# MIT-SPARK/Kimera-Semantics

Measured on AMD Instinct MI355X. Metric: Mvoxel-updates/s + frames/s, 640×480 @5cm voxels, 1/2/4/8 MI355X, higher is better.
Workload: dtype f32; 1 GPU; bag-replay stand-in: 640x480 depth+label trajectory (room), 'fast' integrator, 5 cm voxels, 5 m rays, trunc 0.2 m, p=0.8; pipeline_frames=12, parallelism=frame-sharded x1, points_per_frame=305657, rays_per_frame=85307, updates_per_frame=502687

## Files before the change

include/ks_hip.h:

```cpp
#ifndef KS_HIP_H_
#define KS_HIP_H_

#include <stddef.h>
#include <stdint.h>

#ifdef __cplusplus
extern "C" {
#endif

#define KS_NUM_LABELS 21

enum {
  KS_OK = 0,
  KS_ERR_INVALID_ARG = -1,
  KS_ERR_LABEL_RANGE = -2,
  KS_ERR_PROBABILITY = -3,
  KS_ERR_HIP = -4,
  KS_ERR_POOL_FULL = -5,
  KS_ERR_INDEX_RANGE = -6,
  KS_ERR_NO_DEVICE = -7,
  KS_ERR_UNSUPPORTED = -8,
  KS_ERR_PEER_FAILED = -9
};

// ... 174 lines not shown
typedef struct ks_objects_config {
  float min_weight;
  float surface_distance_m;
  uint32_t label_mask;
  uint32_t min_voxels;
} ks_objects_config;
typedef struct ks_objects_stats {
  uint64_t voxels_surface, components, objects, voxels_in_objects, largest_object_voxels, workspace_bytes;
} ks_objects_stats;
typedef struct ks_object {
  int32_t first_voxel[3];
  uint32_t n_voxels;
  int32_t bb_min[3], bb_max[3];
  int64_t sum[3];
  uint32_t label, pad;
} ks_object;
#define KS_OBJECT_NONE 0xffffffffu
int ks_objects_default_config(ks_objects_config* cfg);
int ks_objects_update(ks_ctx* ctx, const ks_objects_config* cfg, ks_objects_stats* stats );
int ks_objects_size(ks_ctx* ctx, size_t* n);
int ks_objects_download(ks_ctx* ctx, ks_object* out, size_t cap, size_t* n);
int ks_objects_download_blocks(ks_ctx* ctx, const int32_t* idx_xyz, size_t n, uint32_t* out );
int ks_objects_query(ks_ctx* ctx, const float* xyz , size_t n, uint32_t* id);

#define KS_TILE_BYTES 65536
int ks_get_tile_keys(ks_ctx* ctx, uint64_t* out, size_t cap, size_t* n);
int ks_export_tiles_device(ks_ctx* ctx, const uint32_t* slots, size_t n, void* d_payload);
int ks_merge_tiles_device(ks_ctx* ctx, const uint64_t* keys, size_t n, const void* d_payload);
int ks_clear(ks_ctx* ctx);
int ks_clear_voxels(ks_ctx* ctx);
typedef struct ks_remove_stats {
  uint64_t blocks_removed, tiles_removed, tiles_moved, tiles_resident , pool_capacity_tiles;
} ks_remove_stats;
int ks_remove_blocks(ks_ctx* ctx, const int32_t* idx_xyz, size_t n, ks_remove_stats* stats );
int ks_remove_distant_blocks(ks_ctx* ctx, const float center[3], float max_distance_m, ks_remove_stats* stats );
int ks_removed_blocks(ks_ctx* ctx, int32_t* out_xyz, size_t cap, size_t* n);
typedef struct ks_fuse_config {
  float min_weight;
  uint32_t pad;
  uint64_t max_workspace_bytes;
} ks_fuse_config;
typedef struct ks_fuse_stats {
  uint64_t tiles_source, tiles_candidate, tiles_touched, tiles_allocated, voxels_fused, chunks, workspace_bytes;
} ks_fuse_stats;
int ks_fuse_default_config(ks_fuse_config* cfg);
int ks_fuse_map(ks_ctx* dst, ks_ctx* src, const float T_D_S[7], const ks_fuse_config* cfg, ks_fuse_stats* stats );

typedef struct ks_mesh_index_stats {
  uint64_t corners, vertices, max_corners_per_vertex, workspace_bytes;
} ks_mesh_index_stats;
int ks_mesh_index(ks_ctx* ctx, ks_mesh_index_stats* stats );
int ks_mesh_index_size(ks_ctx* ctx, size_t* n_vertices, size_t* n_indices);
int ks_mesh_index_download(ks_ctx* ctx, float* xyz, float* normals, uint8_t* rgba, uint8_t* labels, uint32_t* object_ids,
                           size_t cap_vertices, uint32_t* indices, size_t cap_indices);
int ks_reset_tiles(ks_ctx* ctx, const uint32_t* slots, size_t n);
int ks_tile_owner(uint64_t tile_key, int world);
typedef struct ks_reduce_stats {
  uint64_t tiles_sent, tiles_received, tiles_local, bytes_sent;
} ks_reduce_stats;
int ks_reduce(ks_ctx* ctx, void* rccl_comm, int rank, int world, ks_reduce_stats* stats);

typedef struct ks_round_stats {
  uint64_t updates_marched, updates_applied, bytes_sent, origin_voxel_touched, rays_cast;
} ks_round_stats;
int ks_integrate_round_exact(ks_ctx* marcher, ks_ctx* owner, void* rccl_comm, int rank, int world, uint64_t first_frame,
                             const float T_G_C[7], const float* xyz, const uint8_t* rgba, const uint8_t* labels, size_t n,
                             int freespace_points, ks_round_stats* stats);

int ks_debug_radix_sort(ks_ctx* ctx, void* keys, uint32_t* vals, size_t n, int key_bits, unsigned end_bit);
int ks_debug_radix_sort_range(ks_ctx* ctx, void* keys, uint32_t* vals, size_t n, int key_bits, unsigned begin_bit, unsigned end_bit);
int ks_debug_radix_sort_batch(ks_ctx* ctx, uint64_t* keys, uint32_t* vals, const uint64_t* counts, int nb, size_t cap,
                              unsigned begin_bit, unsigned end_bit);

int ks_synchronize(ks_ctx* ctx);
void* ks_stream(ks_ctx* ctx);
int ks_flush(ks_ctx* ctx, ks_frame_stats* stats);
int ks_profile_enable(ks_ctx* ctx, int level);
int ks_early_out_iterations(ks_ctx* ctx, uint64_t* frames, uint64_t* iterations);
int ks_early_out_stats(ks_ctx* ctx, uint64_t out[5]);
int ks_profile_get(ks_ctx* ctx, ks_profile* out, int reset);
int ks_update_stats(ks_ctx* ctx, uint64_t out[4]);
int ks_pipeline_shape(ks_ctx* ctx, int32_t out[4]);
int ks_stream_plan(ks_ctx* ctx, int32_t out[8]);
int ks_seed_launch_shape(int32_t integration_order_mode, int32_t early_out_phase_growth, uint64_t cap_points, uint32_t* out, int32_t max_phases);

#ifdef __cplusplus
}
#endif
#endif
```

kimera_semantics_amd/binding.py:

```python
from __future__ import annotations

import ctypes as C
import os
import subprocess

import numpy as np

_HERE = os.path.dirname(os.path.abspath(__file__))
LIB_PATH = os.environ.get("KS_HIP_LIB") or os.path.join(_HERE, "libks_hip.so")
NUM_LABELS = 21

KS_METHOD_FAST, KS_METHOD_MERGED = 0, 1
KS_COLOR_MODE_COLOR, KS_COLOR_MODE_SEMANTIC, KS_COLOR_MODE_SEMANTIC_PROBABILITY = 0, 1, 2
KS_ORDER_MIXED, KS_ORDER_SORTED, KS_ORDER_MIXED_1024_GROUPS = 0, 1, 2
KS_BUNDLE_ORDER_REFERENCE, KS_BUNDLE_ORDER_CANONICAL = 0, 1
KS_EARLY_OUT_EXACT = 1
KS_ERR_LABEL_RANGE, KS_ERR_PROBABILITY, KS_ERR_POOL_FULL, KS_ERR_NO_DEVICE, KS_ERR_UNSUPPORTED = -2, -3, -5, -7, -8
KS_ERR_INVALID_ARG, KS_ERR_PEER_FAILED = -1, -9
KS_ERR_HIP, KS_ERR_INDEX_RANGE = -4, -6

STAGES = ["points", "sort_points", "rays", "march", "emit", "sort_pairs", "apply", "apply_long"]

TSDF_DTYPE = np.dtype([("distance", "<f4"), ("weight", "<f4"), ("color", "u1", (4,))])
SEM_DTYPE = np.dtype([("label", "u1"), ("pad", "u1", (3,)), ("priors", "<f4", (NUM_LABELS,)),
                      ("color", "u1", (4,))])

ABI_SYMBOLS = [
    "ks_default_config", "ks_create", "ks_destroy", "ks_last_error", "ks_set_color_to_label",
    "ks_integrate_points", "ks_integrate_points_device", "ks_integrate_depth", "ks_integrate_depth_device", "ks_num_blocks", "ks_get_block_indices",
    "ks_get_updated_block_indices", "ks_count_updated_voxels", "ks_download_updated_voxels", "ks_download_blocks", "ks_upload_blocks", "ks_host_alloc", "ks_host_free", "ks_get_tile_keys", "ks_export_tiles_device", "ks_merge_tiles_device", "ks_clear", "ks_clear_voxels", "ks_reset_tiles", "ks_tile_owner", "ks_reduce",
    "ks_debug_radix_sort", "ks_debug_radix_sort_range", "ks_debug_radix_sort_batch", "ks_synchronize", "ks_flush", "ks_stream",
    "ks_profile_enable", "ks_profile_get", "ks_early_out_iterations", "ks_early_out_stats", "ks_pipeline_shape", "ks_stream_plan", "ks_seed_launch_shape", "ks_update_stats", "ks_integrate_round_exact",
    "ks_mesh_default_config", "ks_mesh_update", "ks_mesh_size", "ks_mesh_download", "ks_mesh_changed_blocks",
    "ks_esdf_default_config", "ks_esdf_update", "ks_esdf_download_blocks", "ks_esdf_query",
    "ks_esdf_refresh", "ks_esdf_changed_blocks",
    "ks_render_default_config", "ks_render_view", "ks_render_view_device",
    "ks_align_default_config", "ks_align_points", "ks_align_points_device",
    "ks_objects_default_config", "ks_objects_update", "ks_objects_size", "ks_objects_download", "ks_objects_download_blocks", "ks_objects_query",
    "ks_remove_blocks", "ks_remove_distant_blocks", "ks_removed_blocks",
    "ks_fuse_default_config", "ks_fuse_map",
    "ks_mesh_index", "ks_mesh_index_size", "ks_mesh_index_download",
]


class KsConfig(C.Structure):
    _fields_ = [
        ("voxel_size", C.c_float), ("voxels_per_side", C.c_int32),
        ("truncation_distance", C.c_float), ("max_weight", C.c_float),
        ("min_ray_length_m", C.c_float), ("max_ray_length_m", C.c_float),
        ("voxel_carving_enabled", C.c_int32), ("use_const_weight", C.c_int32),
        ("allow_clear", C.c_int32), ("use_weight_dropoff", C.c_int32),
        ("use_sparsity_compensation_factor", C.c_int32), ("sparsity_compensation_factor", C.c_float),
        ("enable_anti_grazing", C.c_int32), ("start_voxel_subsampling_factor", C.c_float),
        ("max_consecutive_ray_collisions", C.c_int32), ("clear_checks_every_n_frames", C.c_int32),
        ("integration_order_mode", C.c_int32), ("integrator_threads", C.c_int32),
        ("method", C.c_int32), ("bundle_order", C.c_int32),
        ("semantic_measurement_probability", C.c_float), ("color_mode", C.c_int32),
        ("n_dynamic_labels", C.c_int32), ("dynamic_labels", C.c_uint8 * 32),
        ("label_rgba", (C.c_uint8 * 4) * 256),
        ("early_out_phase_growth", C.c_int32),
        ("device_id", C.c_int32), ("max_tiles", C.c_uint32), ("max_points", C.c_uint32), ("pipeline_frames", C.c_int32),
    ]


class KsRoundStats(C.Structure):
    _fields_ = [("updates_marched", C.c_uint64), ("updates_applied", C.c_uint64), ("bytes_sent", C.c_uint64),
                ("origin_voxel_touched", C.c_uint64), ("rays_cast", C.c_uint64)]


class KsFrameStats(C.Structure):
    _fields_ = [("n_points", C.c_uint64), ("n_valid_points", C.c_uint64), ("n_rays_cast", C.c_uint64),
                ("n_voxel_updates", C.c_uint64), ("n_blocks_allocated", C.c_uint64)]


class KsReduceStats(C.Structure):
    _fields_ = [("tiles_sent", C.c_uint64), ("tiles_received", C.c_uint64), ("tiles_local", C.c_uint64),
                ("bytes_sent", C.c_uint64)]


class KsMeshConfig(C.Structure):
    _fields_ = [("min_weight", C.c_float), ("only_stale", C.c_int32)]


class KsMeshStats(C.Structure):
    _fields_ = [("blocks_meshed", C.c_uint64), ("blocks_total", C.c_uint64), ("triangles_total", C.c_uint64),
                ("triangles_changed", C.c_uint64), ("degenerate_dropped", C.c_uint64)]


MESH_BLOCK_DTYPE = np.dtype([("block", "<i4", (3,)), ("first_vertex", "<u4"), ("n_vertices", "<u4")])


class KsEsdfConfig(C.Structure):
    _fields_ = [("min_weight", C.c_float), ("min_distance_m", C.c_float), ("max_distance_m", C.c_float), ("use_region", C.c_int32),
                ("region_min", C.c_int32 * 3), ("region_max", C.c_int32 * 3), ("max_workspace_bytes", C.c_uint64)]


class KsEsdfStats(C.Structure):
    _fields_ = [("voxels_observed", C.c_uint64), ("voxels_fixed", C.c_uint64), ("voxels_clamped", C.c_uint64),
                ("box_voxels", C.c_uint64 * 3), ("workspace_bytes", C.c_uint64)]


class KsEsdfRefreshStats(C.Structure):
    _fields_ = [("tiles_stale", C.c_uint64), ("tiles_recomputed", C.c_uint64), ("tiles_total", C.c_uint64),
                ("voxels_observed", C.c_uint64), ("voxels_fixed", C.c_uint64), ("voxels_clamped", C.c_uint64),
                ("workspace_bytes", C.c_uint64)]


ESDF_DTYPE = np.dtype([("distance", "<f4"), ("flags", "u1"), ("label", "u1"), ("pad", "u1", (2,))])


class KsRenderConfig(C.Structure):
    _fields_ = [("min_weight", C.c_float), ("min_range_m", C.c_float), ("max_range_m", C.c_float)]


class KsRenderStats(C.Structure):
# ... 44 lines not shown


def object_centroids(records, voxel_size) -> np.ndarray:
    r = np.asarray(records)
    return (r["sum"].astype(np.float64) / np.maximum(r["n_voxels"], 1)[:, None].astype(np.float64) + 0.5) * float(voxel_size)


KS_ALIGN_CONVERGED, KS_ALIGN_ITERATION_LIMIT, KS_ALIGN_TOO_FEW_INLIERS, KS_ALIGN_DEGENERATE = 0, 1, 2, 3


class KsProfile(C.Structure):
    _fields_ = [("ms", C.c_double * 8), ("launches", C.c_uint64 * 8), ("frames", C.c_uint64),
                ("updates", C.c_uint64), ("points", C.c_uint64), ("apply_kernel_ms", C.c_double),
                ("apply_kernel_launches", C.c_uint64), ("apply_kernel_updates", C.c_uint64),
                ("host_ms", C.c_double), ("host_wait_ms", C.c_double)]


def build(force: bool = False) -> str:
    src_dir = os.path.join(_HERE, "csrc")
    srcs = [os.path.join(src_dir, f) for f in ("ks_hip.hip", "ks_types.h", "ks_k_rays.h", "ks_k_bundle_order.h", "ks_k_march.h", "ks_k_exact.h", "ks_k_apply.h",
                                                "ks_k_apply_xl.h", "ks_k_shard.h", "ks_k_shard_merged.h", "ks_k_io.h", "ks_k_mesh.h", "ks_k_mesh_index.h", "ks_k_esdf.h", "ks_k_render.h", "ks_k_align.h", "ks_k_objects.h", "ks_k_remove.h", "ks_k_fuse.h", "ks_mc_tri_table.inc", "ks_device_math.h", "ks_radix_sort.h", "ks_owned.h")]
    srcs.append(os.path.join(_HERE, "..", "include", "ks_hip.h"))
    stale = (not os.path.exists(LIB_PATH)) or any(
        os.path.exists(s) and os.path.getmtime(s) > os.path.getmtime(LIB_PATH) for s in srcs)
    if force or stale:
        subprocess.check_call(["make", "-C", src_dir])
    return LIB_PATH


_lib = None


def lib():
    global _lib
    if _lib is None:
        if not os.path.exists(LIB_PATH):
            raise RuntimeError(f"{LIB_PATH} is missing: run `python -c 'import __graft_entry__ as g; g.build()'` "
                               "(the HIP path has no CPU fallback)")
        L = C.CDLL(LIB_PATH)
        vp = C.c_void_p
        L.ks_default_config.argtypes = [C.POINTER(KsConfig)]
        L.ks_create.argtypes = [C.POINTER(KsConfig), C.POINTER(vp)]
        L.ks_destroy.argtypes = [vp]
        L.ks_destroy.restype = None
        L.ks_last_error.argtypes = [vp]
        L.ks_last_error.restype = C.c_char_p
        L.ks_set_color_to_label.argtypes = [vp, vp, vp, C.c_size_t]
        L.ks_integrate_points.argtypes = [vp, vp, vp, vp, vp, C.c_size_t, C.c_int, C.POINTER(KsFrameStats)]
        L.ks_integrate_points_device.argtypes = [vp, vp, vp, vp, vp, C.c_size_t, C.c_int, C.POINTER(KsFrameStats)]
        L.ks_integrate_depth.argtypes = [vp, vp, vp, C.c_int, vp, vp, C.c_int, C.c_int, vp, C.c_int, C.POINTER(KsFrameStats)]
        L.ks_integrate_depth_device.argtypes = [vp, vp, vp, C.c_int, vp, vp, C.c_int, C.c_int, vp, C.c_int, C.POINTER(KsFrameStats)]
        L.ks_num_blocks.argtypes = [vp, C.POINTER(C.c_size_t)]
        L.ks_get_block_indices.argtypes = [vp, vp, C.c_size_t, C.POINTER(C.c_size_t)]
        L.ks_get_updated_block_indices.argtypes = [vp, vp, C.c_size_t, C.POINTER(C.c_size_t), C.c_int]
        L.ks_download_blocks.argtypes = [vp, vp, C.c_size_t, vp, vp]
        L.ks_count_updated_voxels.argtypes = [vp, C.POINTER(C.c_size_t), C.POINTER(C.c_size_t)]
        L.ks_download_updated_voxels.argtypes = [vp, vp, C.c_size_t, C.POINTER(C.c_size_t), vp, C.c_size_t, C.POINTER(C.c_size_t)]
        L.ks_upload_blocks.argtypes = [vp, vp, C.c_size_t, vp, vp]
        L.ks_host_alloc.argtypes = [C.c_size_t]
        L.ks_host_alloc.restype = C.c_void_p
        L.ks_host_free.argtypes = [vp]
        L.ks_host_free.restype = None
        L.ks_get_tile_keys.argtypes = [vp, vp, C.c_size_t, C.POINTER(C.c_size_t)]
        L.ks_export_tiles_device.argtypes = [vp, vp, C.c_size_t, vp]
        L.ks_merge_tiles_device.argtypes = [vp, vp, C.c_size_t, vp]
        L.ks_clear.argtypes = [vp]
        L.ks_clear_voxels.argtypes = [vp]
        L.ks_reset_tiles.argtypes = [vp, vp, C.c_size_t]
        L.ks_tile_owner.argtypes = [C.c_uint64, C.c_int]
        L.ks_reduce.argtypes = [vp, vp, C.c_int, C.c_int, C.POINTER(KsReduceStats)]
        L.ks_debug_radix_sort.argtypes = [vp, vp, vp, C.c_size_t, C.c_int, C.c_uint]
        L.ks_debug_radix_sort_range.argtypes = [vp, vp, vp, C.c_size_t, C.c_int, C.c_uint, C.c_uint]
        L.ks_debug_radix_sort_batch.argtypes = [vp, vp, vp, vp, C.c_int, C.c_size_t, C.c_uint, C.c_uint]
        L.ks_synchronize.argtypes = [vp]
        L.ks_flush.argtypes = [vp, C.POINTER(KsFrameStats)]
        L.ks_stream.argtypes = [vp]
        L.ks_stream.restype = vp
        L.ks_profile_enable.argtypes = [vp, C.c_int]
        L.ks_profile_get.argtypes = [vp, C.POINTER(KsProfile), C.c_int]
        L.ks_early_out_iterations.argtypes = [vp, C.POINTER(C.c_uint64), C.POINTER(C.c_uint64)]
        L.ks_early_out_stats.argtypes = [vp, C.POINTER(C.c_uint64)]
        L.ks_pipeline_shape.argtypes = [vp, C.POINTER(C.c_int32)]
        L.ks_stream_plan.argtypes = [vp, C.POINTER(C.c_int32)]
        L.ks_seed_launch_shape.argtypes = [C.c_int32, C.c_int32, C.c_uint64, C.POINTER(C.c_uint32), C.c_int32]
        L.ks_update_stats.argtypes = [vp, C.POINTER(C.c_uint64)]
        L.ks_integrate_round_exact.argtypes = [vp, vp, vp, C.c_int, C.c_int, C.c_uint64, vp, vp, vp, vp, C.c_size_t, C.c_int, C.POINTER(KsRoundStats)]
        L.ks_mesh_default_config.argtypes = [C.POINTER(KsMeshConfig)]
        L.ks_mesh_update.argtypes = [vp, C.POINTER(KsMeshConfig), C.POINTER(KsMeshStats)]
        L.ks_mesh_size.argtypes = [vp, C.POINTER(C.c_size_t), C.POINTER(C.c_size_t)]
        L.ks_mesh_download.argtypes = [vp, vp, C.c_size_t, vp, vp, vp, vp, C.c_size_t]
        L.ks_mesh_changed_blocks.argtypes = [vp, vp, C.c_size_t, C.POINTER(C.c_size_t)]
        L.ks_esdf_default_config.argtypes = [C.POINTER(KsEsdfConfig)]
        L.ks_esdf_update.argtypes = [vp, C.POINTER(KsEsdfConfig), C.POINTER(KsEsdfStats)]
        L.ks_esdf_download_blocks.argtypes = [vp, vp, C.c_size_t, vp]
        L.ks_esdf_query.argtypes = [vp, vp, C.c_size_t, vp, vp, vp]
        L.ks_esdf_refresh.argtypes = [vp, C.c_uint64, C.POINTER(KsEsdfRefreshStats)]
        L.ks_esdf_changed_blocks.argtypes = [vp, vp, C.c_size_t, C.POINTER(C.c_size_t)]
        L.ks_render_default_config.argtypes = [C.POINTER(KsRenderConfig)]
        L.ks_render_view.argtypes = [vp, vp, vp, C.c_int, C.c_int, C.POINTER(KsRenderConfig), vp, vp, vp, vp, C.POINTER(KsRenderStats)]
        L.ks_render_view_device.argtypes = [vp, vp, vp, C.c_int, C.c_int, C.POINTER(KsRenderConfig), vp, vp, vp, vp, C.POINTER(KsRenderStats)]
        L.ks_align_default_config.argtypes = [C.POINTER(KsAlignConfig)]
        L.ks_align_points.argtypes = [vp, vp, vp, C.c_size_t, C.POINTER(KsAlignConfig), vp, C.POINTER(KsAlignStats)]
        L.ks_align_points_device.argtypes = [vp, vp, vp, C.c_size_t, C.POINTER(KsAlignConfig), vp, C.POINTER(KsAlignStats)]
        L.ks_objects_default_config.argtypes = [C.POINTER(KsObjectsConfig)]
        L.ks_objects_update.argtypes = [vp, C.POINTER(KsObjectsConfig), C.POINTER(KsObjectsStats)]
        L.ks_objects_size.argtypes = [vp, C.POINTER(C.c_size_t)]
        L.ks_objects_download.argtypes = [vp, vp, C.c_size_t, C.POINTER(C.c_size_t)]
        L.ks_objects_download_blocks.argtypes = [vp, vp, C.c_size_t, vp]
        L.ks_objects_query.argtypes = [vp, vp, C.c_size_t, vp]
        L.ks_remove_blocks.argtypes = [vp, vp, C.c_size_t, C.POINTER(KsRemoveStats)]
        L.ks_remove_distant_blocks.argtypes = [vp, vp, C.c_float, C.POINTER(KsRemoveStats)]
        L.ks_removed_blocks.argtypes = [vp, vp, C.c_size_t, C.POINTER(C.c_size_t)]
        L.ks_fuse_default_config.argtypes = [C.POINTER(KsFuseConfig)]
        L.ks_fuse_map.argtypes = [vp, vp, vp, C.POINTER(KsFuseConfig), C.POINTER(KsFuseStats)]
        L.ks_mesh_index.argtypes = [vp, C.POINTER(KsMeshIndexStats)]
        L.ks_mesh_index_size.argtypes = [vp, C.POINTER(C.c_size_t), C.POINTER(C.c_size_t)]
        L.ks_mesh_index_download.argtypes = [vp, vp, vp, vp, vp, vp, C.c_size_t, vp, C.c_size_t]
        _lib = L
    return _lib


def default_config(**overrides) -> KsConfig:
    cfg = KsConfig()
    lib().ks_default_config(C.byref(cfg))
    apply_overrides(cfg, **overrides)
    return cfg


def apply_overrides(cfg, **overrides):
    for k, v in overrides.items():
        if k == "dynamic_labels":
            cfg.n_dynamic_labels = len(v)
            for i, lab in enumerate(v):
                cfg.dynamic_labels[i] = int(lab)
        elif k == "label_rgba":
            arr = np.ascontiguousarray(np.asarray(v, dtype=np.uint8).reshape(256, 4))
            C.memmove(cfg.label_rgba, arr.ctypes.data, 1024)
        else:
            if not hasattr(cfg, k):
                raise AttributeError(k)
            setattr(cfg, k, v)
    return cfg


class KsError(RuntimeError):
    def __init__(self, code, msg):
        super().__init__(f"ks error {code}: {msg}")
        self.code = code


def _ptr(a):
    return None if a is None else a.ctypes.data


class HipIntegrator:

    def __init__(self, cfg: KsConfig):
        self.cfg = cfg
        self.vps = cfg.voxels_per_side
        self._h = C.c_void_p()
        rc = lib().ks_create(C.byref(cfg), C.byref(self._h))
        if rc != 0:
            raise KsError(rc, lib().ks_last_error(None).decode())

    def _chk(self, rc):
        if rc != 0:
# ... 357 lines not shown
        return stats

    def reset_tiles(self, slots: np.ndarray):
        s = np.ascontiguousarray(slots, dtype=np.uint32)
        self._chk(lib().ks_reset_tiles(self._h, _ptr(s), len(s)))

    def reduce(self, rccl_comm, rank: int, world: int) -> dict:
        st = KsReduceStats()
        self._chk(lib().ks_reduce(self._h, C.c_void_p(rccl_comm) if rccl_comm else None, rank, world, C.byref(st)))
        return {"tiles_sent": st.tiles_sent, "tiles_received": st.tiles_received, "tiles_local": st.tiles_local,
                "bytes_sent": st.bytes_sent}

    def debug_radix_sort(self, keys: np.ndarray, vals=None, end_bit=None):
        keys = np.ascontiguousarray(keys).copy()
        bits = keys.dtype.itemsize * 8
        vals = None if vals is None else np.ascontiguousarray(vals, dtype=np.uint32).copy()
        self._chk(lib().ks_debug_radix_sort(self._h, _ptr(keys), _ptr(vals), keys.shape[0], bits,
                                            bits if end_bit is None else end_bit))
        return keys, vals

    def debug_radix_sort_range(self, keys: np.ndarray, vals=None, begin_bit=0, end_bit=None):
        keys = np.ascontiguousarray(keys).copy()
        bits = keys.dtype.itemsize * 8
        vals = None if vals is None else np.ascontiguousarray(vals, dtype=np.uint32).copy()
        self._chk(lib().ks_debug_radix_sort_range(self._h, _ptr(keys), _ptr(vals), keys.shape[0], bits, begin_bit,
                                                  bits if end_bit is None else end_bit))
        return keys, vals

    def debug_radix_sort_batch(self, keys: np.ndarray, vals: np.ndarray, counts, begin_bit, end_bit):
        keys = np.ascontiguousarray(keys, dtype=np.uint64).copy()
        vals = np.ascontiguousarray(vals, dtype=np.uint32).copy()
        counts = np.ascontiguousarray(counts, dtype=np.uint64)
        nb, cap = keys.shape
        assert vals.shape == (nb, cap) and counts.shape == (nb,)
        self._chk(lib().ks_debug_radix_sort_batch(self._h, _ptr(keys), _ptr(vals), _ptr(counts), nb, cap, begin_bit, end_bit))
        return keys, vals

    def synchronize(self):
        self._chk(lib().ks_synchronize(self._h))

    @property
    def stream(self) -> int:
        return lib().ks_stream(self._h) or 0

    def profile_enable(self, level=1):
        self._chk(lib().ks_profile_enable(self._h, int(level)))

    def early_out_stats(self):
        out = (C.c_uint64 * 5)()
        self._chk(lib().ks_early_out_stats(self._h, out))
        return dict(frames=int(out[0]), rounds=int(out[1]), fallbacks=int(out[2]), event_driven=bool(out[3]), pipelined=bool(out[4]))

    def integrate_round_exact(self, marcher: "HipIntegrator", rccl_comm, rank: int, world: int, first_frame: int, T_G_C, xyz, rgba, labels,
                              freespace=False) -> dict:
        T = np.ascontiguousarray(T_G_C, dtype=np.float32)
        n = 0 if xyz is None else len(xyz)
        x = None if xyz is None else np.ascontiguousarray(xyz, dtype=np.float32)
        c = None if rgba is None else np.ascontiguousarray(rgba, dtype=np.uint8)
        l = None if labels is None else np.ascontiguousarray(labels, dtype=np.uint8)
        st = KsRoundStats()
        self._chk(lib().ks_integrate_round_exact(marcher._h, self._h, rccl_comm, int(rank), int(world), int(first_frame), _ptr(T),
                                                 _ptr(x) if x is not None else None, _ptr(c) if c is not None else None,
                                                 _ptr(l) if l is not None else None, n, int(bool(freespace)), C.byref(st)))
        return dict(updates_marched=int(st.updates_marched), updates_applied=int(st.updates_applied), bytes_sent=int(st.bytes_sent),
                    origin_voxel_touched=bool(st.origin_voxel_touched), rays_cast=int(st.rays_cast))

    def update_stats(self):
        out = (C.c_uint64 * 4)()
        self._chk(lib().ks_update_stats(self._h, out))
        return dict(walked=int(out[0]), serial=int(out[1]), chunks=int(out[2]), replayed=int(out[3]))

    def pipeline_shape(self):
        out = (C.c_int32 * 4)()
        self._chk(lib().ks_pipeline_shape(self._h, out))
        return dict(lag=int(out[0]), slots=int(out[1]), batch=int(out[2]), march_streams=int(out[3]))

    def stream_plan(self):
        out = (C.c_int32 * 8)()
        self._chk(lib().ks_stream_plan(self._h, out))
        side = {1: "own", 0: "tail", -1: "none"}
        return dict(budget=int(out[0]), streams=int(out[1]), march_streams=int(out[2]), long=side[int(out[3])], xlong=side[int(out[4])],
                    march="own" if out[5] else "A", tail="own" if out[6] else "A", streams_held=int(out[7]))

    def early_out_iterations(self):
        f, it = C.c_uint64(), C.c_uint64()
        self._chk(lib().ks_early_out_iterations(self._h, C.byref(f), C.byref(it)))
        return f.value, it.value

    def flush(self) -> KsFrameStats:
        st = KsFrameStats()
        self._chk(lib().ks_flush(self._h, C.byref(st)))
        return st

    def profile(self, reset=False) -> dict:
        p = KsProfile()
        self._chk(lib().ks_profile_get(self._h, C.byref(p), int(reset)))
        return {"ms": {STAGES[i]: p.ms[i] for i in range(8)}, "launches": {STAGES[i]: p.launches[i] for i in range(8)},
                "frames": p.frames, "updates": p.updates, "points": p.points,
                "apply_kernel_ms": p.apply_kernel_ms, "apply_kernel_launches": p.apply_kernel_launches,
                "apply_kernel_updates": p.apply_kernel_updates, "host_ms": p.host_ms, "host_wait_ms": p.host_wait_ms}
```

kimera_semantics_amd/csrc/ks_hip.hip:

```cpp

#include <atomic>
#include <chrono>
#include <condition_variable>
#include <mutex>
#include <thread>
#include <cstring>
#include <string.h>

#include <dlfcn.h>
#include <hip/hip_runtime.h>
#include <hip/hip_ext.h>
#include <rccl/rccl.h>

#include <algorithm>
#include <iterator>
#include <cmath>
#include <cstdio>
#include <cstring>
#include <string>
#include <unordered_map>
#include <vector>

#include "../../include/ks_hip.h"
#include "ks_device_math.h"
// ... 18 lines not shown
#include "ks_k_render.h"
#include "ks_k_align.h"
#include "ks_k_objects.h"
#include "ks_k_remove.h"
#include "ks_k_fuse.h"

using namespace ksk;

namespace {

std::string g_create_error;

const char* dbg_env(const char* name) {
  const char* g = getenv("KS_DEBUG");
  return (g && g[0] == '1') ? getenv(name) : nullptr;
}

}

constexpr int kMaxLag = 16;
constexpr int kSlots = kMaxLag + 8;
constexpr int kMarchStreams = 8;
constexpr int kObsTables = 16;
struct HostSnap {
  Counters c;
  uint32_t n_tiles;
  uint32_t pad[7];
};
struct FrameSlot {
  int index = 0;
  DevBuf<RayDesc> d_rays;
  DevBuf<float> d_deltas;
  DevBuf<uint64_t> d_pairs;
  DevBuf<uint32_t> d_cnt;
  DevBuf<uint32_t> d_lp;
  DevBuf<unsigned long long> d_bt;
  DevBuf<uint8_t> d_live;
  DevBuf<uint32_t> d_seed_gen, d_seed_items, d_seed_n;
  bool wide = false;
  DevBuf<FrameParams> d_F;
  DevBuf<uint64_t> d_gkeys, d_rkeys;
  struct GraphSet {
    hipGraphExec_t g1 = nullptr, g2 = nullptr, g3 = nullptr;
    uint64_t key = 0;
    GraphSet() = default;
    GraphSet(const GraphSet&) = delete;
    GraphSet& operator=(const GraphSet&) = delete;
    ~GraphSet() { reset(); }
    void reset() {
      for (hipGraphExec_t* g : {&g1, &g2, &g3}) {
        if (*g) (void)hipGraphExecDestroy(*g);
        *g = nullptr;
      }
      key = 0;
    }
  } b_graphs[2];
  DevBuf<uint64_t> d_eo_keys[2];
  DevBuf<uint32_t> d_eo_vals[2];
  size_t eo_cap_marks = 0;
  DevBuf<uint4> d_eo_tab;
  DevBuf<unsigned long long> d_eo_xnode;
  DevBuf<uint32_t> d_eo_cnt_b, d_eo_ux, d_eo_dirty, d_eo_list[2], d_eo_chg, d_eo_consulted, d_eo_lp;
  DevBuf<unsigned long long> d_eo_bt;
  DevBuf<EoCtl> d_eo_ctl;
  DevBuf<uint32_t> d_eo_sort_ws;
  DevBuf<uint32_t> d_eo_hseq, d_eo_where;
  DevBuf<uint4> d_eo_rinfo, d_eo_ckpt;
  DevBuf<uint8_t> d_eo_hitb;
  DevBuf<unsigned long long> d_eo_bits_a, d_eo_bits_b;
  DevBuf<unsigned long long> d_eo_btp;
  Event eo_committed;
  Counters* d_counters = nullptr;
  DevBuf<uint32_t> d_ray_list;
  PinnedBuf<HostSnap> h_snap;
  Event a_done;
  Event ready;
  Event tail_done;
  Event fork, join;
  Event join_x;
  Event found;
  bool tail_recorded = false;
  bool join_recorded = false;
  bool b_launched = false;
  size_t steps_max = 0;
  uint64_t frame_no = 0;
  FrameParams F{};
  size_t n = 0;
  int prof_set = -1;
  bool pending = false;
  const Counters& counters() const { return h_snap->c; }
  uint32_t n_tiles() const { return h_snap->n_tiles; }
};

constexpr int kProfSets = 32;
constexpr int kStageEvents = KS_STAGE_COUNT + 3;
struct ProfSet {
  Event ev[kStageEvents];
  Event k0, k1;
  bool used = false, complete = false, stages = false, apply = false, applied = false;
  uint64_t n_pairs = 0, n_points = 0;
};

struct StreamPlanIn {
  bool uses_early_out = false;
  bool exact_early_out = false;
  bool frames_independent = true;
  int pipeline_frames = 0;
  int batch = 1;
  bool xlong = true;
  int budget = 4;
};
struct StreamPlan {
  int budget = 4;
  int n_march = 1;
  bool march_own = false;
  bool tail_own = false;
  bool long_own = true;
  bool xlong_own = true;
  int distinct = 1;
};
inline StreamPlan stream_plan(const StreamPlanIn& in) {
  StreamPlan p;
  p.budget = in.budget;
  if (in.pipeline_frames) {
    p.n_march = (!in.frames_independent || in.batch > 1) ? 1 : std::min(kMarchStreams, std::max(4, in.pipeline_frames));
    if (in.exact_early_out && p.n_march > 4) p.n_march = 4;
    if (in.exact_early_out && in.batch > 1) p.n_march = 2;
    if (!in.uses_early_out) p.n_march = 1;
    p.march_own = in.uses_early_out;
    p.tail_own = true;
  }
  p.long_own = true;
  p.xlong_own = in.xlong;
  auto count = [&p] { return 1 + (p.march_own ? p.n_march : 0) + (p.tail_own ? 1 : 0) + (p.long_own ? 1 : 0) + (p.xlong_own ? 1 : 0); };
  if (p.budget < 8 && count() > p.budget) p.xlong_own = false;
  if (p.budget < 8 && count() > p.budget) p.long_own = false;
  p.distinct = count();
  return p;
}
inline int hw_queue_budget() {
  auto number = [](const char* s, int* out) {
    if (!s) return false;
    char* end = nullptr;
    const long v = strtol(s, &end, 10);
    if (end == s) return false;
    *out = (int)std::min<long>(32, std::max<long>(1, v));
    return true;
  };
  int b = 4;
  number(getenv("GPU_MAX_HW_QUEUES"), &b);
  number(dbg_env("KS_HW_QUEUES"), &b);
  return b;
}

struct ks_ctx {
  Stream streams[kMarchStreams + 4];
  int n_streams = 0;
  ks_config cfg{};
  std::string err;
  hipStream_t stream = nullptr;
  hipStream_t stream_march_[kMarchStreams] = {};
  int n_march = 1;
  int batch = 1;
  std::vector<FrameSlot*> batch_slots;
  hipStream_t prof_march_stream = nullptr;
  hipStream_t stream_tail = nullptr;
  hipStream_t stream_long = nullptr;
  hipStream_t stream_xlong = nullptr;
  StreamPlan plan;
  bool xlong = true;
  float voxel_size_inv = 0.f, log_match = 0.f, log_non_match = 0.f;
  int vps_shift = 1;

  TileTable table{};
  Pool pool{};
  DevBuf<TileEntry> table_ent;
  DevBuf<uint64_t> table_slot_keys;
  DevBuf<uint4> pool_vox;
  DevBuf<uint8_t> pool_updated, pool_dirty;
  DevBuf<uint64_t> d_start_set;
  DevBuf<uint64_t> d_observed_[kObsTables];
  int n_obs = 1;
  uint64_t start_offset = 0, observed_offset = 0;
  int64_t reset_counter = 0;
  uint32_t obs_tag = 0, obs_tag_lo = 1;
  DevBuf<Counters> d_retry_counters;
  std::atomic<size_t> pairs_hint{0};
  bool uses_early_out = false;
  std::vector<SeedPhase> seed_phases;
  DevBuf<SeedPhase> d_seed_phases;
  size_t seed_cap_items = 0;
  std::thread tail_thread;
  std::mutex tail_mu;
  std::mutex capture_mu;
  std::condition_variable tail_cv;
  FrameSlot* tail_job = nullptr;
  bool tail_busy = false, tail_quit = false;
  int tail_rc = KS_OK;
  bool use_tail_thread = false;
  bool use_graphs = true;
  bool test_overlap = true;
  std::atomic<uint64_t> buffers_epoch{1};
  DevBuf<uint8_t> d_color_lut;
  DevBuf<uint32_t> d_label_lut;
  uint32_t tiles_initialised = 0;

  size_t cap_points = 0;
  DevBuf<float> d_xyz;
  DevBuf<uint8_t> d_rgba;
  DevBuf<uint8_t> d_labels;
  DevBuf<uint32_t> d_hash;
  DevBuf<uint32_t> d_skeys32, d_skeys32b;
  DevBuf<float4> d_gpw;
  DevBuf<uint64_t> d_ray_keys;
  DevBuf<uint2> d_glc;
  DevBuf<unsigned long long> d_long_list_[2];
  DevBuf<uint32_t> d_blong;
  std::atomic<uint32_t> bo_hint{~0u};
  bool bo_hint_fixed = false;
  DevBuf<uint64_t> d_key_overflow;
  uint32_t key_overflow_mask = 0;
  uint32_t key_bits = 0;
  DevBuf<uint64_t> d_pkeys, d_pkeys2;
  DevBuf<uint32_t> d_pvals, d_pvals2;
  DevBuf<uint32_t> d_order;
  DevBuf<uint32_t> d_inv_order;
  DevBuf<uint32_t> d_okeys, d_okeys2, d_ovals;
  size_t cap_pairs = 0;
  DevBuf<uint64_t> d_pairs2_[2];
  hipEvent_t pending_join = nullptr;
  ksrs::Workspace sort_ws, sort_ws_tail;
  bool exact_early_out = false;
  DevBuf<uint64_t> d_eo_keys[2];
  DevBuf<uint32_t> d_eo_vals[2];
  size_t cap_marks = 0;
  DevBuf<uint2> d_eo_range;
  DevBuf<uint64_t> d_eo_plain;
  DevBuf<uint32_t> d_eo_lp;
  DevBuf<unsigned long long> d_eo_bt;
  DevBuf<EoState> d_eo_state;
  PinnedBuf<EoState> h_eo_state;
  uint64_t eo_iterations = 0, eo_frames = 0;
  bool eo_device = false;
  int eo_bulk_rounds = 6;
  static constexpr int eo_sweeps = 12;
  int eo_sweep_chunks = 16;
  std::atomic<int> eo_want_bulk{0};
  DevBuf<uint32_t> d_eo_committed;
  uint32_t eo_frame_no = 0;
  hipEvent_t eo_last_commit = nullptr;
  std::atomic<size_t> eo_want_marks{0}, eo_want_x{0};
  size_t eo_cap_marks = 0, eo_cap_x = 0;
  std::atomic<uint64_t> eo_fallbacks{0};
  uint64_t eo_fallbacks_seen = 0;
  std::atomic<int> eo_hopeless{0};
  bool eo_device_off = false;
  bool use_bundle_rank = false;
  BoCtx bo{};
  BoSchedule bo_sched{};
  DevBuf<uint8_t> d_bo_slab;
  int bo_epochs = 0;
  DevBuf<int32_t> d_rx_counts;
  DevBuf<uint64_t> d_tx_keys, d_rx_keys;
  DevBuf<uint32_t> d_tx_slots;
  DevBuf<uint8_t> d_tx_payload, d_rx_payload;
  size_t cap_tx = 0, cap_rx = 0;
  DevBuf<uint32_t> d_xchg_u32;
  DevBuf<uint64_t> d_xchg_u64;
  DevBuf<uint8_t> d_state;
  FrameSlot slot[kSlots];
  int n_slots = 1;
  uint64_t frame_no = 0;
  ks_frame_stats owed{};
  DevBuf<int32_t> d_block_idx;
  DevBuf<uint8_t> d_tsdf_out, d_sem_out;
  DevBuf<uint8_t> d_vox_out;
  size_t cap_out_blocks = 0;

  DevBuf<uint32_t> d_depth_blocks;
  DevBuf<uint8_t> d_img_depth;
  DevBuf<uint8_t> d_img_aux;

  int profiling = 0;
  unsigned long long apply_runs_min_pairs = 1ull << 20;
  bool xl_parallel = true;
  unsigned long long xl_min_pairs = 1ull << 23;
  DevBuf<XlRun> d_xl_runs;
  DevBuf<XlHeader> d_xl_hdr;
  DevBuf<XlChunk> d_xl_chunks;
  DevBuf<uint32_t> d_xl_idx;
  bool shard_export = false;
  int shard_world = 1;
  uint64_t shard_frames_seen = 0;
  DevBuf<uint64_t> d_sh_okey[2];
  DevBuf<uint64_t> d_sh_gkey[2];
  DevBuf<uint32_t> d_sh_seq[2];
  DevBuf<float> d_sh_sdf[2];
  DevBuf<float> d_sh_uw[2];
  DevBuf<uint32_t> d_sh_counts;
  size_t cap_sh = 0;
  uint32_t sh_counts[65] = {0};
  uint64_t sh_exported = 0;
  DevBuf<uint64_t> d_sh_tk;
  DevBuf<uint64_t> d_sh_pairs[2];
  DevBuf<uint32_t> d_sh_vals[2];
  size_t cap_sh_rx = 0;
  DevBuf<uint32_t> d_shm_bno;
  DevBuf<float2> d_shm_btab;
  DevBuf<uint32_t> d_shm_mpos;
  DevBuf<uint32_t> d_shm_cnt;
  size_t cap_shm_n = 0;
  DevBuf<float> d_shm_mixed;
// ... 280 lines not shown
      if ((rc = c->slot[i].d_gkeys.alloc(c, cap))) return rc;
      if ((rc = c->slot[i].d_rkeys.alloc(c, cap))) return rc;
    }
    if (c->cfg.method == KS_METHOD_MERGED && (rc = c->slot[i].d_deltas.alloc(c, cap * kNumLabels))) return rc;
  }
  if ((rc = c->d_hash.alloc(c, cap))) return rc;
  if ((rc = c->d_skeys32.alloc(c, cap))) return rc;
  if ((rc = c->d_skeys32b.alloc(c, cap))) return rc;
  if ((rc = c->d_pkeys.alloc(c, cap))) return rc;
  if ((rc = c->d_pkeys2.alloc(c, cap))) return rc;
  if ((rc = c->d_pvals.alloc(c, cap))) return rc;
  if ((rc = c->d_pvals2.alloc(c, cap))) return rc;
  if ((rc = c->d_order.alloc(c, cap))) return rc;
  if ((rc = c->d_inv_order.alloc(c, cap))) return rc;
  if ((rc = c->d_okeys.alloc(c, cap))) return rc;
  if ((rc = c->d_okeys2.alloc(c, cap))) return rc;
  if ((rc = c->d_ovals.alloc(c, cap))) return rc;
  if (c->cfg.method == KS_METHOD_MERGED) {
    if ((rc = c->d_gpw.alloc(c, cap))) return rc;
    if ((rc = c->d_glc.alloc(c, cap))) return rc;
    if ((rc = c->d_ray_keys.alloc(c, cap))) return rc;
    if ((rc = c->d_blong.alloc(c, cap / kLongRun + 64))) return rc;
    if (c->key_bits) {
      size_t slots = 1024;
      while (slots < 2 * cap) slots <<= 1;
      if ((rc = c->d_key_overflow.alloc(c, slots))) return rc;
      HIPCHK(c, hipMemsetAsync(c->d_key_overflow, 0, slots * sizeof(uint64_t), c->stream));
      c->key_overflow_mask = (uint32_t)(slots - 1);
    }
  }
  if (c->use_bundle_rank && (rc = ensure_bundle_order(c, cap))) return rc;
  if (c->exact_early_out) {
    if ((rc = c->d_eo_lp.alloc(c, cap))) return rc;
    if ((rc = c->d_eo_bt.alloc(c, cap / kScanBlock + 2))) return rc;
    if ((rc = ensure_exact_points(c, cap))) return rc;
  }
  c->cap_points = cap;
  return KS_OK;
}

int ensure_pairs_in(ks_ctx* c, FrameSlot& S, size_t bound) {
  if (bound <= S.d_pairs.size()) return KS_OK;
  if (int rc = S.d_pairs.alloc(c, std::max<size_t>(bound, 1 << 20))) return rc;
  ++c->buffers_epoch;
  return KS_OK;
}
int ensure_pairs_out(ks_ctx* c, size_t n) {
  if (n <= c->cap_pairs) return KS_OK;
  const size_t cap = std::max<size_t>(n + n / 4, 1 << 20);
  c->cap_pairs = 0;
  int rc;
  HIPCHK(c, hipStreamSynchronize(c->stream_long));
  if (c->stream_xlong) HIPCHK(c, hipStreamSynchronize(c->stream_xlong));
  if (c->stream_tail) HIPCHK(c, hipStreamSynchronize(c->stream_tail));
  for (int b = 0; b < 2; ++b) {
    if ((rc = c->d_pairs2_[b].alloc(c, cap))) return rc;
    if ((rc = c->d_long_list_[b].alloc(c, cap / kLongRunLanes + 64 + cap / kXLongRun + 64))) return rc;
    if (c->long_lanes && (rc = c->d_long_sorted_[b].alloc(c, cap / kLongRunLanes + 64))) return rc;
  }
  if (c->d_xl_hdr && (rc = c->d_xl_fb.alloc(c, cap / kXLongRun + 64))) return rc;
  c->cap_pairs = cap;
  return KS_OK;
}

template <typename K>
int sort_keys(ks_ctx* c, K* a, K* b, size_t n, unsigned end_bit, K** result, unsigned begin_bit = 0, bool tail = false) {
  HIPCHK(c, (ksrs::sort<K, false>(tail ? c->sort_ws_tail : c->sort_ws, a, b, nullptr, nullptr, n, end_bit,
                                  tail ? c->stream_tail : c->stream, result, nullptr, begin_bit)));
  return KS_OK;
}
template <typename K>
int sort_pairs(ks_ctx* c, K* ka, K* kb, uint32_t* va, uint32_t* vb, size_t n, unsigned end_bit, K** kres,
               uint32_t** vres, unsigned begin_bit = 0) {
  HIPCHK(c, (ksrs::sort<K, true>(c->sort_ws, ka, kb, va, vb, n, end_bit, c->stream, kres, vres, begin_bit)));
  return KS_OK;
}

inline unsigned bits_for(uint64_t n) {
  unsigned b = 1;
  while (b < 64 && (1ull << b) < n) ++b;
  return b;
}

int launch_batch(ks_ctx* c);
int quiesce(ks_ctx* c);
int reset_set(ks_ctx* c, uint64_t* d_set0, uint64_t* offset, bool observed) {
  const bool full = ++(*offset) >= kFullResetThreshold;
  const bool retag = observed && !full && c->obs_tag + (uint32_t)c->cfg.clear_checks_every_n_frames + 2u >= kObsMaxTag;
  if (full || retag) {
    if (int rc = launch_batch(c)) return rc;
    if (full && c->exact_early_out) {
      if (int rc = quiesce(c)) return rc;
    }
    if (int rc = sync_march(c)) return rc;
    if (full) *offset = 0;
    for (int t = 0; t < (observed ? c->n_obs : 1); ++t) {
      uint64_t* d_set = observed ? c->d_observed_[t] : d_set0;
      if (full) {
        HIPCHK(c, hipMemsetAsync(d_set, 0, (observed ? 2 : 1) * (sizeof(uint64_t) << kSetBits), c->stream));
        const uint64_t poison = observed ? kObsPoison : ~0ull;
        HIPCHK(c, hipMemcpyAsync(d_set, &poison, sizeof(poison), hipMemcpyHostToDevice, c->stream));
      } else {
        hipLaunchKernelGGL(k_obs_retag, dim3((2u << kSetBits) / 256), dim3(256), 0, c->stream, d_set);
      }
    }
    if (observed && full && c->d_eo_plain) {
      HIPCHK(c, hipMemsetAsync(c->d_eo_plain, 0, sizeof(uint64_t) << kSetBits, c->stream));
      const uint64_t poison = ~0ull;
      HIPCHK(c, hipMemcpyAsync(c->d_eo_plain, &poison, sizeof(poison), hipMemcpyHostToDevice, c->stream));
    }
    HIPCHK(c, hipStreamSynchronize(c->stream));
    if (observed) c->obs_tag = 0;
  }
  if (observed) c->obs_tag_lo = c->obs_tag + 1;
  return KS_OK;
}

inline void stage_mark(ks_ctx* c, int set, int ev) {
  if (set >= 0 && c->pset[set].stages)
    (void)hipEventRecord(c->pset[set].ev[ev], ev <= 3 ? c->stream : ev <= 5 ? c->prof_march_stream : c->stream_tail);
}

void resolve_prof(ks_ctx* c, int set) {
  ProfSet& P = c->pset[set];
  if (!P.used || !P.complete) return;
  (void)hipEventSynchronize(P.ev[kStageEvents - 1]);
  if (P.stages) {
    for (int s = 0; s < KS_STAGE_COUNT; ++s) {
      float ms = 0.f;
      const int a = s < 3 ? s : s == 3 ? 4 : s + 2;
      if (hipEventElapsedTime(&ms, P.ev[a], P.ev[a + 1]) == hipSuccess) {
        c->prof.ms[s] += ms;
        c->prof.launches[s] += 1;
      }
    }
  }
  if (P.applied) {
    float kms = 0.f;
    if (hipEventElapsedTime(&kms, P.k0, P.k1) == hipSuccess) {
      c->prof.apply_kernel_ms += kms;
      c->prof.apply_kernel_launches += 1;
      c->prof.apply_kernel_updates += P.n_pairs;
    }
  }
  c->prof.frames += 1;
  c->prof.updates += P.n_pairs;
  c->prof.points += P.n_points;
  P.used = P.complete = P.applied = false;
}

SlotView slot_view(const FrameSlot& S, Counters* counters = nullptr) {
  SlotView v{};
  v.F = S.d_F;
  v.rays = S.d_rays;
  v.cnt = S.d_cnt;
  v.lp = S.d_lp;
  v.bt = S.d_bt;
  v.ray_list = S.d_ray_list;
  v.pairs = S.d_pairs;
  v.pairs_cap = (unsigned long long)S.d_pairs.size();
  v.C = counters ? counters : S.d_counters;
  v.host_snap = (uint32_t*)S.h_snap.get();
  v.eo_stats = S.d_eo_ctl ? &S.d_eo_ctl->n_x : nullptr;
  v.seed_gen = S.d_seed_gen;
  v.seed_items = S.d_seed_items;
  v.seed_n = S.d_seed_n;
  return v;
}

void launch_emit(ks_ctx* c, const BatchView& V, uint32_t nb, bool wide, hipStream_t st) {
  const size_t n = c->cap_points;
  const size_t lds = ((2 * n + kScanBlock - 1) / kScanBlock) * sizeof(unsigned long long);
  if (!(c->cfg.method == KS_METHOD_MERGED && c->cfg.enable_anti_grazing)) {
    if (wide || c->cfg.method == KS_METHOD_MERGED || !c->uses_early_out) {
      hipLaunchKernelGGL(k_emit_lane<8>, dim3((uint32_t)((n + 31) / 32), nb), dim3(256), lds, st, V, c->table, c->pool);
    } else {
      hipLaunchKernelGGL(k_emit_lane<16>, dim3((uint32_t)((n + 63) / 64), nb), dim3(256), lds, st, V, c->table, c->pool);
    }
  } else if (wide) {
    hipLaunchKernelGGL(k_emit<64>, dim3((uint32_t)((n + 3) / 4), nb), dim3(256), lds, st, V, c->table, c->pool);
  } else {
    hipLaunchKernelGGL(k_emit<16>, dim3((uint32_t)((n + 15) / 16), nb), dim3(256), lds, st, V, c->table, c->pool);
  }
}

void enqueue_stage_b(ks_ctx* c, const BatchView& V, uint32_t nb, bool wide, hipStream_t sm, size_t steps_max, int part = 0) {
  const ks_config& cfg = c->cfg;
  const size_t n = c->cap_points;
  if (c->uses_early_out && part != 2) {
    for (size_t j = 0; j < c->seed_phases.size(); ++j) {
      const SeedPhase& P = c->seed_phases[j];
      if (P.item_cap == 0) continue;
      const uint32_t steps_cap = (uint32_t)((steps_max + 3) & ~(size_t)3);
      const size_t lds_wave = (size_t)test_lds_words64(steps_cap) * sizeof(unsigned long long);
      const uint32_t wpb = lds_wave * 4 <= 60 * 1024 ? 4u : lds_wave * 2 <= 60 * 1024 ? 2u : 1u;
      const dim3 grid((P.item_cap + wpb - 1) / wpb, nb), block(64 * wpb);
      if (c->test_overlap) hipLaunchKernelGGL(k_test<true>, grid, block, lds_wave * wpb, sm, V, P.g0, P.g1, (uint32_t)j, P.item_off, P.item_cap, steps_cap);
      else hipLaunchKernelGGL(k_test<false>, grid, block, lds_wave * wpb, sm, V, P.g0, P.g1, (uint32_t)j, P.item_off, P.item_cap, steps_cap);
    }
  }
  if (part == 1) return;
  if (cfg.method == KS_METHOD_MERGED && cfg.enable_anti_grazing)
    hipLaunchKernelGGL(k_count_grazing<16>, dim3((uint32_t)((n + 15) / 16), nb), dim3(256), 0, sm, V);
  hipLaunchKernelGGL(k_scan_local, dim3((uint32_t)(((cfg.method == KS_METHOD_MERGED ? 2 : 1) * n + kScanBlock - 1) / kScanBlock), nb),
                     dim3(1024), 0, sm, V);
  launch_emit(c, V, nb, wide, sm);
  hipLaunchKernelGGL(k_publish, dim3(nb), dim3(64), 0, sm, V, (const uint32_t*)c->table.n_tiles);
}

int ensure_marks(ks_ctx* c, size_t n) {
  if (n <= c->cap_marks) return KS_OK;
  const size_t cap = std::max<size_t>(n + n / 4, 1 << 20);
  c->cap_marks = 0;
  int rc;
  for (int b = 0; b < 2; ++b) {
    if ((rc = c->d_eo_keys[b].alloc(c, cap))) return rc;
    if ((rc = c->d_eo_vals[b].alloc(c, cap))) return rc;
  }
  c->cap_marks = cap;
  return KS_OK;
}
constexpr int kEoMaxIterations = 4096;
int exact_early_out(ks_ctx* c, FrameSlot& S, hipStream_t st, Counters* counters = nullptr) {
  const size_t n = S.n;
  Counters* const d_counters = counters ? counters : S.d_counters;
// ... 240 lines not shown
        going = going || (w[0] != 0u && w[1] == 0u);
      }
      if (!going || chunk >= c->eo_sweep_chunks) break;
      enqueue_sweeps(c, Bt, nb, c->eo_sweeps, sm);
    }
    hipLaunchKernelGGL(k_eo2_sweep_done, dim3(nb), dim3(64), 0, sm, Bt);
    return KS_OK;
  }
  int exact_device() const {
    int rc;
    auto seed_and_rounds = [&] {
      enqueue_stage_b(c, V, nb, S0.wide, sm, steps_max, 1);
      return enqueue_exact_rounds(c, slots, nb, sm);
    };
    auto finish = [&] {
      for (uint32_t k = 0; k < nb; ++k) enqueue_exact_finish(c, *slots[k], sm);
      return KS_OK;
    };
    auto emission = [&] { return enqueue_stage_b(c, V, nb, S0.wide, sm, steps_max, 2), KS_OK; };
    bool graphs = c->use_graphs && !S0.wide;
    if (graphs && (G.key != key || !G.g1 || !G.g2 || !G.g3)) {
      std::lock_guard<std::mutex> cap(c->capture_mu);
      G.reset();
      if ((G.g1 = capture_graph(sm, seed_and_rounds)) && (G.g2 = capture_graph(sm, finish)) && (G.g3 = capture_graph(sm, emission))) {
        G.key = key;
      } else {
        (void)hipGetLastError();
        G.reset();
        c->use_graphs = graphs = false;
      }
    }
    if (graphs) HIPCHK(c, hipGraphLaunch(G.g1, sm));
    else if ((rc = seed_and_rounds()) || (S0.wide && (rc = sweeps_host_driven()))) return rc;
    if (c->eo_last_commit && c->eo_last_commit != S0.eo_committed) HIPCHK(c, hipStreamWaitEvent(sm, c->eo_last_commit, 0));
    if (graphs) HIPCHK(c, hipGraphLaunch(G.g2, sm));
    else finish();
    HIPCHK(c, hipEventRecord(S0.eo_committed, sm));
    c->eo_last_commit = S0.eo_committed;
    if (graphs) HIPCHK(c, hipGraphLaunch(G.g3, sm));
    else emission();
    return KS_OK;
  }
  int exact_host() const {
    enqueue_stage_b(c, V, nb, S0.wide, sm, steps_max, 1);
    if (int rc = exact_early_out(c, S0, sm)) return rc;
    enqueue_stage_b(c, V, nb, S0.wide, sm, steps_max, 2);
    return KS_OK;
  }
  int plain_or_replayed() const {
    if (c->use_graphs && (G.key != key || !G.g1)) {
      std::lock_guard<std::mutex> cap(c->capture_mu);
      G.reset();
      if ((G.g1 = capture_graph(sm, [&] { return enqueue_stage_b(c, V, nb, S0.wide, sm, steps_max), KS_OK; }))) {
        G.key = key;
      } else {
        (void)hipGetLastError();
        c->use_graphs = false;
      }
    }
    if (c->use_graphs && G.g1) HIPCHK(c, hipGraphLaunch(G.g1, sm));
    else enqueue_stage_b(c, V, nb, S0.wide, sm, steps_max);
    return KS_OK;
  }
};

int launch_batch(ks_ctx* c) {
  if (c->batch_slots.empty()) return KS_OK;
  std::vector<FrameSlot*> slots;
  slots.swap(c->batch_slots);
  const uint32_t nb = (uint32_t)slots.size();
  FrameSlot& S0 = *slots[0];
  hipStream_t sm = c->batch > 1 ? c->stream_march_[(S0.frame_no / (uint64_t)c->batch) % (uint64_t)c->n_march] : march_stream(c, S0.frame_no);
  c->prof_march_stream = sm;
  if (sm != c->stream) HIPCHK(c, hipStreamWaitEvent(sm, slots[nb - 1]->a_done, 0));
  const bool stage_events = nb == 1 && S0.prof_set >= 0 && c->pset[S0.prof_set].stages;
  if (stage_events) (void)hipEventRecord(c->pset[S0.prof_set].ev[4], sm);
  BatchView V{};
  size_t steps_max = 0;
  ParamsBatch PB{};
  for (uint32_t k = 0; k < nb; ++k) {
    FrameSlot& S = *slots[k];
    S.F.observed = observed_table(c, S.frame_no);
    if (c->exact_early_out) S.F.eo_frame = c->eo_frame_no++;
    PB.F[k] = S.F;
    PB.out[k] = S.d_F;
    V.s[k] = slot_view(S);
    steps_max = std::max(steps_max, S.steps_max);
  }
  if (nb == 1) hipLaunchKernelGGL(k_set_params, dim3(1), dim3(64), 0, sm, slots[0]->F, slots[0]->d_F);
  else hipLaunchKernelGGL(k_set_params_batch, dim3(nb), dim3(64), 0, sm, PB);
  const uint64_t key = ((uint64_t)c->cap_points << 24) ^ (c->buffers_epoch.load() << 4) ^ (S0.wide ? 1u : 0u) ^ ((uint64_t)nb << 1);
  const BatchLaunch B{c, slots.data(), nb, S0, sm, V, steps_max, key, S0.b_graphs[nb == (uint32_t)c->batch ? 0 : 1]};
  if (int rc = !c->exact_early_out ? B.plain_or_replayed() : c->eo_device && !c->eo_device_off ? B.exact_device() : B.exact_host()) return rc;
  for (uint32_t k = 0; k < nb; ++k) {
    HIPCHK(c, hipEventRecord(slots[k]->ready, sm));
    slots[k]->b_launched = true;
  }
  if (stage_events) (void)hipEventRecord(c->pset[S0.prof_set].ev[5], sm);
  return KS_OK;
}

void fill_frame_params(ks_ctx* c, FrameParams& F, const float Tq[7], size_t n, int freespace) {
  const ks_config& cfg = c->cfg;
  F = FrameParams{};
  F.T.w = Tq[0];
  F.T.v = {Tq[1], Tq[2], Tq[3]};
  F.T.t = {Tq[4], Tq[5], Tq[6]};
  F.voxel_size_inv = c->voxel_size_inv;
  F.min_ray = cfg.min_ray_length_m;
  F.max_ray = cfg.max_ray_length_m;
  F.trunc = cfg.truncation_distance;
  F.start_inv = cfg.start_voxel_subsampling_factor * c->voxel_size_inv;
  F.log_match = c->log_match;
  F.log_non_match = c->log_non_match;
  F.tsdf.voxel_size = cfg.voxel_size;
  F.tsdf.trunc = cfg.truncation_distance;
  F.tsdf.max_weight = cfg.max_weight;
  F.tsdf.dropoff_denominator = cfg.truncation_distance - cfg.voxel_size;
  F.tsdf.sparsity_factor = cfg.sparsity_compensation_factor;
  F.tsdf.use_dropoff = cfg.use_weight_dropoff;
  F.tsdf.use_sparsity = cfg.use_sparsity_compensation_factor;
  F.start_offset = c->start_offset;
  F.observed_offset = c->observed_offset;
  F.obs_tag = c->obs_tag;
  F.obs_tag_lo = c->obs_tag_lo;
  F.max_collisions = cfg.max_consecutive_ray_collisions;
  F.n = (uint32_t)n;
  const uint32_t q = (uint32_t)(n / kOrderStep);
  const bool by_1024 = cfg.integration_order_mode == KS_ORDER_MIXED_1024_GROUPS;
  F.order_groups = q == 0 ? 1u : by_1024 ? kOrderStep : q;
  F.order_per = q == 0 ? 0u : by_1024 ? q : kOrderStep;
  F.chains = order_chains(cfg.integration_order_mode, n);
  F.carving = cfg.voxel_carving_enabled;
  F.allow_clear = cfg.allow_clear;
  F.freespace = freespace;
  F.use_const_weight = cfg.use_const_weight;
  F.method = cfg.method;
  F.color_mode = cfg.color_mode;
  F.sorted_order = cfg.integration_order_mode == KS_ORDER_SORTED;
  F.n_dynamic = cfg.n_dynamic_labels;
  const unsigned pb = bits_for(n);
  F.point_mask = (1u << pb) - 1u;
  F.clear_bit = (cfg.method == KS_METHOD_MERGED) ? (1u << pb) : 0u;
  F.seq_bits = pb + (cfg.method == KS_METHOD_MERGED ? 1u : 0u);
  F.inv_order = F.sorted_order ? c->d_inv_order : nullptr;
  std::memcpy(F.dynamic_labels, cfg.dynamic_labels, 32);
  F.early_out = c->uses_early_out;
}
void begin_prof_set(ks_ctx* c, FrameSlot& S, size_t n) {
  const int set = (int)(c->frame_no % kProfSets);
  resolve_prof(c, set);
  ProfSet& P = c->pset[set];
  P.used = true;
  P.complete = P.applied = false;
  P.stages = c->profiling == 1;
  P.apply = c->profiling == 1 || (c->frame_no % 4) == 0;
  P.n_points = n;
  P.n_pairs = 0;
  S.prof_set = set;
}
int stage_a_fast(ks_ctx* c, FrameSlot& S, const float* d_xyz, const uint8_t* d_rgba, const uint8_t* d_labels, size_t n) {
  const FrameParams& F = S.F;
  hipStream_t st = c->stream;
  const uint32_t nb1k = (uint32_t)((n + 1023) / 1024);
  hipLaunchKernelGGL(k_points_fast, dim3(nb1k), dim3(1024), 0, st, F, d_xyz, d_rgba, d_labels, c->d_color_lut,
                     S.d_rays, c->d_hash, c->d_skeys32, c->d_pvals, S.d_cnt, S.d_live, S.d_counters);
  stage_mark(c, S.prof_set, 1);
  uint32_t *sk = nullptr, *sv = nullptr;
  if (int rc = sort_pairs(c, c->d_skeys32.get(), c->d_skeys32b.get(), c->d_pvals.get(), c->d_pvals2.get(), n, kSetBits + 1, &sk, &sv)) return rc;
  stage_mark(c, S.prof_set, 2);
  hipLaunchKernelGGL(k_dedup, dim3(nb1k), dim3(1024), 0, st, F, sk, sv, c->d_hash, c->d_start_set, S.d_ray_list, S.d_rays, S.d_cnt, S.d_live, S.d_counters);
  if (c->uses_early_out && n > 0) {
    const uint32_t n_gen = (uint32_t)((n + F.chains - 1) / F.chains);
    uint32_t n_ph = 0;
    while (n_ph < c->seed_phases.size() && c->seed_phases[n_ph].g0 < n_gen) ++n_ph;
    HIPCHK(c, hipMemsetAsync(S.d_seed_n, 0, c->seed_phases.size() * sizeof(uint32_t), st));
    hipLaunchKernelGGL(k_seed_list, dim3((F.chains + 63u) / 64u, n_ph), dim3(64 * kSeedSegs), 0, st, F, (const SeedPhase*)c->d_seed_phases,
                       (const uint8_t*)S.d_live, S.d_seed_gen, S.d_seed_items, S.d_seed_n, S.d_counters);
  }
  hipLaunchKernelGGL(k_dedup_commit, dim3(nb1k), dim3(1024), 0, st, F, sk, sv, c->d_hash, c->d_start_set, S.d_counters);
  return KS_OK;
}
void enqueue_bundle_order(ks_ctx* c, hipStream_t st, size_t n, const uint64_t* sk, const uint32_t* sv) {
  const uint32_t capb = (uint32_t)((c->cap_points + kBoBlock - 1) / kBoBlock);
  const size_t lds_f = (2 * c->cap_points / kBoBlock + 3) * sizeof(uint32_t), lds_e = ((size_t)capb + 2) * sizeof(uint32_t);
  hipLaunchKernelGGL(k_bo_scan_flags, dim3((uint32_t)((2 * n + kBoBlock - 1) / kBoBlock)), dim3(kBoBlock), 0, st, (uint32_t)n, c->bo);
  hipLaunchKernelGGL(k_bo_init, dim3((uint32_t)((n + kBoBlock - 1) / kBoBlock)), dim3(kBoBlock), lds_f, st, (uint32_t)n, sk, sv, c->bo);
  const uint32_t nbb = (uint32_t)((n + kBoBlock - 1) / kBoBlock);
  int e_small = 0;
  while (e_small < c->bo_epochs && c->bo_sched.b[e_small] <= kBoSmallBuckets) ++e_small;
  if (e_small > 0) hipLaunchKernelGGL(k_bo_small, dim3(2), dim3(kBoBlock), 0, st, c->bo, e_small);
  const size_t nh_floor = c->bo_hint_fixed ? (e_small > 0 ? (size_t)c->bo_sched.t[e_small - 1] + 1 : 1) : 2 * (size_t)kBoSmallBuckets;
  const size_t nh = std::min<size_t>(n, std::max<size_t>(c->bo_hint.load(std::memory_order_relaxed), nh_floor));
  int e_last = -1;
  for (int e = e_small; e <= c->bo_epochs; ++e) {
    if (e > 0 && c->bo_sched.t[e - 1] >= nh) break;
    hipLaunchKernelGGL(k_bo_link, dim3(nbb, 2), dim3(kBoBlock), lds_e, st, c->bo, e, (e == e_small && e_small > 0) ? 1 : 0);
    if (e < c->bo_epochs && c->bo_sched.t[e] < nh)
      hipLaunchKernelGGL(k_bo_walk, dim3(nbb, 2), dim3(kBoBlock), 0, st, c->bo, e);
    else
      e_last = e;
  }
  if (nh < n && e_last >= 0 && e_last < c->bo_epochs) hipLaunchKernelGGL(k_bo_rest, dim3(2), dim3(kBoBlock), lds_e, st, c->bo, e_last);
}
int stage_a_merged(ks_ctx* c, FrameSlot& S, const float* d_xyz, const uint8_t* d_rgba, const uint8_t* d_labels, size_t n, const uint32_t* order_ptr) {
  const ks_config& cfg = c->cfg;
  FrameParams& F = S.F;
  hipStream_t st = c->stream;
  const uint32_t nb = (uint32_t)((n + 255) / 256);
  const uint32_t nb1k = (uint32_t)((n + 1023) / 1024);
  if (c->key_bits) {
    const float reach = cfg.max_ray_length_m + 2.0f * cfg.voxel_size;
    const float tq[3] = {F.T.t.x, F.T.t.y, F.T.t.z};
    for (int a = 0; a < 3; ++a) {
      const float lo = std::floor((tq[a] - reach) * c->voxel_size_inv) - 2.0f;
      F.key_base[a] = (int32_t)std::min(std::max(lo, -2.0e9f), 2.0e9f);
    }
    F.key_bits = c->key_bits;
  }
  hipLaunchKernelGGL(k_points_merged, dim3(nb1k), dim3(1024), 0, st, F, d_xyz, d_rgba, d_labels, c->d_color_lut, c->d_pkeys, c->d_skeys32, c->d_pvals,
                     S.d_cnt, c->use_bundle_rank ? c->bo.flag : nullptr, c->d_key_overflow, c->key_overflow_mask, S.d_counters);
  stage_mark(c, S.prof_set, 1);
  uint64_t* sk = nullptr;
  uint32_t *sk32 = nullptr, *sv = nullptr;
  if (c->key_bits) {
    if (int rc = sort_pairs(c, c->d_skeys32.get(), c->d_skeys32b.get(), c->d_pvals.get(), c->d_pvals2.get(), n, 32, &sk32, &sv)) return rc;
    sk = c->d_pkeys;
// ... 184 lines not shown
  HIPCHK(c, hipStreamSynchronize(st));
  if (int rc = ensure_pairs_in(c, S, (size_t)cnt->n_pairs + (size_t)cnt->n_pairs / 4)) return rc;
  return repeat_emission(c, S, st, false, cnt, new_tiles);
}
int take_error_exits(ks_ctx* c, int set, hipStream_t st, uint32_t err) {
  skip_update_stages(c, set);
  finish_prof(c, set, st, 0);
  if (err & kErrLabel) {
    c->err = "semantic label >= 21 (CHECK_LT in the reference)";
    return KS_ERR_LABEL_RANGE;
  }
  c->fatal = true;
  c->err = (err & kErrPool) ? "voxel tile pool exhausted: raise ks_config.max_tiles" : "voxel index out of the packed range / tile table full";
  return (err & kErrPool) ? KS_ERR_POOL_FULL : KS_ERR_INDEX_RANGE;
}
#define KS_LAUNCH_TIMED_IF(timed, ev0, ev1, kernel, grid, block, stream, ...)                 \
  if (timed) hipExtLaunchKernelGGL(kernel, grid, block, 0, stream, ev0, ev1, 0, __VA_ARGS__); \
  else hipLaunchKernelGGL(kernel, grid, block, 0, stream, __VA_ARGS__)
struct UpdateLaunch {
  ks_ctx* c;
  const FrameSlot& S;
  const FrameParams& F;
  hipStream_t st, sl, sx;
  int set, par;
  uint64_t* sp;
  unsigned long long n_pairs, *d_long_list, *d_xlong_list;
  bool by_runs, time_apply, lanes_on;
  template <int MODE, bool MERGED> void apply() const {
    if (by_runs) {
      const uint32_t rb = (uint32_t)((n_pairs + kRunPer * 256u - 1) / (kRunPer * 256u));
      KS_LAUNCH_TIMED_IF(time_apply, c->pset[set].k0, c->pset[set].k1, (k_apply_runs<MODE, MERGED, 256u>), dim3(rb), dim3(256), st, F, n_pairs, sp,
                         S.d_rays.get(), S.d_deltas.get(), c->table, c->pool, c->d_label_lut.get(), kLongRun);
    } else {
      const uint32_t ab = (uint32_t)((n_pairs + 255) / 256);
      KS_LAUNCH_TIMED_IF(time_apply, c->pset[set].k0, c->pset[set].k1, (k_apply<MODE, MERGED>), dim3(ab), dim3(256), st, F, n_pairs, sp,
                         S.d_rays.get(), S.d_deltas.get(), c->table, c->pool, c->d_label_lut.get(), d_long_list, S.d_counters);
    }
  }
  template <int MODE> void xlong_runs() const {
    const uint32_t xb = (uint32_t)std::min<unsigned long long>(n_pairs / kXLongRun + 1, 512);
    if (c->xl_parallel && n_pairs >= c->xl_min_pairs) {
      hipLaunchKernelGGL(k_xl_measure<MODE>, dim3(kXlMaxRuns / 256), dim3(256), 0, sx, F, n_pairs, (const uint64_t*)sp, c->pool,
                         (const unsigned long long*)d_xlong_list, (const Counters*)S.d_counters, c->d_xl_runs);
      hipLaunchKernelGGL(k_xl_number, dim3(1), dim3(1024), 0, sx, (const unsigned long long*)d_xlong_list, (const Counters*)S.d_counters,
                         c->d_xl_runs, c->d_xl_idx, c->d_xl_fb, c->d_xl_hdr, c->cap_xl_chunks);
      hipLaunchKernelGGL(k_xl_chunks, dim3(4096), dim3(256), 0, sx, F, (const uint64_t*)sp, (const RayDesc*)S.d_rays, (const float*)S.d_deltas,
                         c->table, c->d_xl_runs, (const uint32_t*)c->d_xl_idx, (const XlHeader*)c->d_xl_hdr, c->d_xl_chunks);
      hipLaunchKernelGGL(k_xl_walk<MODE>, dim3(2048), dim3(64), 0, sx, F, (const uint64_t*)sp, (const RayDesc*)S.d_rays, (const float*)S.d_deltas,
                         c->table, c->pool, (const uint32_t*)c->d_label_lut, c->d_xl_runs, (const uint32_t*)c->d_xl_idx, c->d_xl_hdr,
                         (const XlChunk*)c->d_xl_chunks, c->d_xl_fb);
      hipLaunchKernelGGL(k_apply_xlong<MODE>, dim3(xb), dim3(256), 0, sx, F, n_pairs, sp, S.d_rays, S.d_deltas, c->table, c->pool, c->d_label_lut,
                         (const unsigned long long*)c->d_xl_fb, (const uint32_t*)&c->d_xl_hdr->n_fallback);
    } else {
      hipLaunchKernelGGL(k_apply_xlong<MODE>, dim3(xb), dim3(256), 0, sx, F, n_pairs, sp, S.d_rays, S.d_deltas, c->table, c->pool, c->d_label_lut,
                         d_xlong_list, (const uint32_t*)&S.d_counters->n_xlong);
    }
  }
  template <int MODE> void long_runs() const {
    const uint32_t lb = (uint32_t)std::min<unsigned long long>(n_pairs / kLongRun + 1, 4096);
    if (lanes_on) {
      const uint32_t cap_long = (uint32_t)(n_pairs / (kLongRun + 1) + 1);
      hipLaunchKernelGGL(k_long_measure, dim3((cap_long + 255) / 256), dim3(256), 0, sl, F.seq_bits, n_pairs, (const uint64_t*)sp, d_long_list,
                         (const Counters*)S.d_counters, c->d_long_hdr_[par], kLongRun);
      hipLaunchKernelGGL(k_long_bucket, dim3((cap_long + 255) / 256), dim3(256), 0, sl, (const unsigned long long*)d_long_list,
                         (const Counters*)S.d_counters, c->d_long_hdr_[par], c->d_long_sorted_[par]);
      hipLaunchKernelGGL((k_apply_long_lanes<MODE, 6u>), dim3((cap_long / 64 + kLongClasses + 3) / 4), dim3(256), 0, sl, F, (const uint64_t*)sp,
                         (const RayDesc*)S.d_rays, (const float*)S.d_deltas, c->table, c->pool, (const uint32_t*)c->d_label_lut,
                         (const LongHdr*)c->d_long_hdr_[par], (const unsigned long long*)c->d_long_sorted_[par]);
      hipLaunchKernelGGL(k_apply_long<MODE>, dim3(std::min<uint32_t>(lb, 1024u)), dim3(128), 0, sl, F, n_pairs, sp, S.d_rays, S.d_deltas, c->table,
                         c->pool, c->d_label_lut, (const unsigned long long*)c->d_long_sorted_[par], (const Counters*)S.d_counters,
                         (const LongHdr*)c->d_long_hdr_[par]);
    } else {
      hipLaunchKernelGGL(k_apply_long<MODE>, dim3(lb), dim3(128), 0, sl, F, n_pairs, sp, S.d_rays, S.d_deltas, c->table, c->pool, c->d_label_lut,
                         d_long_list, S.d_counters);
    }
  }
  template <int MODE> void launch() const {
    c->cfg.method == KS_METHOD_MERGED ? apply<MODE, true>() : apply<MODE, false>();
    stage_mark(c, set, 9);
    if (sx) xlong_runs<MODE>();
    long_runs<MODE>();
  }
};
#undef KS_LAUNCH_TIMED_IF
int enqueue_update(ks_ctx* c, FrameSlot& S, hipStream_t st, unsigned long long n_pairs, uint32_t new_tiles, int set) {
  if (n_pairs == 0) {
    if (c->pending_join) HIPCHK(c, hipStreamWaitEvent(st, c->pending_join, 0));
    c->pending_join = nullptr;
    skip_update_stages(c, set);
    return KS_OK;
  }
  const FrameParams& F = S.F;
  int rc;
  if ((rc = ensure_pairs_out(c, n_pairs))) return rc;
  stage_mark(c, set, 7);
  const unsigned end_bit = F.seq_bits + 9 + bits_for(new_tiles);
  uint64_t* sp = nullptr;
  const int par = (int)(S.frame_no & 1u);
  unsigned long long* const d_long_list = c->d_long_list_[par];
  if ((rc = sort_keys(c, S.d_pairs.get(), c->d_pairs2_[par].get(), n_pairs, std::min(56u, end_bit), &sp, F.seq_bits, true))) return rc;
  stage_mark(c, set, 8);
  const bool by_runs = n_pairs >= c->apply_runs_min_pairs;
  const bool time_apply = set >= 0 && c->pset[set].apply;
  if (time_apply) c->pset[set].applied = true;
  hipStream_t sl = c->stream_long, sx = c->stream_xlong;
  const bool long_beside = sl != st, xlong_beside = sx && sx != st;
  unsigned long long* const d_xlong_list = sx ? d_long_list + (c->cap_pairs / kLongRunLanes + 64) : nullptr;
  const bool lanes_on = by_runs && sx && c->long_lanes && n_pairs >= c->long_lanes_min_pairs;
  const bool find_beside = by_runs && xlong_beside && long_beside;
  const dim3 find_grid((uint32_t)((n_pairs + 256 * kFindLongItems - 1) / (256 * kFindLongItems)));
  if (!find_beside)
    hipLaunchKernelGGL(k_find_long, find_grid, dim3(256), 0, st, F.seq_bits, n_pairs, (const uint64_t*)sp, d_long_list, d_xlong_list,
                       S.d_counters, kLongRun);
  if (c->pending_join) HIPCHK(c, hipStreamWaitEvent(st, c->pending_join, 0));
  c->pending_join = nullptr;
  if (long_beside || xlong_beside) HIPCHK(c, hipEventRecord(S.fork, st));
  if (long_beside) HIPCHK(c, hipStreamWaitEvent(sl, S.fork, 0));
  if (lanes_on) HIPCHK(c, hipMemsetAsync(c->d_long_hdr_[par], 0, sizeof(LongHdr), sl));
  if (find_beside) {
    hipLaunchKernelGGL(k_find_long, find_grid, dim3(256), 0, sl, F.seq_bits, n_pairs, (const uint64_t*)sp, d_long_list, d_xlong_list,
                       S.d_counters, kLongRun);
    HIPCHK(c, hipEventRecord(S.found, sl));
    HIPCHK(c, hipStreamWaitEvent(sx, S.found, 0));
  } else if (xlong_beside) {
    HIPCHK(c, hipStreamWaitEvent(sx, S.fork, 0));
  }
  const UpdateLaunch U{c, S, F, st, sl, sx, set, par, sp, n_pairs, d_long_list, d_xlong_list, by_runs, time_apply, lanes_on};
  switch (c->cfg.color_mode) {
    case KS_COLOR_MODE_COLOR: U.launch<KS_COLOR_MODE_COLOR>(); break;
    case KS_COLOR_MODE_SEMANTIC: U.launch<KS_COLOR_MODE_SEMANTIC>(); break;
    default: U.launch<KS_COLOR_MODE_SEMANTIC_PROBABILITY>(); break;
  }
  if (xlong_beside) {
    HIPCHK(c, hipEventRecord(S.join_x, sx));
    HIPCHK(c, hipStreamWaitEvent(sl, S.join_x, 0));
  }
  if (long_beside) {
    HIPCHK(c, hipEventRecord(S.join, sl));
    S.join_recorded = true;
    if (!(set >= 0 && c->pset[set].stages)) c->pending_join = S.join;
    else HIPCHK(c, hipStreamWaitEvent(st, S.join, 0));
  }
  return KS_OK;
}

int frame_tail(ks_ctx* c, FrameSlot& S) {
  if (!S.pending) return KS_OK;
  S.pending = false;
  if (c->fatal) return KS_OK;
  int rc;
  if (!S.b_launched && (rc = launch_batch(c))) return rc;
  hipStream_t st = c->stream_tail;
  const auto w0 = std::chrono::steady_clock::now();
  HIPCHK(c, hipEventSynchronize(S.ready));
  if (c->profiling) c->prof.host_wait_ms += std::chrono::duration<double, std::milli>(std::chrono::steady_clock::now() - w0).count();
  Counters cnt = S.counters();
  uint32_t new_tiles = std::min(S.n_tiles(), c->cfg.max_tiles);
  const uint32_t tiles_before = c->tiles_initialised;
  const int set = S.prof_set;
  stage_mark(c, set, 6);
  if (c->eo_device && !c->eo_device_off) {
    c->eo_frames += 1;
    c->eo_iterations += S.h_snap->pad[2];
    if (!(cnt.err & kErrExact)) c->eo_hopeless.store(0, std::memory_order_relaxed);
  }
  if ((cnt.err & kErrExact) && !(cnt.err & (kErrLabel | kErrIndex)) && (rc = repair_after_fallback(c, S, st, &cnt, &new_tiles))) return rc;
  c->pairs_hint.store(std::max<size_t>(c->pairs_hint.load(std::memory_order_relaxed), cnt.n_pairs), std::memory_order_relaxed);
  if ((cnt.err & kErrPairs) && !(cnt.err & ~kErrPairs) && (rc = repair_after_overflow(c, S, st, &cnt, &new_tiles))) return rc;
  if (new_tiles > c->tiles_initialised) {
    hipLaunchKernelGGL(k_init_tiles, dim3(new_tiles - c->tiles_initialised), dim3(512), 0, st, c->pool, c->tiles_initialised);
    c->tiles_initialised = new_tiles;
  }
  if (cnt.err) return take_error_exits(c, set, st, cnt.err);
  const unsigned long long n_pairs = cnt.n_pairs;
  const bool marcher = c->shard_export;
  if (marcher) skip_update_stages(c, set);
  if ((rc = marcher ? shard_export_frame(c, S, n_pairs, st) : enqueue_update(c, S, st, n_pairs, new_tiles, set))) return rc;
  finish_prof(c, set, st, n_pairs);
  HIPCHK(c, hipEventRecord(S.tail_done, st));
  S.tail_recorded = true;
  if (!marcher) HIPCHK(c, hipGetLastError());
  owe_stats(c, S, cnt, n_pairs, !marcher && new_tiles > tiles_before ? new_tiles - tiles_before : 0u);
  if (c->use_bundle_rank && !c->bo_hint_fixed && !marcher) {
    const uint32_t want = cnt.n_rays + cnt.n_rays / 4u + 2048u;
    const uint32_t cur = c->bo_hint.load(std::memory_order_relaxed);
    c->bo_hint.store(cur == ~0u ? want : std::max(want, cur - cur / 64u), std::memory_order_relaxed);
  }
  return KS_OK;
}

void deliver_stats(ks_ctx* c, ks_frame_stats* stats) {
  if (stats) *stats = c->owed;
  c->owed = ks_frame_stats{};
}

int flush_pending(ks_ctx* c) {
  for (int k = 0; k < c->n_slots; ++k) {
    FrameSlot& S = c->slot[(c->frame_no + k) % (uint64_t)c->n_slots];
    if (S.pending) {
      const int rc = frame_tail(c, S);
      if (rc) return rc;
    }
  }
  return KS_OK;
}

int ensure_exchange(ks_ctx* c, size_t n) {
  if (n <= c->d_xchg_u64.size()) return KS_OK;
  const size_t cap = std::max<size_t>(n + n / 2, 1024);
  c->d_xchg_u64.release();
  if (int rc = c->d_xchg_u32.alloc(c, 2 * cap + 2)) return rc;
  return c->d_xchg_u64.alloc(c, cap);
}

int quiesce(ks_ctx* c) {
  const int rc = flush_pending(c);
  if (c->stream_tail != c->stream) HIPCHK(c, hipStreamSynchronize(c->stream_tail));
  HIPCHK(c, hipStreamSynchronize(c->stream_long));
  c->pending_join = nullptr;
  if (int rc2 = sync_march(c)) return rc2;
  HIPCHK(c, hipStreamSynchronize(c->stream));
  return rc;
}

void tail_worker(ks_ctx* c) {
  (void)hipSetDevice(c->cfg.device_id);
  std::unique_lock<std::mutex> lk(c->tail_mu);
  for (;;) {
    c->tail_cv.wait(lk, [&] { return c->tail_job != nullptr || c->tail_quit; });
    if (c->tail_quit) return;
    FrameSlot* S = c->tail_job;
    c->tail_job = nullptr;
    lk.unlock();
    int rc;
    {
      std::lock_guard<std::mutex> cap(c->capture_mu);
      rc = frame_tail(c, *S);
    }
    lk.lock();
    c->tail_rc = rc;
    c->tail_busy = false;
    c->tail_cv.notify_all();
  }
}
void tail_post(ks_ctx* c, FrameSlot* S) {
  std::lock_guard<std::mutex> lk(c->tail_mu);
  c->tail_job = S;
  c->tail_busy = true;
  c->tail_rc = KS_OK;
  c->tail_cv.notify_all();
// ... 357 lines not shown
    c->eo_device = c->exact_early_out && !(hl && hl[0] == '1');
    if (c->exact_early_out && (!c->eo_device || c->cfg.clear_checks_every_n_frames > 1)) c->cfg.pipeline_frames = 0;
    const bool wide_rays = steps_max_of(c->cfg, (float)(1.0 / cfg->voxel_size)) > 400;
    if (c->exact_early_out && wide_rays) c->cfg.pipeline_frames = 0;
    c->eo_bulk_rounds = wide_rays ? 32 : 20;
  }
  c->uses_early_out = uses_early_out;
  c->use_bundle_rank = cfg->method == KS_METHOD_MERGED && cfg->bundle_order == KS_BUNDLE_ORDER_REFERENCE;
  if (const char* bh = dbg_env("KS_BO_HINT")) {
    c->bo_hint_fixed = true;
    c->bo_hint.store(atoi(bh) > 0 ? (uint32_t)atoi(bh) : ~0u, std::memory_order_relaxed);
  }
  if (cfg->method == KS_METHOD_MERGED && !cfg->enable_anti_grazing) {
    const double extent = 2.0 * std::ceil(((double)cfg->max_ray_length_m + 2.0 * (double)cfg->voxel_size) / (double)cfg->voxel_size) + 8.0;
    unsigned w = 1;
    while (w < 32 && (double)(1u << w) < extent) ++w;
    if (const char* kb = dbg_env("KS_KEY_WINDOW_BITS")) w = (unsigned)std::max(0, atoi(kb));
    c->key_bits = (w >= 1 && w <= 10) ? w : 0;
  }
  c->log_match = lm;
  c->log_non_match = lnm;
  c->voxel_size_inv = (float)(1.0 / cfg->voxel_size);
  c->vps_shift = vps == 8 ? 0 : vps == 16 ? 1 : vps == 32 ? 2 : 3;
#define CRCHK(expr)                                                        \
  do {                                                                     \
    hipError_t e_ = (expr);                                                \
    if (e_ != hipSuccess) {                                                \
      g_create_error = std::string(#expr) + ": " + hipGetErrorString(e_);  \
      ks_destroy(c);                                                       \
      return KS_ERR_HIP;                                                   \
    }                                                                      \
  } while (0)
#define CRKS(expr)                \
  do {                            \
    if ((expr) != KS_OK) {        \
      g_create_error = c->err;    \
      ks_destroy(c);              \
      return KS_ERR_HIP;          \
    }                             \
  } while (0)
  auto new_stream = [c](hipStream_t* out) {
    Stream& s = c->streams[c->n_streams];
    if (int rc = s.create(c, hipStreamNonBlocking)) return rc;
    ++c->n_streams;
    *out = s;
    return (int)KS_OK;
  };
  CRCHK(hipSetDevice(cfg->device_id));
  CRKS(new_stream(&c->stream));
  const bool frames_independent = !uses_early_out || c->cfg.clear_checks_every_n_frames <= 1;
  c->batch = 1;
  if (const char* ov = dbg_env("KS_TEST_OVERLAP")) c->test_overlap = atoi(ov) != 0;
  if (c->cfg.pipeline_frames >= 2 && frames_independent && (!c->exact_early_out || c->eo_device) && c->cfg.integration_order_mode != KS_ORDER_SORTED) {
    c->batch = c->cfg.pipeline_frames >= 16 ? 8 : c->cfg.pipeline_frames >= 8 ? 4 : 1;
  }
  c->n_slots = !c->cfg.pipeline_frames ? 1 : (c->cfg.pipeline_frames > 8 || c->batch > 4) ? kSlots : 12;
  {
    const char* xp = dbg_env("KS_XLONG");
    c->xlong = xp ? atoi(xp) != 0 : true;
    StreamPlanIn in;
    in.uses_early_out = uses_early_out;
    in.exact_early_out = c->exact_early_out;
    in.frames_independent = frames_independent;
    in.pipeline_frames = c->cfg.pipeline_frames;
    in.batch = c->batch;
    in.xlong = c->xlong;
    in.budget = hw_queue_budget();
    c->plan = stream_plan(in);
  }
  {
    const StreamPlan& P = c->plan;
    c->n_march = P.n_march;
    for (int i = 0; i < P.n_march; ++i) {
      if (P.march_own) CRKS(new_stream(&c->stream_march_[i]));
      else c->stream_march_[i] = c->stream;
    }
    if (P.tail_own) CRKS(new_stream(&c->stream_tail));
    else c->stream_tail = c->stream;
    if (P.long_own) CRKS(new_stream(&c->stream_long));
    else c->stream_long = c->stream_tail;
    if (P.xlong_own) CRKS(new_stream(&c->stream_xlong));
    else if (c->xlong) c->stream_xlong = c->stream_tail;
    if (const char* ar = dbg_env("KS_APPLY_RUNS")) c->apply_runs_min_pairs = atoi(ar) ? 0ull : ~0ull;
    if (const char* ll = dbg_env("KS_LONG_LANES")) {
      c->long_lanes = atoi(ll) != 0;
      if (atoi(ll) == 2) c->long_lanes_min_pairs = 0ull;
    }
    if (c->long_lanes)
      for (int b = 0; b < 2; ++b) CRKS(c->d_long_hdr_[b].alloc(c, 1));
    if (const char* xl = dbg_env("KS_XL_PARALLEL")) {
      c->xl_parallel = atoi(xl) != 0;
      if (atoi(xl) == 2) c->xl_min_pairs = 0ull;
    }
    if (const char* xc = dbg_env("KS_XL_CAP_CHUNKS")) c->cap_xl_chunks = (uint32_t)std::max(1, atoi(xc));
    if (c->stream_xlong && c->xl_parallel) {
      CRKS(c->d_xl_runs.alloc(c, kXlMaxRuns));
      CRKS(c->d_xl_idx.alloc(c, kXlMaxRuns));
      CRKS(c->d_xl_hdr.alloc(c, 1));
      CRCHK(hipMemset(c->d_xl_hdr, 0, sizeof(XlHeader)));
      CRKS(c->d_xl_chunks.alloc(c, c->cap_xl_chunks));
    }
  }
  for (auto& P : c->pset) {
    for (auto& e : P.ev) CRKS(e.create(c, 0));
    CRKS(P.k0.create(c, 0));
    CRKS(P.k1.create(c, 0));
  }
  uint32_t cap = 1024;
  while (cap < 2u * cfg->max_tiles) cap <<= 1;
  c->table.mask = cap - 1;
  c->table.max_tiles = cfg->max_tiles;
  const size_t mt = cfg->max_tiles;
  CRKS(c->table_ent.alloc(c, cap));
  CRKS(c->table_slot_keys.alloc(c, mt));
  c->table.ent = c->table_ent;
  c->table.slot_keys = c->table_slot_keys;
  CRCHK(hipMemset(c->table.ent, 0xff, cap * sizeof(TileEntry)));
  CRKS(c->pool_vox.alloc(c, mt * kTileVoxels * 8));
  CRKS(c->pool_updated.alloc(c, kFlagPlane + mt));
  CRKS(c->pool_dirty.alloc(c, mt));
  c->pool.vox = c->pool_vox;
  c->pool.updated = c->pool_updated;
  c->pool.dirty = c->pool_dirty;
  CRCHK(hipMemset(c->pool.updated, 0, mt));
  CRCHK(hipMemset(c->pool.dirty, 0, mt));
  CRCHK(hipMemset(c->pool.mesh_stale(), 0, mt));
  CRKS(c->d_start_set.alloc(c, (size_t)1 << kSetBits));
  c->n_obs = (uses_early_out && frames_independent) ? std::min(kObsTables, std::max(c->n_march, c->batch * c->n_march)) : 1;
  for (int t = 0; t < c->n_obs; ++t) {
    CRKS(c->d_observed_[t].alloc(c, (size_t)2 << kSetBits));
    CRCHK(hipMemset(c->d_observed_[t], 0, 2 * (sizeof(uint64_t) << kSetBits)));
    CRCHK(hipMemcpy(c->d_observed_[t], &kObsPoison, 8, hipMemcpyHostToDevice));
  }
  CRCHK(hipMemset(c->d_start_set, 0, sizeof(uint64_t) << kSetBits));
  const uint64_t poison = ~0ull;
  CRCHK(hipMemcpy(c->d_start_set, &poison, 8, hipMemcpyHostToDevice));
  CRKS(c->d_retry_counters.alloc(c, 1));
  if (c->exact_early_out) {
    CRKS(c->d_eo_committed.alloc(c, 16));
    CRCHK(hipMemset(c->d_eo_committed, 0, 64));
    CRKS(c->d_eo_range.alloc(c, (size_t)1 << kSetBits));
    CRKS(c->d_eo_plain.alloc(c, (size_t)1 << kSetBits));
    CRCHK(hipMemset(c->d_eo_plain, 0, sizeof(uint64_t) << kSetBits));
    CRCHK(hipMemcpy(c->d_eo_plain, &poison, 8, hipMemcpyHostToDevice));
    CRKS(c->d_eo_state.alloc(c, 1));
    CRKS(c->h_eo_state.alloc(c, 1));
  }
  CRKS(c->d_label_lut.alloc(c, 256));
  CRCHK(hipMemcpy(c->d_label_lut, cfg->label_rgba, 1024, hipMemcpyHostToDevice));
  static_assert(sizeof(Counters) == 32, "snapshot layout");
  CRKS(c->d_state.alloc(c, 64 * (kSlots + 1)));
  CRCHK(hipMemset(c->d_state, 0, 64 * (kSlots + 1)));
  c->table.n_tiles = (uint32_t*)(c->d_state + 64 * kSlots);
  for (int i = 0; i < kSlots; ++i) {
    FrameSlot& S = c->slot[i];
    S.index = i;
    S.d_counters = (Counters*)(c->d_state + 64 * i);
    CRKS(S.h_snap.alloc(c, 1));
    CRKS(S.d_F.alloc(c, 1));
    std::memset(S.h_snap, 0, sizeof(HostSnap));
    for (Event* e : {&S.a_done, &S.ready, &S.tail_done, &S.fork, &S.join, &S.join_x, &S.found}) CRKS(e->create(c, hipEventDisableTiming));
  }
#undef CRKS
#undef CRCHK
  c->pairs_hint.store((size_t)cfg->max_points * 4, std::memory_order_relaxed);
  size_t eo_marks0 = std::max<size_t>((size_t)1 << 20, 4 * (size_t)cfg->max_points), eo_x0 = std::max<size_t>((size_t)1 << 17, (size_t)cfg->max_points);
// ... 2443 lines not shown
    HIPCHK(d, hipStreamSynchronize(st));
    HIPCHK(d, hipGetLastError());
    if (stats) {
      stats->tiles_touched += nu;
      stats->voxels_fused += voxels;
      stats->tiles_allocated = d->tiles_initialised - tiles_before;
    }
  }
  return KS_OK;
}

int ks_clear_voxels(ks_ctx* c) {
  if (!c) return KS_ERR_INVALID_ARG;
  return clear_impl(c, true);
}

int ks_flush(ks_ctx* c, ks_frame_stats* stats) {
  if (!c) return KS_ERR_INVALID_ARG;
  if (stats) std::memset(stats, 0, sizeof(*stats));
  const int rc = flush_pending(c);
  deliver_stats(c, stats);
  return rc;
}

int ks_synchronize(ks_ctx* c) {
  if (!c) return KS_ERR_INVALID_ARG;
  if (int rc = quiesce(c)) return rc;
  HIPCHK(c, hipStreamSynchronize(c->stream));
  return KS_OK;
}

void* ks_stream(ks_ctx* c) { return c ? (void*)c->stream : nullptr; }

#ifdef KS_STATS
int ks_debug_test_stats(unsigned long long* out16) {
  if (hipMemcpyFromSymbol(out16, HIP_SYMBOL(g_test_stats), 16 * sizeof(unsigned long long)) != hipSuccess) return KS_ERR_HIP;
  unsigned long long z[16] = {0};
  if (hipMemcpyToSymbol(HIP_SYMBOL(g_test_stats), z, sizeof(z)) != hipSuccess) return KS_ERR_HIP;
  return KS_OK;
}
#endif

int ks_early_out_iterations(ks_ctx* c, uint64_t* frames, uint64_t* iterations) {
  if (!c) return KS_ERR_INVALID_ARG;
  if (frames) *frames = c->eo_frames;
  if (iterations) *iterations = c->eo_iterations;
  return KS_OK;
}

int ks_early_out_stats(ks_ctx* c, uint64_t out[5]) {
  if (!c || !out) return KS_ERR_INVALID_ARG;
  out[0] = c->eo_frames;
  out[1] = c->eo_iterations;
  out[2] = c->eo_fallbacks.load(std::memory_order_relaxed);
  out[3] = (c->eo_device && !c->eo_device_off) ? 1 : 0;
  out[4] = (c->exact_early_out && c->cfg.pipeline_frames > 0) ? 1 : 0;
  return KS_OK;
}

int ks_update_stats(ks_ctx* c, uint64_t out[4]) {
  if (!c || !out) return KS_ERR_INVALID_ARG;
  out[0] = out[1] = out[2] = out[3] = 0;
  if (!c->d_xl_hdr) return KS_OK;
  if (int rc = quiesce(c)) return rc;
  if (c->stream_xlong) HIPCHK(c, hipStreamSynchronize(c->stream_xlong));
  XlHeader h;
  HIPCHK(c, hipMemcpy(&h, c->d_xl_hdr, sizeof(h), hipMemcpyDeviceToHost));
  out[0] = h.tot_walked;
  out[1] = h.tot_fallback;
  out[2] = h.tot_chunks;
  out[3] = h.tot_replayed;
  return KS_OK;
}

int ks_pipeline_shape(ks_ctx* c, int32_t out[4]) {
  if (!c || !out) return KS_ERR_INVALID_ARG;
  out[0] = c->cfg.pipeline_frames;
  out[1] = c->n_slots;
  out[2] = c->batch;
  out[3] = c->n_march;
  return KS_OK;
}

int ks_stream_plan(ks_ctx* c, int32_t out[8]) {
  if (!c || !out) return KS_ERR_INVALID_ARG;
  const StreamPlan& P = c->plan;
  out[0] = P.budget;
  out[1] = P.distinct;
  out[2] = P.n_march;
  out[3] = P.long_own ? 1 : 0;
  out[4] = !c->xlong ? -1 : P.xlong_own ? 1 : 0;
  out[5] = P.march_own ? 1 : 0;
  out[6] = P.tail_own ? 1 : 0;
  out[7] = c->n_streams;
  return KS_OK;
}

int ks_seed_launch_shape(int32_t order_mode, int32_t phase_growth, uint64_t cap_points, uint32_t* out, int32_t max_phases) {
  if (order_mode < KS_ORDER_MIXED || order_mode > KS_ORDER_MIXED_1024_GROUPS || phase_growth < 16 || phase_growth > 4096 || cap_points == 0 ||
      cap_points > kObsMaxPoints || (max_phases > 0 && !out))
    return KS_ERR_INVALID_ARG;
  const std::vector<SeedPhase> ph = seed_launch_shape(order_mode, phase_growth, std::max<size_t>((size_t)cap_points, 1024));
  for (size_t j = 0; j < ph.size() && (int64_t)j < (int64_t)max_phases; ++j) {
    out[3 * j] = ph[j].g0;
    out[3 * j + 1] = ph[j].g1;
    out[3 * j + 2] = ph[j].item_cap;
  }
  return (int)ph.size();
}

int ks_profile_enable(ks_ctx* c, int level) {
  if (!c || level < 0 || level > 2) return KS_ERR_INVALID_ARG;
  c->profiling = level;
  return KS_OK;
}

int ks_profile_get(ks_ctx* c, ks_profile* out, int reset) {
  if (!c || !out) return KS_ERR_INVALID_ARG;
  if (int rc = quiesce(c)) return rc;
  HIPCHK(c, hipStreamSynchronize(c->stream));
  for (int i = 0; i < kProfSets; ++i) resolve_prof(c, i);
  *out = c->prof;
  if (reset) c->prof = ks_profile{};
  return KS_OK;
}

}
```

kimera_semantics_amd/csrc/ks_k_apply.h:

```cpp
#pragma once
#include "ks_types.h"

namespace ksk {
struct VoxelRef {
  uint32_t slot, local;
  int vx, vy, vz;
};
__device__ __forceinline__ VoxelRef voxel_ref(const TileTable& T, uint32_t vox) {
  VoxelRef v;
  v.slot = vox >> 9;
  v.local = vox & 511u;
  int tx, ty, tz;
  unpack_tile(T.slot_keys[v.slot], tx, ty, tz);
  v.vx = tx * 8 + (int)(v.local & 7u);
  v.vy = ty * 8 + (int)((v.local >> 3) & 7u);
  v.vz = tz * 8 + (int)(v.local >> 6);
  return v;
}

__device__ __forceinline__ uint32_t perm_u(uint32_t x, uint32_t src_lane) {
  return (uint32_t)__builtin_amdgcn_ds_bpermute((int)(src_lane << 2), (int)x);
}
__device__ __forceinline__ float perm_f(float x, uint32_t src_lane) { return __uint_as_float(perm_u(__float_as_uint(x), src_lane)); }

struct UpdateOps {
  float sdf, uw, dm, dn;
  uint32_t info, color, rp;
};
template <bool HOT_ONLY>
__device__ __forceinline__ UpdateOps load_update_ops(const FrameParams& F, const RayDesc* __restrict__ rays, uint64_t key,
                                                     const VoxelRef& v) {
  UpdateOps u;
  u.rp = (uint32_t)key & F.point_mask;
  const uint4* r4 = (const uint4*)rays + (size_t)ray_index(F, u.rp) * 2;
  const uint4 d0 = r4[0];
  tsdf_operands(F.tsdf, F.T.t, {__uint_as_float(d0.x), __uint_as_float(d0.y), __uint_as_float(d0.z)}, v.vx, v.vy, v.vz,
                __uint_as_float(d0.w), u.sdf, u.uw);
  if (HOT_ONLY) {
    const uint32_t b = (uint32_t)(key >> 56);
    u.color = 0u;
    u.dm = F.log_match;
    u.dn = F.log_non_match;
    u.info = (b & 0x1fu) | (((b >> 5) & 3u) << 8) | (((b >> 7) & 1u) << 10);
  } else {
    const uint4 d1 = r4[1];
    u.color = d1.x;
    u.dm = __uint_as_float(d1.y);
    u.dn = __uint_as_float(d1.z);
    u.info = d1.w;
  }
  return u;
}

template <int COLOR_MODE, bool MERGED>
__global__ void __launch_bounds__(256) k_apply(FrameParams F, unsigned long long n_pairs,
                                               const uint64_t* __restrict__ pairs, const RayDesc* __restrict__ rays,
                                               const float* __restrict__ deltas, TileTable T, Pool P,
                                               const uint32_t* __restrict__ label_lut,
                                               unsigned long long* __restrict__ long_list, Counters* C) {
  __shared__ uint32_t s_lut[256];
  s_lut[threadIdx.x] = label_lut[threadIdx.x];
  const uint32_t lane = lane_id();
  const unsigned long long wbase = ((unsigned long long)blockIdx.x * 4ull + (threadIdx.x >> 6)) * 64ull;
  const unsigned long long i = wbase + lane;
  const bool valid = i < n_pairs;
  uint64_t key = 0;
  uint32_t vox = 0xffffffffu;
  bool head = false, is_long = false;
  UpdateOps u{};
  if (valid) {
    key = pairs[i];
    vox = (uint32_t)(key >> F.seq_bits);
    head = (i == 0) || ((uint32_t)(pairs[i - 1] >> F.seq_bits) != vox);
    if (head) is_long = (i + kLongRun < n_pairs) && ((uint32_t)(pairs[i + kLongRun] >> F.seq_bits) == vox);
    u = load_update_ops<!MERGED && COLOR_MODE != KS_COLOR_MODE_COLOR>(F, rays, key, voxel_ref(T, vox));
  }
  __syncthreads();

  const unsigned long long bounds = __ballot(head || !valid);
  const unsigned long long H = __ballot(head && !is_long);
  const uint32_t grp = lane >> 3, sub = lane & 7u;
  const uint32_t cbase = (sub - 1u) * 4u;
  const unsigned long long below = (1ull << lane) - 1ull;
  const uint32_t nh = (uint32_t)__popcll(H);
  const bool is_h = (H >> lane) & 1ull;
  const uint32_t dst = is_h ? (uint32_t)__popcll(H & below) : nh + (uint32_t)__popcll(~H & below);
  const uint32_t head_lane = (uint32_t)__builtin_amdgcn_ds_permute((int)(dst << 2), (int)lane);
  uint32_t it = 0;
  auto next_head = [&]() {
    const uint32_t r = 8u * it + grp;
    ++it;
    const uint32_t p = perm_u(head_lane, r & 63u);
    return r < nh ? (int)p : -1;
  };
  auto fetch = [&](int& pos, uint32_t& v, uint4& q) {
    pos = (8u * it < nh) ? next_head() : (++it, -1);
    v = perm_u(vox, pos >= 0 ? (uint32_t)pos : lane);
    q = (P.vox + (size_t)(pos >= 0 ? v : 0u) * 8)[sub];
  };
  const uint32_t n_it = (nh + 7u) >> 3;
  int nxt_pos, nxt2_pos;
  uint32_t nxt_vox, nxt2_vox;
  uint4 nxt_q, nxt2_q;
  fetch(nxt_pos, nxt_vox, nxt_q);
  fetch(nxt2_pos, nxt2_vox, nxt2_q);
  for (uint32_t cur = 0; cur < n_it; ++cur) {
    const int my_pos = nxt_pos;
    const bool active = my_pos >= 0;
    const uint32_t hp = active ? (uint32_t)my_pos : lane;
    const uint32_t hvox = nxt_vox;
    const uint4 q = nxt_q;
    nxt_pos = nxt2_pos;
    nxt_vox = nxt2_vox;
    nxt_q = nxt2_q;
    fetch(nxt2_pos, nxt2_vox, nxt2_q);
    uint32_t len = 0;
    if (active) {
      const unsigned long long above = (hp < 63u) ? (bounds >> (hp + 1u)) : 0ull;
      len = above ? (uint32_t)__ffsll((long long)above) : (64u - hp);
    }
    uint4* rec = P.vox + (size_t)(active ? hvox : 0u) * 8;
    float dist = __uint_as_float(q.x), weight = __uint_as_float(q.y);
    uint32_t color = q.z;
    float p0 = __uint_as_float(q.x), p1 = __uint_as_float(q.y), p2 = __uint_as_float(q.z), p3 = __uint_as_float(q.w);

    for (uint32_t s = 0;; ++s) {
      const bool on = active && s < len;
      if (__ballot(on) == 0ull) break;
      const uint32_t src = on ? hp + s : lane;
      const float sdf_s = perm_f(u.sdf, src), uw_s = perm_f(u.uw, src);
      constexpr bool per_ray_inc = MERGED;
      const float dm_s = per_ray_inc ? perm_f(u.dm, src) : F.log_match;
      const float dn_s = per_ray_inc ? perm_f(u.dn, src) : F.log_non_match;
      const uint32_t info_s = perm_u(u.info, src);
      uint32_t color_s = 0, rp_s = 0;
      if (COLOR_MODE == KS_COLOR_MODE_COLOR) color_s = perm_u(u.color, src);
      if (MERGED) rp_s = perm_u(u.rp, src);
      {
        const float nw = weight + uw_s;
        const bool upd = on && sub == 0u && !(nw < kEps);
        const float ns = (sdf_s * uw_s + dist * weight) / nw;
        const float nd = __builtin_amdgcn_fmed3f(ns, -F.tsdf.trunc, F.tsdf.trunc);
        if (COLOR_MODE == KS_COLOR_MODE_COLOR) {
          if (upd && fabsf(sdf_s) < F.tsdf.trunc) color = blend_two_colors(color, weight, color_s, uw_s);
        }
        dist = upd ? nd : dist;
        weight = upd ? std_min(F.tsdf.max_weight, nw) : weight;
      }
      const uint32_t kind = (info_s >> 8) & 3u;
      const bool sem_lane = on && (sub - 1u) < 6u;
      {
        const uint32_t lab = info_s & 0xffu;
        const bool pure = sem_lane && kind == 1u;
        const float a0 = p0 + ((cbase == lab) ? dm_s : dn_s);
        const float a1 = p1 + ((cbase + 1u == lab) ? dm_s : dn_s);
        const float a2 = p2 + ((cbase + 2u == lab) ? dm_s : dn_s);
        const float a3 = p3 + ((cbase + 3u == lab) ? dm_s : dn_s);
        p0 = pure ? a0 : p0;
        p1 = pure ? a1 : p1;
        p2 = pure ? a2 : p2;
        p3 = pure ? a3 : p3;
      }
      if (MERGED) {
        if (sem_lane && kind == 2u) {
          const float* dl = deltas + (size_t)rp_s * kNumLabels + cbase;
          p0 += dl[0];
          if (sub < 6u) { p1 += dl[1]; p2 += dl[2]; p3 += dl[3]; }
        }
      }
    }
    if (active && hp + len == 64u) {
      const VoxelRef v = voxel_ref(T, hvox);
      for (unsigned long long j = wbase + 64ull; j < n_pairs; ++j) {
        const uint64_t k = pairs[j];
        if ((uint32_t)(k >> F.seq_bits) != hvox) break;
        const UpdateOps t = load_update_ops<!MERGED && COLOR_MODE != KS_COLOR_MODE_COLOR>(F, rays, k, v);
        if (sub == 0u) {
          tsdf_combine<COLOR_MODE == KS_COLOR_MODE_COLOR>(F.tsdf, t.sdf, t.uw, t.color, dist, weight, color);
        } else if (sub < 7u) {
          const uint32_t kind = (t.info >> 8) & 3u;
          if (kind == 1u) {
            const uint32_t lab = t.info & 0xffu;
            p0 += (cbase == lab) ? t.dm : t.dn;
            p1 += (cbase + 1u == lab) ? t.dm : t.dn;
            p2 += (cbase + 2u == lab) ? t.dm : t.dn;
            p3 += (cbase + 3u == lab) ? t.dm : t.dn;
          } else if (kind == 2u) {
            const float* dl = deltas + (size_t)t.rp * kNumLabels + cbase;
            p0 += dl[0];
            if (sub < 6u) { p1 += dl[1]; p2 += dl[2]; p3 += dl[3]; }
          }
        }
      }
    }

    float bv = -INFINITY;
    uint32_t bi = 1000u;
    if (sub >= 1u && sub < 7u) {
      bv = p0; bi = cbase;
      if (sub < 6u) {
        if (p1 > bv) { bv = p1; bi = cbase + 1u; }
        if (p2 > bv) { bv = p2; bi = cbase + 2u; }
        if (p3 > bv) { bv = p3; bi = cbase + 3u; }
      }
    }
#pragma unroll
    for (int o = 1; o < 8; o <<= 1) {
      const float ov = perm_f(bv, lane ^ (uint32_t)o);
      const uint32_t oi = perm_u(bi, lane ^ (uint32_t)o);
      if (ov > bv || (ov == bv && oi < bi)) { bv = ov; bi = oi; }
    }
    if (COLOR_MODE == KS_COLOR_MODE_SEMANTIC) color = s_lut[bi & 255u];
    else if (COLOR_MODE == KS_COLOR_MODE_SEMANTIC_PROBABILITY) color = rainbow_color_map((double)(float)exp((double)bv));
    uint4 outv = make_uint4(0u, 0u, 0u, 0u);
    if (sub == 0u) outv = make_uint4(__float_as_uint(dist), __float_as_uint(weight), color, bi);
    else if (sub < 6u) outv = make_uint4(__float_as_uint(p0), __float_as_uint(p1), __float_as_uint(p2), __float_as_uint(p3));
    else if (sub == 6u) outv = make_uint4(__float_as_uint(p0), 1u, 0u, 0u);
    const bool wr = active && sub < 7u;
    rec[wr ? sub : 7u] = wr ? outv : make_uint4(0u, 0u, 0u, 0u);
  }
}

constexpr uint32_t kRunPer = 4;
constexpr uint32_t kRunThreads = 512;
constexpr uint32_t kRunTile = kRunPer * kRunThreads;
constexpr uint32_t kRunHalo = 32;

template <int COLOR_MODE, bool MERGED, uint32_t THREADS = kRunThreads>
__global__ void __launch_bounds__(THREADS) k_apply_runs(FrameParams F, unsigned long long n_pairs,
                                                            const uint64_t* __restrict__ pairs, const RayDesc* __restrict__ rays,
                                                            const float* __restrict__ deltas, TileTable T, Pool P,
                                                            const uint32_t* __restrict__ label_lut, uint32_t max_len) {
  constexpr bool HOT_ONLY = !MERGED && COLOR_MODE != KS_COLOR_MODE_COLOR;
  constexpr bool BLEND = COLOR_MODE == KS_COLOR_MODE_COLOR;
  constexpr uint32_t kTile = kRunPer * THREADS, kSlots = kTile + kRunHalo;
  constexpr uint32_t kMixSlots = kTile / 32;
  static_assert(kRunHalo == kLongRun, "a short run must end inside the halo");
  static_assert(kRunHalo <= 64 && THREADS % 64 == 0 && THREADS >= 256, "tile shape");
  __shared__ float s_sdf[kSlots], s_uw[kSlots];
  __shared__ uint16_t s_info[kSlots];
  __shared__ float s_dm[MERGED ? kSlots : 1], s_dn[MERGED ? kSlots : 1];
  __shared__ uint32_t s_col[BLEND ? kSlots : 1];
  __shared__ unsigned long long s_bounds[kSlots / 64 + 3 + THREADS / 64];
  __shared__ uint32_t s_run[kTile];
  __shared__ uint32_t s_run_vox[kTile];
  __shared__ uint32_t s_hist[kLongRun + 2];
  __shared__ uint32_t s_lut[256];
  __shared__ float s_mix[MERGED ? kMixSlots : 1][kNumLabels];
  __shared__ uint32_t s_n_mix, s_next_task;
  const uint32_t lane = lane_id(), tid = threadIdx.x;
  const unsigned long long base = (unsigned long long)blockIdx.x * kTile;
  if (tid < 256u) s_lut[tid] = label_lut[tid];
  if (tid < kLongRun + 2) s_hist[tid] = 0u;
  if (tid == 0) {
    s_n_mix = 0u;
    s_next_task = 0u;
  }
  if (tid < 2) s_bounds[kSlots / 64 + 1 + tid] = ~0ull;

  constexpr uint32_t NA = kRunPer + 1;
  uint64_t key[NA];
  bool valid[NA];
  {
    uint64_t pkey[NA];
#pragma unroll
    for (uint32_t k = 0; k < NA; ++k) {
      const uint32_t j = k * THREADS + tid;
      const unsigned long long i = base + j;
      valid[k] = j < kSlots && i < n_pairs;
      key[k] = valid[k] ? pairs[i] : 0ull;
      pkey[k] = (valid[k] && i > 0) ? pairs[i - 1] : ~0ull;
    }
    __syncthreads();
#pragma unroll
    for (uint32_t k = 0; k < NA; ++k) {
      const uint32_t j = k * THREADS + tid;
      const bool head = valid[k] && ((base + j == 0) || ((uint32_t)(pkey[k] >> F.seq_bits) != (uint32_t)(key[k] >> F.seq_bits)));
      const unsigned long long m = __ballot(head || !valid[k]);
      if (lane == 0) s_bounds[j >> 6] = m;
    }
  }
  __syncthreads();

  uint32_t my_len[kRunPer];
  bool need[NA];
#pragma unroll
  for (uint32_t k = 0; k < NA; ++k) {
    const uint32_t j = k * THREADS + tid;
    need[k] = false;
    if (k < kRunPer) my_len[k] = 0u;
    if (valid[k]) {
      const uint32_t q = j + 1u, sh = q & 63u;
      const unsigned long long lo = s_bounds[q >> 6], hi = s_bounds[(q >> 6) + 1u];
      const uint32_t fwd = (uint32_t)(sh ? ((lo >> sh) | (hi << (64u - sh))) : lo);
      uint32_t back;
      {
        const int p0 = (int)j - 31;
        const uint32_t w0 = (uint32_t)(p0 >= 0 ? p0 : 0) >> 6;
        const unsigned long long a0 = s_bounds[w0], a1 = s_bounds[w0 + 1u];
        if (p0 >= 0) {
          const uint32_t s0 = (uint32_t)p0 & 63u;
          back = (uint32_t)(s0 ? ((a0 >> s0) | (a1 << (64u - s0))) : a0);
        } else {
// ... 344 lines not shown
    p[0] = __uint_as_float(q1.x); p[1] = __uint_as_float(q1.y); p[2] = __uint_as_float(q1.z); p[3] = __uint_as_float(q1.w);
    p[4] = __uint_as_float(q2.x); p[5] = __uint_as_float(q2.y); p[6] = __uint_as_float(q2.z); p[7] = __uint_as_float(q2.w);
    p[8] = __uint_as_float(q3.x); p[9] = __uint_as_float(q3.y); p[10] = __uint_as_float(q3.z); p[11] = __uint_as_float(q3.w);
    p[12] = __uint_as_float(q4.x); p[13] = __uint_as_float(q4.y); p[14] = __uint_as_float(q4.z); p[15] = __uint_as_float(q4.w);
    p[16] = __uint_as_float(q5.x); p[17] = __uint_as_float(q5.y); p[18] = __uint_as_float(q5.z); p[19] = __uint_as_float(q5.w);
    p[20] = __uint_as_float(q6);
    const VoxelRef v = voxel_ref(T, vox);
    const float vs = F.tsdf.voxel_size;
    v_voxel_origin = sub3({((float)v.vx + 0.5f) * vs, ((float)v.vy + 0.5f) * vs, ((float)v.vz + 0.5f) * vs}, F.T.t);
  } else {
#pragma unroll
    for (int l = 0; l < kNumLabels; ++l) p[l] = 0.f;
  }
  const TsdfParams& Pm = F.tsdf;
  for (uint32_t g = 0; __ballot(g < len) != 0ull; g += D) {
#pragma unroll
    for (uint32_t j = 0; j < D; ++j) {
      const uint32_t s = g + j;
      const bool on = s < len;
      const RayDesc d = dq[j];
      const uint32_t rp = (uint32_t)kq[j] & F.point_mask;
      dq[j] = rays[(s + D < len) ? ray_index(F, (uint32_t)kq[j + D] & F.point_mask) : 0u];
      if (on) {
        const f3 v_point_origin = sub3({d.px, d.py, d.pz}, F.T.t);
        const float dist_G = norm3(v_point_origin);
        const float dist_G_V = dot3(v_voxel_origin, v_point_origin) / dist_G;
        const float sdf = dist_G - dist_G_V;
        float uw = d.weight;
        if (Pm.use_dropoff && sdf < -Pm.voxel_size) {
          uw = d.weight * (Pm.trunc + sdf) / Pm.dropoff_denominator;
          uw = std_max(uw, 0.0f);
        }
        if (Pm.use_sparsity) {
          if (fabsf(sdf) < Pm.trunc) uw *= Pm.sparsity_factor;
        }
        const float nw = weight + uw;
        if (!(nw < kEps)) {
          const float ns = (sdf * uw + dist * weight) / nw;
          if (BLEND) {
            if (fabsf(sdf) < Pm.trunc) color = blend_two_colors(color, weight, d.color, uw);
          }
          dist = __builtin_amdgcn_fmed3f(ns, -Pm.trunc, Pm.trunc);
          weight = std_min(Pm.max_weight, nw);
        }
        const uint32_t kind = (d.info >> 8) & 3u, lab = d.info & 0xffu;
        if (kind == 1u) {
          const float dm = d.d_match, dn = d.d_non;
#pragma unroll
          for (int l = 0; l < kNumLabels; ++l) p[l] += ((uint32_t)l == lab) ? dm : dn;
        } else if (kind == 2u) {
          const float* dl = deltas + (size_t)rp * kNumLabels;
#pragma unroll
          for (int l = 0; l < kNumLabels; ++l) p[l] += dl[l];
        }
      }
    }
#pragma unroll
    for (uint32_t j = 0; j < D; ++j) {
      kq[j] = kq[j + D];
      kq[j + D] = (g + 2 * D + j < len) ? pairs[start + g + 2 * D + j] : 0ull;
    }
  }
  if (has) {
    float bv = p[0];
    uint32_t bi = 0u;
#pragma unroll
    for (int l = 1; l < kNumLabels; ++l)
      if (p[l] > bv) {
        bv = p[l];
        bi = (uint32_t)l;
      }
    if (COLOR_MODE == KS_COLOR_MODE_SEMANTIC) color = s_lut[bi & 255u];
    else if (COLOR_MODE == KS_COLOR_MODE_SEMANTIC_PROBABILITY) color = rainbow_color_map((double)(float)exp((double)bv));
    rec[0] = make_uint4(__float_as_uint(dist), __float_as_uint(weight), color, bi);
    rec[1] = make_uint4(__float_as_uint(p[0]), __float_as_uint(p[1]), __float_as_uint(p[2]), __float_as_uint(p[3]));
    rec[2] = make_uint4(__float_as_uint(p[4]), __float_as_uint(p[5]), __float_as_uint(p[6]), __float_as_uint(p[7]));
    rec[3] = make_uint4(__float_as_uint(p[8]), __float_as_uint(p[9]), __float_as_uint(p[10]), __float_as_uint(p[11]));
    rec[4] = make_uint4(__float_as_uint(p[12]), __float_as_uint(p[13]), __float_as_uint(p[14]), __float_as_uint(p[15]));
    rec[5] = make_uint4(__float_as_uint(p[16]), __float_as_uint(p[17]), __float_as_uint(p[18]), __float_as_uint(p[19]));
    rec[6] = make_uint4(__float_as_uint(p[20]), 1u, 0u, 0u);
  }
}

template <int COLOR_MODE>
__global__ void __launch_bounds__(128) k_apply_long(FrameParams F, unsigned long long n_pairs,
                                                   const uint64_t* __restrict__ pairs, const RayDesc* __restrict__ rays,
                                                   const float* __restrict__ deltas, TileTable T, Pool P,
                                                   const uint32_t* __restrict__ label_lut,
                                                   const unsigned long long* __restrict__ long_list, const Counters* C,
                                                   const LongHdr* __restrict__ H = nullptr) {
  __shared__ float s_inc[2][64][kNumLabels];
  __shared__ int s_cnt[2];
  __shared__ uint32_t s_best;
  __shared__ float s_best_val;
  constexpr int PF = 4;
  uint32_t n_long = C->n_long, list_base = 0u;
  if (H) {
    n_long = 0u;
    for (int c = 0; c < kLongClasses; ++c) {
      if (c < kLongLaneClasses) list_base += H->count[c];
      else n_long += H->count[c];
    }
  }
  const int lane = (int)lane_id();
  const bool consumer = (threadIdx.x >> 6) != 0u;
  const int cls = lane < kNumLabels ? lane : 0;
  const TsdfParams& Pm = F.tsdf;
  for (uint32_t run = blockIdx.x; run < n_long; run += gridDim.x) {
    const unsigned long long start = long_list[list_base + run] & 0xffffffffffffull;
    const uint32_t vox = (uint32_t)(pairs[start] >> F.seq_bits);
    const VoxelRef v = voxel_ref(T, vox);
    uint32_t* rec = (uint32_t*)(P.vox + (size_t)vox * 8);
    float dist = __uint_as_float(rec[0]), weight = __uint_as_float(rec[1]);
    uint32_t color = rec[2];
    if (consumer) {
      float pri = (lane < kNumLabels) ? __uint_as_float(rec[4 + lane]) : 0.0f;
      for (int buf = 0;; buf ^= 1) {
        __syncthreads();
        const int cnt = s_cnt[buf];
        if (cnt == 0) break;
        if (cnt == 64) {
          float x[64];
#pragma unroll
          for (int k = 0; k < 64; ++k) x[k] = s_inc[buf][k][cls];
#pragma unroll
          for (int k = 0; k < 64; ++k) pri += x[k];
        } else {
#pragma unroll 8
          for (int k = 0; k < cnt; ++k) pri += s_inc[buf][k][cls];
        }
        if (cnt < 64) break;
      }
      int best = 0;
      float m = bcast_f(pri, 0);
#pragma unroll
      for (int l = 1; l < kNumLabels; ++l) {
        const float x = bcast_f(pri, l);
        if (x > m) { m = x; best = l; }
      }
      if (lane < kNumLabels) rec[4 + lane] = __float_as_uint(pri);
      if (lane == 0) {
        s_best = (uint32_t)best;
        s_best_val = m;
      }
      __syncthreads();
      __syncthreads();
      continue;
    }
    int buf = 0;
    const f3 c = {((float)v.vx + 0.5f) * Pm.voxel_size, ((float)v.vy + 0.5f) * Pm.voxel_size,
                  ((float)v.vz + 0.5f) * Pm.voxel_size};
    const f3 v_voxel_origin = sub3(c, F.T.t);

    const unsigned long long last = n_pairs - 1ull;
    unsigned long long base = start;
    uint64_t key_q[PF], key_n[PF];
    RayDesc d_q[PF];
#pragma unroll
    for (int i = 0; i < PF; ++i) {
      key_q[i] = pairs[min(base + 64ull * i + lane, last)];
      key_n[i] = pairs[min(base + 64ull * (PF + i) + lane, last)];
    }
#pragma unroll
    for (int i = 0; i < PF; ++i) d_q[i] = rays[ray_index(F, (uint32_t)key_q[i] & F.point_mask)];

    auto batch = [&](const uint64_t key_cur, const RayDesc& d) -> bool {
      const bool in = (base + lane < n_pairs) && ((uint32_t)(key_cur >> F.seq_bits) == vox);
      const int cnt = (int)__popcll(__ballot(in));
      if (cnt == 0) {
        if (lane == 0) s_cnt[buf] = 0;
        __syncthreads();
        return false;
      }
      float sdf = 0.f, uw = 0.f;
      if (in) {
        const f3 v_point_origin = sub3({d.px, d.py, d.pz}, F.T.t);
        const float dist_G = norm3(v_point_origin);
        const float dist_G_V = dot3(v_voxel_origin, v_point_origin) / dist_G;
        sdf = dist_G - dist_G_V;
        uw = d.weight;
        if (Pm.use_dropoff && sdf < -Pm.voxel_size) {
          uw = d.weight * (Pm.trunc + sdf) / Pm.dropoff_denominator;
          uw = std_max(uw, 0.0f);
        }
        if (Pm.use_sparsity) {
          if (fabsf(sdf) < Pm.trunc) uw *= Pm.sparsity_factor;
        }
        const uint32_t kind = (d.info >> 8) & 3u;
        const uint32_t lab = d.info & 0xffu;
        if (kind == 2u) {
          const float* dl = deltas + (size_t)((uint32_t)key_cur & F.point_mask) * kNumLabels;
#pragma unroll
          for (int l = 0; l < kNumLabels; ++l) s_inc[buf][lane][l] = dl[l];
        } else {
          const float a = (kind == 1u) ? d.d_match : 0.0f, b = (kind == 1u) ? d.d_non : 0.0f;
#pragma unroll
          for (int l = 0; l < kNumLabels; ++l) s_inc[buf][lane][l] = ((uint32_t)l == lab) ? a : b;
        }
      }
      __builtin_amdgcn_wave_barrier();

      float my_w = 0.0f, my_nw = 1.0f;
      if (weight == Pm.max_weight && __ballot(in && !(uw >= 0.0f)) == 0ull) {
        my_w = weight;
        my_nw = weight + uw;
      } else {
        float w_run = weight;
        for (int k = 0; k < cnt; ++k) {
          const float nw = w_run + bcast_f(uw, k);
          if (lane == k) { my_w = w_run; my_nw = nw; }
          if (!(nw < kEps)) w_run = std_min(Pm.max_weight, nw);
        }
        weight = w_run;
      }
      const bool my_skip = my_nw < kEps;
      const float my_r = 1.0f / my_nw;
      const float my_p = sdf * uw;
      const bool my_sat = my_skip || ((sdf - Pm.trunc) * uw >= 1e-6f * Pm.trunc * my_nw);
      const bool all_sat = (__ballot(in && !my_sat) == 0ull);
      if (!(all_sat && dist == Pm.trunc && COLOR_MODE != KS_COLOR_MODE_COLOR)) {
        for (int k = 0; k < cnt; ++k) {
          if (bcast_u(my_skip ? 1u : 0u, k)) continue;
          const float w_k = bcast_f(my_w, k), nw_k = bcast_f(my_nw, k), r_k = bcast_f(my_r, k);
          const float num = bcast_f(my_p, k) + dist * w_k;
          const float q = div_by_recip(num, nw_k, r_k);
          if (COLOR_MODE == KS_COLOR_MODE_COLOR) {
            if (fabsf(bcast_f(sdf, k)) < Pm.trunc)
              color = blend_two_colors(color, w_k, bcast_u(d.color, k), bcast_f(uw, k));
          }
          dist = (q > 0.0f) ? std_min(Pm.trunc, q) : std_max(-Pm.trunc, q);
        }
      }
      if (lane == 0) s_cnt[buf] = cnt;
      __syncthreads();
      buf ^= 1;
      return cnt == 64;
    };
    for (bool more = true; more;) {
#pragma unroll
      for (int j = 0; j < PF; ++j) {
        const uint64_t key_cur = key_q[j];
        const RayDesc d = d_q[j];
        key_q[j] = key_n[j];
        d_q[j] = rays[ray_index(F, (uint32_t)key_n[j] & F.point_mask)];
        key_n[j] = pairs[min(base + 64ull * (2 * PF) + lane, last)];
        more = batch(key_cur, d);
        if (!more) break;
        base += 64;
      }
    }
    __syncthreads();
    const uint32_t best = s_best;
    const float m = s_best_val;
    if (COLOR_MODE == KS_COLOR_MODE_SEMANTIC) color = label_lut[best];
    else if (COLOR_MODE == KS_COLOR_MODE_SEMANTIC_PROBABILITY)
      color = rainbow_color_map((double)(float)exp((double)m));
    if (lane == 0) {
      *(uint4*)rec = make_uint4(__float_as_uint(dist), __float_as_uint(weight), color, best);
      rec[25] = 1u;
    }
    __syncthreads();
  }
}

template <int COLOR_MODE>
__global__ void __launch_bounds__(256) k_apply_xlong(FrameParams F, unsigned long long n_pairs,
                                                    const uint64_t* __restrict__ pairs, const RayDesc* __restrict__ rays,
                                                    const float* __restrict__ deltas, TileTable T, Pool P,
                                                    const uint32_t* __restrict__ label_lut,
                                                    const unsigned long long* __restrict__ xlong_list, const uint32_t* __restrict__ n_runs_ptr) {
  __shared__ float s_inc[2][16][kNumLabels][4];
  __shared__ float4 s_tab[3][64];
  __shared__ int s_cnt[3];
  __shared__ uint32_t s_best;
  __shared__ float s_best_val;
  const uint32_t n_x = *n_runs_ptr;
  const int lane = (int)lane_id();
  const int role = (int)(threadIdx.x >> 6);
  const int cls = lane < kNumLabels ? lane : 0;
  const TsdfParams& Pm = F.tsdf;
  for (uint32_t run = blockIdx.x; run < n_x; run += gridDim.x) {
    const unsigned long long start = xlong_list[run];
    const uint32_t vox = (uint32_t)(pairs[start] >> F.seq_bits);
    uint32_t* rec = (uint32_t*)(P.vox + (size_t)vox * 8);
    if (role >= 2) {
      const int f = role - 2;
      const VoxelRef v = voxel_ref(T, vox);
      const f3 c = {((float)v.vx + 0.5f) * Pm.voxel_size, ((float)v.vy + 0.5f) * Pm.voxel_size,
                    ((float)v.vz + 0.5f) * Pm.voxel_size};
      const f3 v_voxel_origin = sub3(c, F.T.t);
      const unsigned long long last = n_pairs - 1ull;
      auto key_of = [&](unsigned long long own) { return pairs[min(start + 64ull * ((unsigned long long)f + 2ull * own) + lane, last)]; };
      uint64_t key_q[2] = {key_of(0), key_of(1)}, key_n[2] = {key_of(2), key_of(3)};
      RayDesc d_q[2] = {rays[ray_index(F, (uint32_t)key_q[0] & F.point_mask)], rays[ray_index(F, (uint32_t)key_q[1] & F.point_mask)]};
      unsigned long long own = 0;
      bool h_in = false;
      uint32_t h_kind = 0, h_lab = 0, h_rp = 0;
      float h_a = 0.f, h_b = 0.f;
      auto first_half = [&]() {
        const unsigned long long b = (unsigned long long)f + 2ull * own;
        const uint64_t key_cur = key_q[0];
        const RayDesc d = d_q[0];
        const RayDesc d_new = rays[ray_index(F, (uint32_t)key_n[0] & F.point_mask)];
        const uint64_t key_new = key_of(own + 4ull);
        const bool in = (start + 64ull * b + lane < n_pairs) && ((uint32_t)(key_cur >> F.seq_bits) == vox);
        const int cnt = (int)__popcll(__ballot(in));
        float sdf = 0.f, uw = 0.f;
        if (in) {
          const f3 v_point_origin = sub3({d.px, d.py, d.pz}, F.T.t);
          const float dist_G = norm3(v_point_origin);
          const float dist_G_V = dot3(v_voxel_origin, v_point_origin) / dist_G;
          sdf = dist_G - dist_G_V;
          uw = d.weight;
          if (Pm.use_dropoff && sdf < -Pm.voxel_size) {
            uw = d.weight * (Pm.trunc + sdf) / Pm.dropoff_denominator;
            uw = std_max(uw, 0.0f);
          }
          if (Pm.use_sparsity) {
            if (fabsf(sdf) < Pm.trunc) uw *= Pm.sparsity_factor;
          }
        }
        s_tab[b % 3ull][lane] = make_float4(sdf, uw, __uint_as_float(d.color), 0.0f);
        if (lane == 0) s_cnt[b % 3ull] = cnt;
        h_in = in;
        h_kind = (d.info >> 8) & 3u;
        h_lab = d.info & 0xffu;
        h_rp = (uint32_t)key_cur & F.point_mask;
        h_a = (h_kind == 1u) ? d.d_match : 0.0f;
        h_b = (h_kind == 1u) ? d.d_non : 0.0f;
        key_q[0] = key_q[1];
        d_q[0] = d_q[1];
        key_q[1] = key_n[0];
        d_q[1] = d_new;
        key_n[0] = key_n[1];
        key_n[1] = key_new;
      };
      auto second_half = [&]() {
        const unsigned long long b = (unsigned long long)f + 2ull * own;
        float* inc = &s_inc[b & 1ull][lane >> 2][0][lane & 3];
        if (h_in) {
          if (h_kind == 2u) {
            const float* dl = deltas + (size_t)h_rp * kNumLabels;
#pragma unroll
            for (int l = 0; l < kNumLabels; ++l) inc[4 * l] = dl[l];
          } else {
            float a = h_a, b = h_b;
            KS_VALUE_BARRIER(a);
            KS_VALUE_BARRIER(b);
#pragma unroll
            for (int l = 0; l < kNumLabels; ++l) inc[4 * l] = ((uint32_t)l == h_lab) ? a : b;
          }
        }
        ++own;
      };
      if (f == 0) first_half();
      for (unsigned long long s = 0;; ++s) {
        if ((int)(s & 1ull) == f) second_half();
        else first_half();
        const int cnt_prev = s >= 1ull ? s_cnt[(s - 1ull) % 3ull] : 64;
        __syncthreads();
        if (cnt_prev < 64) break;
      }
      __syncthreads();
      __syncthreads();
      continue;
    }
    if (role == 1) {
      float pri = (lane < kNumLabels) ? __uint_as_float(rec[4 + lane]) : 0.0f;
      __syncthreads();
      for (unsigned long long s = 1;; ++s) {
        const unsigned long long b = s - 1ull;
        const int cnt = s_cnt[b % 3ull];
        if (cnt == 64) {
          float4 x[16];
#pragma unroll
          for (int g = 0; g < 16; ++g) x[g] = *(const float4*)&s_inc[b & 1ull][g][cls][0];
#pragma unroll
          for (int g = 0; g < 16; ++g) {
            pri += x[g].x;
            pri += x[g].y;
            pri += x[g].z;
            pri += x[g].w;
          }
        } else {
#pragma unroll 4
          for (int k = 0; k < cnt; ++k) pri += s_inc[b & 1ull][k >> 2][cls][k & 3];
        }
        __syncthreads();
        if (cnt < 64) break;
      }
      int best = 0;
      float m = bcast_f(pri, 0);
#pragma unroll
      for (int l = 1; l < kNumLabels; ++l) {
        const float x = bcast_f(pri, l);
        if (x > m) { m = x; best = l; }
      }
      if (lane < kNumLabels) rec[4 + lane] = __float_as_uint(pri);
      if (lane == 0) {
        s_best = (uint32_t)best;
        s_best_val = m;
      }
      __syncthreads();
      __syncthreads();
      continue;
    }
    float dist = __uint_as_float(rec[0]), weight = __uint_as_float(rec[1]);
    uint32_t color = rec[2];
    __syncthreads();
    for (unsigned long long s = 1;; ++s) {
      const unsigned long long b = s - 1ull;
      const int cnt = s_cnt[b % 3ull];
      const float4 t = s_tab[b % 3ull][lane];
      const bool in = lane < cnt;
      const float sdf = t.x, uw = t.y;
      const uint32_t d_color = __float_as_uint(t.z);
      if (cnt > 0) {
        float my_w = 0.0f, my_nw = 1.0f;
        if (weight == Pm.max_weight && __ballot(in && !(uw >= 0.0f)) == 0ull) {
          my_w = weight;
          my_nw = weight + uw;
        } else {
          float w_run = weight;
          for (int k = 0; k < cnt; ++k) {
            const float nw = w_run + bcast_f(uw, k);
            if (lane == k) { my_w = w_run; my_nw = nw; }
            if (!(nw < kEps)) w_run = std_min(Pm.max_weight, nw);
          }
          weight = w_run;
        }
        const bool my_skip = my_nw < kEps;
        const float my_r = 1.0f / my_nw;
        const float my_p = sdf * uw;
        const bool my_sat = my_skip || ((sdf - Pm.trunc) * uw >= 1e-6f * Pm.trunc * my_nw);
        const bool all_sat = (__ballot(in && !my_sat) == 0ull);
        if (!(all_sat && dist == Pm.trunc && COLOR_MODE != KS_COLOR_MODE_COLOR)) {
          for (int k = 0; k < cnt; ++k) {
            if (bcast_u(my_skip ? 1u : 0u, k)) continue;
            const float w_k = bcast_f(my_w, k), nw_k = bcast_f(my_nw, k), r_k = bcast_f(my_r, k);
            const float num = bcast_f(my_p, k) + dist * w_k;
            const float q = div_by_recip(num, nw_k, r_k);
            if (COLOR_MODE == KS_COLOR_MODE_COLOR) {
              if (fabsf(bcast_f(sdf, k)) < Pm.trunc)
                color = blend_two_colors(color, w_k, bcast_u(d_color, k), bcast_f(uw, k));
            }
            dist = (q > 0.0f) ? std_min(Pm.trunc, q) : std_max(-Pm.trunc, q);
          }
        }
      }
      __syncthreads();
      if (cnt < 64) break;
    }
    __syncthreads();
    const uint32_t best = s_best;
    const float m = s_best_val;
    if (COLOR_MODE == KS_COLOR_MODE_SEMANTIC) color = label_lut[best];
    else if (COLOR_MODE == KS_COLOR_MODE_SEMANTIC_PROBABILITY)
      color = rainbow_color_map((double)(float)exp((double)m));
    if (lane == 0) {
      *(uint4*)rec = make_uint4(__float_as_uint(dist), __float_as_uint(weight), color, best);
      rec[25] = 1u;
    }
    __syncthreads();
  }
}

}
```

kimera_semantics_amd/csrc/ks_k_march.h:

```cpp
#pragma once
#include "ks_types.h"

namespace ksk {

constexpr uint64_t kObsPoison = 0x00000000ffffffffull;
constexpr uint64_t kObsRetired = 0x00000000fffffffeull;
constexpr uint32_t kObsMaxTag = 1023;
constexpr uint32_t kObsMaxPoints = (1u << 22) - 2;

__device__ __forceinline__ uint64_t obs_entry(uint32_t tag, uint32_t pos, uint32_t hash) {
  return ((uint64_t)tag << 54) | ((uint64_t)(pos + 1u) << 32) | (uint64_t)hash;
}
__device__ __forceinline__ bool obs_match(uint64_t e, uint32_t h, uint32_t tag_lo, uint32_t tag) {
  const uint32_t posf = (uint32_t)(e >> 32) & 0x3fffffu, t = (uint32_t)(e >> 54);
  return posf != 0u && t >= tag_lo && t <= tag && (uint32_t)e == h;
}

__global__ void __launch_bounds__(256) k_obs_retag(uint64_t* __restrict__ set) {
  const uint32_t i = blockIdx.x * blockDim.x + threadIdx.x;
  if (i < (2u << kSetBits)) {
    const uint64_t e = set[i];
    if (e != 0ull) set[i] = kObsRetired;
  }
}
// ... 500 lines not shown
#pragma unroll
  for (int o = 1; o < 64; o <<= 1) {
    const uint32_t y = __shfl_up(x, o);
    if (lane >= (uint32_t)o) x += y;
  }
  if (lane == 63) s_wave[wave] = x;
  __syncthreads();
  uint32_t wbase = 0;
  for (uint32_t w = 0; w < wave; ++w) wbase += s_wave[w];
  uint32_t run = wbase + x - mine;
#pragma unroll
  for (int k = 0; k < 4; ++k) {
    if (i0 + k < n_scan) lp[i0 + k] = run;
    run += v[k];
  }
  if (threadIdx.x == 1023) bt[blockIdx.x] = (unsigned long long)(wbase + x);
}

#define KS_SLOT_ARGS(V)                                       \
  const SlotView& sv = (V).s[blockIdx.y];                     \
  const uint32_t* __restrict__ ray_list = sv.ray_list;        \
  const RayDesc* __restrict__ rays = sv.rays;                 \
  const uint32_t* __restrict__ cnt = sv.cnt;                  \
  const uint32_t* __restrict__ lp = sv.lp;                    \
  const unsigned long long* __restrict__ bt = sv.bt;          \
  uint64_t* __restrict__ pairs = sv.pairs;                    \
  const unsigned long long pairs_cap = sv.pairs_cap;          \
  Counters* C = sv.C;                                         \
  const FrameParams F = *sv.F;

template <int LPR>
__global__ void __launch_bounds__(256) k_emit(BatchView V, TileTable T, Pool P) {
  KS_SLOT_ARGS(V)
  if (blockIdx.x != 0 && blockIdx.x * (256u / LPR) >= C->n_rays) return;
  extern __shared__ unsigned long long s_bt[];
  __shared__ unsigned long long s_carry;
  const uint32_t nb = (scan_length(F) + kScanBlock - 1) / kScanBlock;
  if (threadIdx.x == 0) s_carry = 0ull;
  __syncthreads();
  for (uint32_t b0 = 0; b0 < nb; b0 += 256) {
    const uint32_t b = b0 + threadIdx.x;
    const unsigned long long v = b < nb ? bt[b] : 0ull;
    __shared__ unsigned long long s_w[4];
    unsigned long long x = v;
#pragma unroll
    for (int o = 1; o < 64; o <<= 1) {
      const unsigned long long y = __shfl_up(x, o);
      if (lane_id() >= (uint32_t)o) x += y;
    }
    if (lane_id() == 63) s_w[threadIdx.x >> 6] = x;
    __syncthreads();
    unsigned long long wb = s_carry;
    for (uint32_t w = 0; w < (threadIdx.x >> 6); ++w) wb += s_w[w];
    if (b < nb) s_bt[b] = wb + x - v;
    __syncthreads();
    if (threadIdx.x == 255) s_carry = wb + x;
    __syncthreads();
  }
  const unsigned long long total = s_carry;
  if (blockIdx.x == 0 && threadIdx.x == 0) C->n_pairs = total;
  if (total > pairs_cap) {
    if (blockIdx.x == 0 && threadIdx.x == 0) atomicOr(&C->err, kErrPairs);
    return;
  }
  if (C->err & (kErrLabel | kErrIndex | kErrExact)) return;
  const LaneGroup<LPR> G;
  const uint32_t n_rays = C->n_rays;
  const uint32_t r = (blockIdx.x * 256u + threadIdx.x) / LPR;
  const bool have = r < n_rays;
  uint32_t p = 0, count = 0;
  unsigned long long base = 0;
  uint64_t key_lo = 0;
  bool clearing = false;
  uint64_t own_key = 0;
  Dda round{};
  if (have) {
    p = ray_list[r];
    const RayDesc d = rays[ray_index(F, p)];
    clearing = ((d.info >> 10) & 1u) != 0;
    const uint32_t si = p + ((F.method == KS_METHOD_MERGED && clearing) ? F.n : 0u);
    count = cnt[si] & ~kCntBroke;
    base = s_bt[si / kScanBlock] + lp[si];
    key_lo = ((uint64_t)((d.info & 0x1fu) | (((d.info >> 8) & 3u) << 5) | (((d.info >> 10) & 1u) << 7)) << 56) |
             (uint64_t)((F.method == KS_METHOD_MERGED && clearing) ? (p | F.clear_bit) : p);
    own_key = F.ray_keys ? F.ray_keys[p] : 0ull;
    round.setup(F.T.t, {d.px, d.py, d.pz}, clearing, F.carving != 0, F.max_ray, F.voxel_size_inv, F.trunc,
                F.method == KS_METHOD_MERGED);
  }
  const uint32_t walk = have ? (F.grazing_keys ? (uint32_t)round.steps + 1u : count) : 0u;
  uint32_t emitted = 0;
  uint64_t last_tile = kEmpty64;
  uint32_t slot = 0;
  for (uint32_t s0 = 0; __ballot(s0 < walk) != 0ull; s0 += LPR) {
    const bool in = s0 < walk;
    const Dda mine = dda_at_lane<LPR>(round, G.l);
    const bool step_on = in && (s0 + G.l < walk);
    const bool emit = step_on && !grazing_skip(F, mine.cx, mine.cy, mine.cz, clearing, own_key);
    uint32_t hpos = 0, got = 0;
    bool need_tile = false;
    if (emit) {
      const uint64_t tk = pack_tile(mine.cx >> 3, mine.cy >> 3, mine.cz >> 3);
      if (tk != last_tile) {
        need_tile = true;
        last_tile = tk;
        got = tile_slot_nowait(T, C, tk, &hpos);
      }
    }
    if (need_tile) {
      uint32_t spins = 0;
      while (got == kSlotPending) {
        got = __hip_atomic_load(&T.ent[hpos].val, __ATOMIC_RELAXED, __HIP_MEMORY_SCOPE_AGENT);
        if (++spins > (1u << 22)) {
          atomicOr(&C->err, kErrTable);
          got = kSlotBad;
        }
      }
      slot = got;
      if (slot < T.max_tiles) { P.updated[slot] = 1; P.dirty[slot] = 1; P.mesh_stale()[slot] = kStaleAll; }
      else atomicOr(&C->err, kErrPool);
    }
    const uint64_t em = G.bits(__ballot(emit));
    if (emit) {
      const uint32_t local = (uint32_t)(mine.cx & 7) + 8u * ((uint32_t)(mine.cy & 7) + 8u * (uint32_t)(mine.cz & 7));
      const uint32_t k = emitted + (uint32_t)__popcll(em & ((1ull << G.l) - 1ull));
      pairs[base + k] = ((uint64_t)(slot * (uint32_t)kTileVoxels + local) << F.seq_bits) | key_lo;
    }
    emitted += (uint32_t)__popcll(em);
    if (in && s0 + LPR < walk) dda_next_round<LPR>(G, round, mine);
  }
}

template <int RPW>
__global__ void __launch_bounds__(256) k_emit_lane(BatchView V, TileTable T, Pool P) {
  KS_SLOT_ARGS(V)
  if (blockIdx.x != 0 && blockIdx.x * 4u * (uint32_t)RPW >= C->n_rays) return;
  extern __shared__ unsigned long long s_bt[];
  __shared__ unsigned long long s_carry;
  __shared__ float s_e[4][3 * kES];
  const uint32_t nb = (scan_length(F) + kScanBlock - 1) / kScanBlock;
  if (threadIdx.x == 0) s_carry = 0ull;
  __syncthreads();
  for (uint32_t b0 = 0; b0 < nb; b0 += 256) {
    const uint32_t b = b0 + threadIdx.x;
    const unsigned long long v = b < nb ? bt[b] : 0ull;
    __shared__ unsigned long long s_w[4];
    unsigned long long x = v;
#pragma unroll
    for (int o = 1; o < 64; o <<= 1) {
      const unsigned long long y = __shfl_up(x, o);
      if (lane_id() >= (uint32_t)o) x += y;
    }
    if (lane_id() == 63) s_w[threadIdx.x >> 6] = x;
    __syncthreads();
    unsigned long long wb = s_carry;
    for (uint32_t w = 0; w < (threadIdx.x >> 6); ++w) wb += s_w[w];
    if (b < nb) s_bt[b] = wb + x - v;
    __syncthreads();
    if (threadIdx.x == 255) s_carry = wb + x;
    __syncthreads();
  }
  const unsigned long long total = s_carry;
  if (blockIdx.x == 0 && threadIdx.x == 0) C->n_pairs = total;
  if (total > pairs_cap) {
    if (blockIdx.x == 0 && threadIdx.x == 0) atomicOr(&C->err, kErrPairs);
    return;
  }
  if (C->err & (kErrLabel | kErrIndex | kErrExact)) return;
  const uint32_t lane = lane_id();
  const uint32_t n_rays = C->n_rays;
  const uint32_t r = (blockIdx.x * 4u + (threadIdx.x >> 6)) * (uint32_t)RPW + lane;
  uint32_t count = 0;
  unsigned long long base = 0;
  uint64_t key_lo = 0;
  Dda dda{};
  if (lane < (uint32_t)RPW && r < n_rays) {
    const uint32_t p = ray_list[r];
    const RayDesc d = rays[ray_index(F, p)];
    const bool clearing = ((d.info >> 10) & 1u) != 0;
    const uint32_t si = p + ((F.method == KS_METHOD_MERGED && clearing) ? F.n : 0u);
    count = cnt[si] & ~kCntBroke;
    base = s_bt[si / kScanBlock] + lp[si];
    key_lo = ((uint64_t)((d.info & 0x1fu) | (((d.info >> 8) & 3u) << 5) | (((d.info >> 10) & 1u) << 7)) << 56) |
             (uint64_t)((F.method == KS_METHOD_MERGED && clearing) ? (p | F.clear_bit) : p);
    dda.setup(F.T.t, {d.px, d.py, d.pz}, clearing, F.carving != 0, F.max_ray, F.voxel_size_inv, F.trunc,
              F.method == KS_METHOD_MERGED);
  }
  auto wait_slot = [&](uint32_t got, uint32_t hpos) -> uint32_t {
    uint32_t spins = 0;
    while (got == kSlotPending) {
      got = __hip_atomic_load(&T.ent[hpos].val, __ATOMIC_RELAXED, __HIP_MEMORY_SCOPE_AGENT);
      if (++spins > (1u << 22)) {
        atomicOr(&C->err, kErrTable);
        got = kSlotBad;
      }
    }
    if (got < T.max_tiles) { P.updated[got] = 1; P.dirty[got] = 1; P.mesh_stale()[got] = kStaleAll; }
    else atomicOr(&C->err, kErrPool);
    return got;
  };
  const unsigned long long long_mask = __ballot(count > kLaneWalk);
  const bool by_wave = tails_by_wavefront(long_mask, count);
  const uint32_t own = (by_wave && count > kLaneWalk) ? kLaneWalk : count;
  uint64_t last_tile = kEmpty64;
  uint32_t slot = 0;
  for (uint32_t s = 0; __ballot(s < own) != 0ull; ++s) {
    const bool on = s < own;
    uint32_t hpos = 0, got = 0;
    bool need_tile = false;
    if (on) {
      const uint64_t tk = pack_tile(dda.cx >> 3, dda.cy >> 3, dda.cz >> 3);
      if (tk != last_tile) {
        need_tile = true;
        last_tile = tk;
        got = tile_slot_nowait(T, C, tk, &hpos);
      }
    }
    if (need_tile) slot = wait_slot(got, hpos);
    if (on) {
      const uint32_t local = (uint32_t)(dda.cx & 7) + 8u * ((uint32_t)(dda.cy & 7) + 8u * (uint32_t)(dda.cz & 7));
      const uint64_t key = ((uint64_t)(slot * (uint32_t)kTileVoxels + local) << F.seq_bits) | key_lo;
      pairs[base + s] = key;
    }
    dda.advance(on);
  }
  float* escr = s_e[threadIdx.x >> 6];
  for (unsigned long long todo = by_wave ? long_mask : 0ull; todo != 0ull; todo &= todo - 1ull) {
    const int j = __ffsll((long long)todo) - 1;
    Dda ust = dda_bcast(dda, j);
    const uint32_t c_j = __shfl(count, j);
    const unsigned long long base_j = __shfl(base, j);
    const uint64_t key_j = __shfl(key_lo, j);
    if (dda_parallel_ok(ust)) {
      for (uint32_t s0 = kLaneWalk; s0 < c_j; s0 += 64) {
        dda_round64(ust, escr, lane, [&](uint32_t rr, int vx, int vy, int vz) {
          if (s0 + rr < c_j) {
            uint32_t hpos = 0;
            const uint32_t got = tile_slot_nowait(T, C, pack_tile(vx >> 3, vy >> 3, vz >> 3), &hpos);
            const uint32_t sl = wait_slot(got, hpos);
            const uint32_t local = (uint32_t)(vx & 7) + 8u * ((uint32_t)(vy & 7) + 8u * (uint32_t)(vz & 7));
            pairs[base_j + s0 + rr] = ((uint64_t)(sl * (uint32_t)kTileVoxels + local) << F.seq_bits) | key_j;
          }
        });
      }
    } else if ((int)lane == j) {
      for (uint32_t s = kLaneWalk; s < count; ++s) {
        uint32_t hpos = 0;
        const uint32_t got = tile_slot_nowait(T, C, pack_tile(dda.cx >> 3, dda.cy >> 3, dda.cz >> 3), &hpos);
        const uint32_t sl = wait_slot(got, hpos);
        const uint32_t local = (uint32_t)(dda.cx & 7) + 8u * ((uint32_t)(dda.cy & 7) + 8u * (uint32_t)(dda.cz & 7));
        pairs[base + s] = ((uint64_t)(sl * (uint32_t)kTileVoxels + local) << F.seq_bits) | key_lo;
        dda.advance();
      }
    }
  }
}

template <int LPR>
__global__ void __launch_bounds__(256) k_count_grazing(BatchView V) {
  const SlotView& sv = V.s[blockIdx.y];
  const uint32_t* __restrict__ ray_list = sv.ray_list;
  const RayDesc* __restrict__ rays = sv.rays;
  uint32_t* __restrict__ cnt = sv.cnt;
  const Counters* C = sv.C;
  const FrameParams F = *sv.F;
  const LaneGroup<LPR> G;
  const uint32_t r = (blockIdx.x * 256u + threadIdx.x) / LPR;
// ... 66 lines not shown
```

kimera_semantics_amd/csrc/ks_types.h:

```cpp
#pragma once
#include <hip/hip_runtime.h>
#include <stdint.h>

#include "../../include/ks_hip.h"
#include "ks_device_math.h"

namespace ksk {
using namespace ksd;

constexpr uint64_t kEmpty64 = ~0ull;
constexpr uint32_t kEmpty32 = ~0u;
constexpr int kSetBits = 20;
constexpr uint64_t kSetMask = (1ull << kSetBits) - 1;
constexpr uint64_t kFullResetThreshold = 10000;
constexpr float kPriorInit = -0.60205999132f;
constexpr int kCoordBias = 1 << 20;
constexpr int kTileBias = 1 << 17;

constexpr __host__ __device__ __forceinline__ uint64_t pack_tile(int tx, int ty, int tz) {
  return ((uint64_t)(uint32_t)(tx + kTileBias) << 36) | ((uint64_t)(uint32_t)(ty + kTileBias) << 18) |
         (uint64_t)(uint32_t)(tz + kTileBias);
}
constexpr __host__ __device__ __forceinline__ void unpack_tile(uint64_t k, int& tx, int& ty, int& tz) {
  tx = (int)((k >> 36) & 0x3ffffu) - kTileBias;
// ... 63 lines not shown
#define KS_WAIT_LOADS() __builtin_amdgcn_s_waitcnt(0x0F70)
#endif
#ifndef KS_VALUE_BARRIER
#define KS_VALUE_BARRIER(x) asm volatile("" : "+v"(x))
#endif

__device__ __forceinline__ uint32_t wave_append(bool pred, uint32_t* counter) {
  const unsigned long long m = __ballot(pred);
  const uint32_t lane = lane_id();
  uint32_t base = 0;
  if (lane == 0 && m) base = atomicAdd(counter, (uint32_t)__popcll(m));
  base = __shfl(base, 0);
  return base + (uint32_t)__popcll(m & ((1ull << lane) - 1ull));
}
__device__ __forceinline__ uint32_t block_append(bool pred, uint32_t* counter) {
  __shared__ uint32_t s_wave[16];
  __shared__ uint32_t s_base;
  const unsigned long long m = __ballot(pred);
  const uint32_t lane = lane_id(), wave = threadIdx.x >> 6, nwaves = blockDim.x >> 6;
  if (lane == 0) s_wave[wave] = (uint32_t)__popcll(m);
  __syncthreads();
  if (threadIdx.x == 0) {
    uint32_t total = 0;
    for (uint32_t w = 0; w < nwaves; ++w) {
      const uint32_t t = s_wave[w];
      s_wave[w] = total;
      total += t;
    }
    s_base = total ? atomicAdd(counter, total) : 0u;
  }
  __syncthreads();
  const uint32_t pos = s_base + s_wave[wave] + (uint32_t)__popcll(m & ((1ull << lane) - 1ull));
  __syncthreads();
  return pos;
}
__device__ __forceinline__ void block_count(bool pred, uint32_t* counter) {
  __shared__ uint32_t s_cnt;
  if (threadIdx.x == 0) s_cnt = 0;
  __syncthreads();
  const unsigned long long m = __ballot(pred);
  if (lane_id() == 0 && m) atomicAdd(&s_cnt, (uint32_t)__popcll(m));
  __syncthreads();
  if (threadIdx.x == 0 && s_cnt) atomicAdd(counter, s_cnt);
}

struct RayDesc {
  float px, py, pz;
  float weight;
  uint32_t color;
  float d_match, d_non;
  uint32_t info;
};

struct TileEntry {
  uint64_t key;
  uint32_t val;
  uint32_t pad;
};

struct TileTable {
  TileEntry* ent;
  uint64_t* slot_keys;
  uint32_t* n_tiles;
  uint32_t mask;
  uint32_t max_tiles;
};

constexpr size_t kFlagPlane = 1u << 23;
struct Pool {
  uint4* vox;
  uint8_t* updated;
  uint8_t* dirty;
  __host__ __device__ __forceinline__ uint8_t* mesh_stale() const { return updated + kFlagPlane; }
};
constexpr uint8_t kStaleMesh = 1, kStaleEsdf = 2, kStaleAll = kStaleMesh | kStaleEsdf;

struct FrameParams {
  Pose T;
  float voxel_size_inv;
  float min_ray, max_ray, trunc;
  float start_inv;
  float log_match, log_non_match;
  TsdfParams tsdf;
  uint64_t start_offset, observed_offset;
  uint32_t obs_tag, obs_tag_lo;
  uint64_t* observed;
  int32_t max_collisions;
  uint32_t n;
  uint32_t order_groups, order_per;
  uint32_t chains;
  int carving, allow_clear, freespace, use_const_weight;
  int method, color_mode, early_out, sorted_order;
  int n_dynamic;
  const uint64_t* grazing_keys;
  const uint64_t* ray_keys;
  const uint32_t* order;
  const uint32_t* inv_order;
  uint32_t seq_bits;
  uint32_t point_mask;
  uint32_t clear_bit;
  uint32_t eo_frame;
  int32_t key_base[3];
  uint32_t key_bits;
  uint8_t dynamic_labels[32];
};

__device__ __forceinline__ uint32_t point_order(const FrameParams& F, const uint32_t* order, uint32_t p) {
  if (F.sorted_order) return order[p];
  if (F.order_groups * F.order_per <= p) return p;
  return (p % F.order_groups) * F.order_per + p / F.order_groups;
}

__device__ __forceinline__ bool grazing_skip(const FrameParams& F, int cx, int cy, int cz, bool clearing, uint64_t own_key) {
  if (!F.grazing_keys) return false;
  const int lim = kCoordBias - 1;
  if (abs(cx) >= lim || abs(cy) >= lim || abs(cz) >= lim) return false;
  const uint64_t k = pack_coord3(cx, cy, cz);
  if (!clearing && k == own_key) return false;
  uint32_t lo = 0, hi = F.n;
  while (lo < hi) {
    const uint32_t mid = (lo + hi) >> 1;
    if (F.grazing_keys[mid] < k) lo = mid + 1;
    else hi = mid;
  }
  return lo < F.n && F.grazing_keys[lo] == k;
}

__device__ __forceinline__ uint32_t ray_index(const FrameParams& F, uint32_t p) {
  return (F.method == KS_METHOD_FAST) ? point_order(F, F.order, p) : p;
}

__device__ __forceinline__ uint32_t point_position(const FrameParams& F, const uint32_t* inv_order, uint32_t idx) {
  if (F.sorted_order) return inv_order[idx];
  if (F.order_groups * F.order_per <= idx) return idx;
  return (idx % F.order_per) * F.order_groups + idx / F.order_per;
}

__host__ __device__ __forceinline__ uint32_t mix64(uint64_t k) {
  k ^= k >> 33;
  k *= 0xff51afd7ed558ccdull;
  k ^= k >> 33;
  k *= 0xc4ceb9fe1a85ec53ull;
  k ^= k >> 33;
  return (uint32_t)k;
}

constexpr uint32_t kSlotPending = 0xffffffffu;
constexpr uint32_t kSlotBad = 0xfffffffeu;

__device__ __forceinline__ void tile_insert(const TileTable& T, Counters* C, uint64_t key) {
  uint32_t h = mix64(key) & T.mask;
  for (uint32_t probes = 0; probes <= T.mask; ++probes) {
    const uint64_t k = __hip_atomic_load(&T.ent[h].key, __ATOMIC_RELAXED, __HIP_MEMORY_SCOPE_AGENT);
    if (k == key) return;
    if (k == kEmpty64) {
      const uint64_t old = atomicCAS((unsigned long long*)&T.ent[h].key, (unsigned long long)kEmpty64, (unsigned long long)key);
      if (old == kEmpty64) {
        uint32_t slot = atomicAdd(T.n_tiles, 1u);
        if (slot < T.max_tiles) {
          T.slot_keys[slot] = key;
        } else {
          atomicOr(&C->err, kErrPool);
          slot = kSlotBad;
        }
        __hip_atomic_store(&T.ent[h].val, slot, __ATOMIC_RELAXED, __HIP_MEMORY_SCOPE_AGENT);
        return;
      }
      if (old == key) return;
    }
    h = (h + 1) & T.mask;
  }
  atomicOr(&C->err, kErrTable);
}

__device__ __forceinline__ uint32_t tile_slot_nowait(const TileTable& T, Counters* C, uint64_t key, uint32_t* hpos) {
  uint32_t h = mix64(key) & T.mask;
  for (uint32_t probes = 0; probes <= T.mask; ++probes) {
    const uint4 e = *(const uint4*)&T.ent[h];
    uint64_t k = (uint64_t)e.x | ((uint64_t)e.y << 32);
    if (k == key && e.z != kSlotPending) {
      *hpos = h;
      return e.z;
    }
    if (k != key) k = __hip_atomic_load(&T.ent[h].key, __ATOMIC_RELAXED, __HIP_MEMORY_SCOPE_AGENT);
    if (k == kEmpty64) {
      const uint64_t old = atomicCAS((unsigned long long*)&T.ent[h].key, (unsigned long long)kEmpty64, (unsigned long long)key);
      if (old == kEmpty64) {
        uint32_t slot = atomicAdd(T.n_tiles, 1u);
        if (slot < T.max_tiles) {
          T.slot_keys[slot] = key;
        } else {
          atomicOr(&C->err, kErrPool);
          slot = kSlotBad;
        }
        __hip_atomic_store(&T.ent[h].val, slot, __ATOMIC_RELAXED, __HIP_MEMORY_SCOPE_AGENT);
        return slot;
      }
      k = old;
    }
    if (k == key) {
      *hpos = h;
      return __hip_atomic_load(&T.ent[h].val, __ATOMIC_RELAXED, __HIP_MEMORY_SCOPE_AGENT);
    }
    h = (h + 1) & T.mask;
  }
  atomicOr(&C->err, kErrTable);
  return kSlotBad;
}

__device__ __forceinline__ uint32_t tile_lookup(const TileTable& T, uint64_t key) {
  uint32_t h = mix64(key) & T.mask;
  for (uint32_t probes = 0; probes <= T.mask; ++probes) {
// ... 32 lines not shown
```

Baseline: 1014 Mvoxel-updates/s.

## Batch tail sort and apply across frames in a launch batch

Frame indices are encoded into the pair keys so that the pair lists of all frames in a batch can be concatenated, sorted once and applied by batch variants of the apply kernels. A per-frame table supplies the ray arrays and origins. The goal is to cut per-frame sort and launch overhead and the host-side tail work when each frame has few pairs. In exchange it adds a concat copy, wider sort keys, host synchronisation on the last slot of the batch, and extra eligibility rules that fall back to per-frame tails.

```diff
diff --git a/include/ks_hip.h b/include/ks_hip.h
--- a/include/ks_hip.h
+++ b/include/ks_hip.h
@@ -280,6 +280,8 @@
 int ks_update_stats(ks_ctx* ctx, uint64_t out[4]);
 int ks_pipeline_shape(ks_ctx* ctx, int32_t out[4]);
 int ks_stream_plan(ks_ctx* ctx, int32_t out[8]);
+int ks_tail_batch_stats(ks_ctx* ctx, uint64_t out[4]);
+int ks_tail_batch_rule(const uint32_t* err, const uint64_t* n_pairs, int32_t nb, int32_t marcher, int32_t profiling, uint64_t apply_runs_min_pairs);
 int ks_seed_launch_shape(int32_t integration_order_mode, int32_t early_out_phase_growth, uint64_t cap_points, uint32_t* out, int32_t max_phases);
 
 #ifdef __cplusplus
diff --git a/kimera_semantics_amd/binding.py b/kimera_semantics_amd/binding.py
--- a/kimera_semantics_amd/binding.py
+++ b/kimera_semantics_amd/binding.py
@@ -30,7 +30,7 @@
     "ks_integrate_points", "ks_integrate_points_device", "ks_integrate_depth", "ks_integrate_depth_device", "ks_num_blocks", "ks_get_block_indices",
     "ks_get_updated_block_indices", "ks_count_updated_voxels", "ks_download_updated_voxels", "ks_download_blocks", "ks_upload_blocks", "ks_host_alloc", "ks_host_free", "ks_get_tile_keys", "ks_export_tiles_device", "ks_merge_tiles_device", "ks_clear", "ks_clear_voxels", "ks_reset_tiles", "ks_tile_owner", "ks_reduce",
     "ks_debug_radix_sort", "ks_debug_radix_sort_range", "ks_debug_radix_sort_batch", "ks_synchronize", "ks_flush", "ks_stream",
-    "ks_profile_enable", "ks_profile_get", "ks_early_out_iterations", "ks_early_out_stats", "ks_pipeline_shape", "ks_stream_plan", "ks_seed_launch_shape", "ks_update_stats", "ks_integrate_round_exact",
+    "ks_profile_enable", "ks_profile_get", "ks_early_out_iterations", "ks_early_out_stats", "ks_pipeline_shape", "ks_stream_plan", "ks_tail_batch_stats", "ks_tail_batch_rule", "ks_seed_launch_shape", "ks_update_stats", "ks_integrate_round_exact",
     "ks_mesh_default_config", "ks_mesh_update", "ks_mesh_size", "ks_mesh_download", "ks_mesh_changed_blocks",
     "ks_esdf_default_config", "ks_esdf_update", "ks_esdf_download_blocks", "ks_esdf_query",
     "ks_esdf_refresh", "ks_esdf_changed_blocks",
@@ -241,6 +241,8 @@
         L.ks_early_out_stats.argtypes = [vp, C.POINTER(C.c_uint64)]
         L.ks_pipeline_shape.argtypes = [vp, C.POINTER(C.c_int32)]
         L.ks_stream_plan.argtypes = [vp, C.POINTER(C.c_int32)]
+        L.ks_tail_batch_stats.argtypes = [vp, C.POINTER(C.c_uint64)]
+        L.ks_tail_batch_rule.argtypes = [C.POINTER(C.c_uint32), C.POINTER(C.c_uint64), C.c_int32, C.c_int32, C.c_int32, C.c_uint64]
         L.ks_seed_launch_shape.argtypes = [C.c_int32, C.c_int32, C.c_uint64, C.POINTER(C.c_uint32), C.c_int32]
         L.ks_update_stats.argtypes = [vp, C.POINTER(C.c_uint64)]
         L.ks_integrate_round_exact.argtypes = [vp, vp, vp, C.c_int, C.c_int, C.c_uint64, vp, vp, vp, vp, C.c_size_t, C.c_int, C.POINTER(KsRoundStats)]
@@ -764,6 +766,11 @@
         return dict(budget=int(out[0]), streams=int(out[1]), march_streams=int(out[2]), long=side[int(out[3])], xlong=side[int(out[4])],
                     march="own" if out[5] else "A", tail="own" if out[6] else "A", streams_held=int(out[7]))
 
+    def tail_batch_stats(self):
+        out = (C.c_uint64 * 4)()
+        self._chk(lib().ks_tail_batch_stats(self._h, out))
+        return dict(batches=int(out[0]), frames=int(out[1]), per_frame_batches=int(out[2]), pairs=int(out[3]))
+
     def early_out_iterations(self):
         f, it = C.c_uint64(), C.c_uint64()
         self._chk(lib().ks_early_out_iterations(self._h, C.byref(f), C.byref(it)))
diff --git a/kimera_semantics_amd/csrc/ks_hip.hip b/kimera_semantics_amd/csrc/ks_hip.hip
--- a/kimera_semantics_amd/csrc/ks_hip.hip
+++ b/kimera_semantics_amd/csrc/ks_hip.hip
@@ -124,6 +124,10 @@
   bool tail_recorded = false;
   bool join_recorded = false;
   bool b_launched = false;
+  int batch_index = 0, batch_nb = 1;
+  FrameSlot* batch_slots[kBatchMax] = {};
+  bool tail_batched = false;
+  uint32_t tb_blocks = 0;
   size_t steps_max = 0;
   uint64_t frame_no = 0;
   FrameParams F{};
@@ -141,6 +145,7 @@
   Event k0, k1;
   bool used = false, complete = false, stages = false, apply = false, applied = false;
   uint64_t n_pairs = 0, n_points = 0;
+  uint64_t n_applied = 0;
 };
 
 struct StreamPlanIn {
@@ -270,6 +275,12 @@
   DevBuf<uint32_t> d_okeys, d_okeys2, d_ovals;
   size_t cap_pairs = 0;
   DevBuf<uint64_t> d_pairs2_[2];
+  DevBuf<uint64_t> d_pairs_cat_[2];
+  DevBuf<TailFrame> d_tail_frames_[2];
+  size_t cap_cat = 0;
+  int last_par = -1;
+  bool tail_batch_on = true;
+  uint64_t tb_stats[4] = {0, 0, 0, 0};
   hipEvent_t pending_join = nullptr;
   ksrs::Workspace sort_ws, sort_ws_tail;
   bool exact_early_out = false;
@@ -716,6 +727,11 @@
   return b;
 }
 
+inline unsigned tail_frame_bits(const ks_ctx* c) {
+  if (c->batch <= 1 || c->cfg.method != KS_METHOD_FAST || c->shard_export) return 0u;
+  const unsigned fb = bits_for((uint64_t)c->batch);
+  return bits_for(c->cap_points) + fb + 9u + 23u <= 56u ? fb : 0u;
+}
 int launch_batch(ks_ctx* c);
 int quiesce(ks_ctx* c);
 int reset_set(ks_ctx* c, uint64_t* d_set0, uint64_t* offset, bool observed) {
@@ -774,7 +790,7 @@
     if (hipEventElapsedTime(&kms, P.k0, P.k1) == hipSuccess) {
       c->prof.apply_kernel_ms += kms;
       c->prof.apply_kernel_launches += 1;
-      c->prof.apply_kernel_updates += P.n_pairs;
+      c->prof.apply_kernel_updates += P.n_applied;
     }
   }
   c->prof.frames += 1;
@@ -1181,6 +1197,11 @@
     FrameSlot& S = *slots[k];
     S.F.observed = observed_table(c, S.frame_no);
     if (c->exact_early_out) S.F.eo_frame = c->eo_frame_no++;
+    if (S.F.frame_bits) S.F.frame_bits = (S.F.frame_bits & 0xffu) | (k << 8);
+    S.batch_index = (int)k;
+    S.batch_nb = (int)nb;
+    for (uint32_t j = 0; j < (uint32_t)kBatchMax; ++j) S.batch_slots[j] = j < nb ? slots[j] : nullptr;
+    S.tail_batched = false;
     PB.F[k] = S.F;
     PB.out[k] = S.d_F;
     V.s[k] = slot_view(S);
@@ -1242,6 +1263,10 @@
   F.point_mask = (1u << pb) - 1u;
   F.clear_bit = (cfg.method == KS_METHOD_MERGED) ? (1u << pb) : 0u;
   F.seq_bits = pb + (cfg.method == KS_METHOD_MERGED ? 1u : 0u);
+  if (const unsigned fb = tail_frame_bits(c)) {
+    F.frame_bits = bits_for(c->cap_points);
+    F.seq_bits = F.frame_bits + fb;
+  }
   F.inv_order = F.sorted_order ? c->d_inv_order : nullptr;
   std::memcpy(F.dynamic_labels, cfg.dynamic_labels, 32);
   F.early_out = c->uses_early_out;
@@ -1592,6 +1617,29 @@
     long_runs<MODE>();
   }
 };
+struct BatchUpdateLaunch {
+  ks_ctx* c;
+  const FrameParams& F;
+  hipStream_t st, sl, sx;
+  int set;
+  uint64_t* sp;
+  unsigned long long n_pairs, *d_long_list, *d_xlong_list;
+  const TailFrame* tab;
+  Counters* C;
+  template <int MODE> void launch() const {
+    const uint32_t ab = (uint32_t)((n_pairs + 255) / 256);
+    KS_LAUNCH_TIMED_IF(set >= 0, c->pset[set].k0, c->pset[set].k1, (k_apply_batch<MODE>), dim3(ab), dim3(256), st, F, n_pairs, (const uint64_t*)sp, tab,
+                       c->table, c->pool, (const uint32_t*)c->d_label_lut.get());
+    if (sx) {
+      const uint32_t xb = (uint32_t)std::min<unsigned long long>(n_pairs / kXLongRun + 1, 512);
+      hipLaunchKernelGGL(k_apply_xlong_batch<MODE>, dim3(xb), dim3(256), 0, sx, F, n_pairs, (const uint64_t*)sp, tab, c->table, c->pool,
+                         (const uint32_t*)c->d_label_lut.get(), (const unsigned long long*)d_xlong_list, (const uint32_t*)&C->n_xlong);
+    }
+    const uint32_t lb = (uint32_t)std::min<unsigned long long>(n_pairs / kLongRun + 1, 4096);
+    hipLaunchKernelGGL(k_apply_long_batch<MODE>, dim3(lb), dim3(128), 0, sl, F, n_pairs, (const uint64_t*)sp, tab, c->table, c->pool,
+                       (const uint32_t*)c->d_label_lut.get(), (const unsigned long long*)d_long_list, (const Counters*)C);
+  }
+};
 #undef KS_LAUNCH_TIMED_IF
 int enqueue_update(ks_ctx* c, FrameSlot& S, hipStream_t st, unsigned long long n_pairs, uint32_t new_tiles, int set) {
   if (n_pairs == 0) {
@@ -1607,12 +1655,20 @@
   const unsigned end_bit = F.seq_bits + 9 + bits_for(new_tiles);
   uint64_t* sp = nullptr;
   const int par = (int)(S.frame_no & 1u);
+  if (par == c->last_par && c->pending_join) {
+    HIPCHK(c, hipStreamWaitEvent(st, c->pending_join, 0));
+    c->pending_join = nullptr;
+  }
+  c->last_par = par;
   unsigned long long* const d_long_list = c->d_long_list_[par];
   if ((rc = sort_keys(c, S.d_pairs.get(), c->d_pairs2_[par].get(), n_pairs, std::min(56u, end_bit), &sp, F.seq_bits, true))) return rc;
   stage_mark(c, set, 8);
   const bool by_runs = n_pairs >= c->apply_runs_min_pairs;
   const bool time_apply = set >= 0 && c->pset[set].apply;
-  if (time_apply) c->pset[set].applied = true;
+  if (time_apply) {
+    c->pset[set].applied = true;
+    c->pset[set].n_applied = n_pairs;
+  }
   hipStream_t sl = c->stream_long, sx = c->stream_xlong;
   const bool long_beside = sl != st, xlong_beside = sx && sx != st;
   unsigned long long* const d_xlong_list = sx ? d_long_list + (c->cap_pairs / kLongRunLanes + 64) : nullptr;
@@ -1654,6 +1710,137 @@
   return KS_OK;
 }
 
+bool tail_batch_rule(const uint32_t* err, const unsigned long long* n_pairs, int nb, bool marcher, int profiling, unsigned long long runs_min_pairs,
+                     unsigned long long xl_min_pairs) {
+  if (nb < 2 || nb > kBatchMax || marcher || profiling == 1) return false;
+  unsigned long long total = 0;
+  for (int k = 0; k < nb; ++k) {
+    if (err[k] || n_pairs[k] >= runs_min_pairs || n_pairs[k] >= xl_min_pairs) return false;
+    total += n_pairs[k];
+  }
+  return total > 0;
+}
+int ensure_tail_batch(ks_ctx* c, size_t n) {
+  int rc;
+  for (int b = 0; b < 2; ++b)
+    if (!c->d_tail_frames_[b] && (rc = c->d_tail_frames_[b].alloc(c, kBatchMax))) return rc;
+  if (n <= c->cap_cat) return KS_OK;
+  const size_t cap = std::max<size_t>(n + n / 4, 1 << 20);
+  c->cap_cat = 0;
+  HIPCHK(c, hipStreamSynchronize(c->stream_long));
+  if (c->stream_xlong) HIPCHK(c, hipStreamSynchronize(c->stream_xlong));
+  if (c->stream_tail) HIPCHK(c, hipStreamSynchronize(c->stream_tail));
+  for (int b = 0; b < 2; ++b)
+    if ((rc = c->d_pairs_cat_[b].alloc(c, cap))) return rc;
+  c->cap_cat = cap;
+  return KS_OK;
+}
+int tail_batch(ks_ctx* c, FrameSlot& S0) {
+  const int nb = S0.batch_nb;
+  FrameSlot* const* slots = S0.batch_slots;
+  if (nb < 2 || !S0.F.frame_bits) return KS_OK;
+  int rc;
+  if (!c->tail_batch_on) {
+    c->tb_stats[2] += 1;
+    return KS_OK;
+  }
+  hipStream_t st = c->stream_tail;
+  HIPCHK(c, hipEventSynchronize(slots[nb - 1]->ready));
+  uint32_t err[kBatchMax];
+  unsigned long long np[kBatchMax], total = 0;
+  bool same_keys = true;
+  for (int k = 0; k < nb; ++k) {
+    err[k] = slots[k]->counters().err;
+    np[k] = slots[k]->counters().n_pairs;
+    total += np[k];
+    same_keys = same_keys && (k == 0 || slots[k]->pending) && slots[k]->F.seq_bits == S0.F.seq_bits && (slots[k]->F.frame_bits & 0xffu) == (S0.F.frame_bits & 0xffu);
+  }
+  if (!same_keys || !tail_batch_rule(err, np, nb, c->shard_export, c->profiling, c->apply_runs_min_pairs,
+                                     c->stream_xlong && c->xl_parallel ? c->xl_min_pairs : ~0ull)) {
+    c->tb_stats[2] += 1;
+    return KS_OK;
+  }
+  uint32_t tiles = c->tiles_initialised;
+  for (int k = 0; k < nb; ++k) {
+    const uint32_t nt = std::min(slots[k]->n_tiles(), c->cfg.max_tiles);
+    slots[k]->tb_blocks = nt > tiles ? nt - tiles : 0u;
+    tiles = std::max(tiles, nt);
+  }
+  if (tiles > c->tiles_initialised) {
+    hipLaunchKernelGGL(k_init_tiles, dim3(tiles - c->tiles_initialised), dim3(512), 0, st, c->pool, c->tiles_initialised);
+    c->tiles_initialised = tiles;
+  }
+  if ((rc = ensure_pairs_out(c, total)) || (rc = ensure_tail_batch(c, total))) return rc;
+  const int par = c->last_par == 0 ? 1 : 0;
+  c->last_par = par;
+  const FrameParams& F = S0.F;
+  TailFrames TF{};
+  PairLists L{};
+  unsigned long long longest = 0;
+  for (int k = 0; k < kBatchMax; ++k) {
+    const FrameSlot& S = *slots[std::min(k, nb - 1)];
+    TF.f[k].rays = S.d_rays;
+    TF.f[k].t = S.F.T.t;
+    TF.f[k].point_mask = S.F.point_mask;
+    TF.f[k].order_groups = S.F.order_groups;
+    TF.f[k].order_per = S.F.order_per;
+    L.src[k] = S.d_pairs;
+    L.off[k + 1] = L.off[k] + (k < nb ? np[k] : 0ull);
+    longest = std::max(longest, k < nb ? np[k] : 0ull);
+  }
+  TailFrame* const tab = c->d_tail_frames_[par];
+  hipLaunchKernelGGL(k_set_tail_frames, dim3(kBatchMax), dim3(64), 0, st, TF, tab);
+  hipLaunchKernelGGL(k_cat_pairs, dim3((uint32_t)std::min<unsigned long long>((longest + 1023) / 1024, 2048), (uint32_t)nb), dim3(256), 0, st, L,
+                     c->d_pairs_cat_[par].get());
+  const unsigned end_bit = F.seq_bits + 9 + bits_for(tiles);
+  uint64_t* sp = nullptr;
+  if ((rc = sort_keys(c, c->d_pairs_cat_[par].get(), c->d_pairs2_[par].get(), total, std::min(56u, end_bit), &sp, F.seq_bits, true))) return rc;
+  hipStream_t sl = c->stream_long, sx = c->stream_xlong;
+  const bool long_beside = sl != st, xlong_beside = sx && sx != st;
+  unsigned long long* const d_long_list = c->d_long_list_[par];
+  unsigned long long* const d_xlong_list = sx ? d_long_list + (c->cap_pairs / kLongRunLanes + 64) : nullptr;
+  const dim3 find_grid((uint32_t)((total + 256 * kFindLongItems - 1) / (256 * kFindLongItems)));
+  hipLaunchKernelGGL(k_find_long, find_grid, dim3(256), 0, st, F.seq_bits, total, (const uint64_t*)sp, d_long_list, d_xlong_list, S0.d_counters, kLongRun);
+  if (c->pending_join) HIPCHK(c, hipStreamWaitEvent(st, c->pending_join, 0));
+  c->pending_join = nullptr;
+  if (long_beside || xlong_beside) HIPCHK(c, hipEventRecord(S0.fork, st));
+  if (long_beside) HIPCHK(c, hipStreamWaitEvent(sl, S0.fork, 0));
+  if (xlong_beside) HIPCHK(c, hipStreamWaitEvent(sx, S0.fork, 0));
+  int timed = -1;
+  for (int k = 0; k < nb && timed < 0; ++k)
+    if (slots[k]->prof_set >= 0 && c->pset[slots[k]->prof_set].apply) timed = slots[k]->prof_set;
+  if (timed >= 0) {
+    c->pset[timed].applied = true;
+    c->pset[timed].n_applied = total;
+  }
+  const BatchUpdateLaunch U{c, F, st, sl, sx, timed, sp, total, d_long_list, d_xlong_list, tab, S0.d_counters};
+  switch (c->cfg.color_mode) {
+    case KS_COLOR_MODE_COLOR: U.launch<KS_COLOR_MODE_COLOR>(); break;
+    case KS_COLOR_MODE_SEMANTIC: U.launch<KS_COLOR_MODE_SEMANTIC>(); break;
+    default: U.launch<KS_COLOR_MODE_SEMANTIC_PROBABILITY>(); break;
+  }
+  if (xlong_beside) {
+    HIPCHK(c, hipEventRecord(S0.join_x, sx));
+    HIPCHK(c, hipStreamWaitEvent(sl, S0.join_x, 0));
+  }
+  for (int k = 0; k < nb; ++k) {
+    FrameSlot& S = *slots[k];
+    if (long_beside) {
+      HIPCHK(c, hipEventRecord(S.join, sl));
+      S.join_recorded = true;
+    }
+    HIPCHK(c, hipEventRecord(S.tail_done, st));
+    S.tail_recorded = true;
+    S.tail_batched = true;
+  }
+  if (long_beside) c->pending_join = S0.join;
+  HIPCHK(c, hipGetLastError());
+  c->tb_stats[0] += 1;
+  c->tb_stats[1] += (uint64_t)nb;
+  c->tb_stats[3] += total;
+  return KS_OK;
+}
+
 int frame_tail(ks_ctx* c, FrameSlot& S) {
   if (!S.pending) return KS_OK;
   S.pending = false;
@@ -1663,6 +1850,7 @@
   hipStream_t st = c->stream_tail;
   const auto w0 = std::chrono::steady_clock::now();
   HIPCHK(c, hipEventSynchronize(S.ready));
+  if (S.batch_index == 0 && (rc = tail_batch(c, S))) return rc;
   if (c->profiling) c->prof.host_wait_ms += std::chrono::duration<double, std::milli>(std::chrono::steady_clock::now() - w0).count();
   Counters cnt = S.counters();
   uint32_t new_tiles = std::min(S.n_tiles(), c->cfg.max_tiles);
@@ -1676,6 +1864,13 @@
   }
   if ((cnt.err & kErrExact) && !(cnt.err & (kErrLabel | kErrIndex)) && (rc = repair_after_fallback(c, S, st, &cnt, &new_tiles))) return rc;
   c->pairs_hint.store(std::max<size_t>(c->pairs_hint.load(std::memory_order_relaxed), cnt.n_pairs), std::memory_order_relaxed);
+  if (S.tail_batched) {
+    S.tail_batched = false;
+    skip_update_stages(c, set);
+    finish_prof(c, set, st, cnt.n_pairs);
+    owe_stats(c, S, cnt, cnt.n_pairs, S.tb_blocks);
+    return KS_OK;
+  }
   if ((cnt.err & kErrPairs) && !(cnt.err & ~kErrPairs) && (rc = repair_after_overflow(c, S, st, &cnt, &new_tiles))) return rc;
   if (new_tiles > c->tiles_initialised) {
     hipLaunchKernelGGL(k_init_tiles, dim3(new_tiles - c->tiles_initialised), dim3(512), 0, st, c->pool, c->tiles_initialised);
@@ -2199,6 +2394,7 @@
     if (P.xlong_own) CRKS(new_stream(&c->stream_xlong));
     else if (c->xlong) c->stream_xlong = c->stream_tail;
     if (const char* ar = dbg_env("KS_APPLY_RUNS")) c->apply_runs_min_pairs = atoi(ar) ? 0ull : ~0ull;
+    if (const char* tb = dbg_env("KS_TAIL_BATCH")) c->tail_batch_on = atoi(tb) != 0;
     if (const char* ll = dbg_env("KS_LONG_LANES")) {
       c->long_lanes = atoi(ll) != 0;
       if (atoi(ll) == 2) c->long_lanes_min_pairs = 0ull;
@@ -4808,6 +5004,19 @@
   return KS_OK;
 }
 
+int ks_tail_batch_stats(ks_ctx* c, uint64_t out[4]) {
+  if (!c || !out) return KS_ERR_INVALID_ARG;
+  for (int i = 0; i < 4; ++i) out[i] = c->tb_stats[i];
+  return KS_OK;
+}
+
+int ks_tail_batch_rule(const uint32_t* err, const uint64_t* n_pairs, int32_t nb, int32_t marcher, int32_t profiling, uint64_t apply_runs_min_pairs) {
+  if (!err || !n_pairs || nb < 0 || nb > kBatchMax) return KS_ERR_INVALID_ARG;
+  unsigned long long np[kBatchMax];
+  for (int k = 0; k < nb; ++k) np[k] = n_pairs[k];
+  return tail_batch_rule(err, np, nb, marcher != 0, profiling, apply_runs_min_pairs, ~0ull) ? 1 : 0;
+}
+
 int ks_stream_plan(ks_ctx* c, int32_t out[8]) {
   if (!c || !out) return KS_ERR_INVALID_ARG;
   const StreamPlan& P = c->plan;
diff --git a/kimera_semantics_amd/csrc/ks_k_apply.h b/kimera_semantics_amd/csrc/ks_k_apply.h
--- a/kimera_semantics_amd/csrc/ks_k_apply.h
+++ b/kimera_semantics_amd/csrc/ks_k_apply.h
@@ -27,14 +27,24 @@
   float sdf, uw, dm, dn;
   uint32_t info, color, rp;
 };
-template <bool HOT_ONLY>
+template <bool HOT_ONLY, bool BATCH = false>
 __device__ __forceinline__ UpdateOps load_update_ops(const FrameParams& F, const RayDesc* __restrict__ rays, uint64_t key,
-                                                     const VoxelRef& v) {
+                                                     const VoxelRef& v, const TailFrame* __restrict__ tab = nullptr) {
   UpdateOps u;
-  u.rp = (uint32_t)key & F.point_mask;
-  const uint4* r4 = (const uint4*)rays + (size_t)ray_index(F, u.rp) * 2;
+  const uint4* r4;
+  f3 origin;
+  if constexpr (BATCH) {
+    const TailFrame& f = tail_frame(F, tab, key);
+    u.rp = (uint32_t)key & f.point_mask;
+    r4 = (const uint4*)f.rays + (size_t)tail_ray_index(f, key) * 2;
+    origin = f.t;
+  } else {
+    u.rp = (uint32_t)key & F.point_mask;
+    r4 = (const uint4*)rays + (size_t)ray_index(F, u.rp) * 2;
+    origin = F.T.t;
+  }
   const uint4 d0 = r4[0];
-  tsdf_operands(F.tsdf, F.T.t, {__uint_as_float(d0.x), __uint_as_float(d0.y), __uint_as_float(d0.z)}, v.vx, v.vy, v.vz,
+  tsdf_operands(F.tsdf, origin, {__uint_as_float(d0.x), __uint_as_float(d0.y), __uint_as_float(d0.z)}, v.vx, v.vy, v.vz,
                 __uint_as_float(d0.w), u.sdf, u.uw);
   if (HOT_ONLY) {
     const uint32_t b = (uint32_t)(key >> 56);
@@ -52,12 +62,26 @@
   return u;
 }
 
-template <int COLOR_MODE, bool MERGED>
-__global__ void __launch_bounds__(256) k_apply(FrameParams F, unsigned long long n_pairs,
-                                               const uint64_t* __restrict__ pairs, const RayDesc* __restrict__ rays,
-                                               const float* __restrict__ deltas, TileTable T, Pool P,
-                                               const uint32_t* __restrict__ label_lut,
-                                               unsigned long long* __restrict__ long_list, Counters* C) {
+template <bool BATCH>
+__device__ __forceinline__ RayDesc pair_ray(const FrameParams& F, const RayDesc* __restrict__ rays, const TailFrame* __restrict__ tab, uint64_t key) {
+  if constexpr (BATCH) {
+    const TailFrame& f = tail_frame(F, tab, key);
+    return f.rays[tail_ray_index(f, key)];
+  } else {
+    return rays[ray_index(F, (uint32_t)key & F.point_mask)];
+  }
+}
+template <bool BATCH>
+__device__ __forceinline__ f3 pair_origin(const FrameParams& F, const TailFrame* __restrict__ tab, uint64_t key) {
+  if constexpr (BATCH) return tail_frame(F, tab, key).t;
+  else return F.T.t;
+}
+
+template <int COLOR_MODE, bool MERGED, bool BATCH>
+__device__ __forceinline__ void apply_body(FrameParams F, unsigned long long n_pairs,
+                                           const uint64_t* __restrict__ pairs, const RayDesc* __restrict__ rays,
+                                           const float* __restrict__ deltas, TileTable T, Pool P,
+                                           const uint32_t* __restrict__ label_lut, const TailFrame* __restrict__ tab) {
   __shared__ uint32_t s_lut[256];
   s_lut[threadIdx.x] = label_lut[threadIdx.x];
   const uint32_t lane = lane_id();
@@ -73,7 +97,7 @@
     vox = (uint32_t)(key >> F.seq_bits);
     head = (i == 0) || ((uint32_t)(pairs[i - 1] >> F.seq_bits) != vox);
     if (head) is_long = (i + kLongRun < n_pairs) && ((uint32_t)(pairs[i + kLongRun] >> F.seq_bits) == vox);
-    u = load_update_ops<!MERGED && COLOR_MODE != KS_COLOR_MODE_COLOR>(F, rays, key, voxel_ref(T, vox));
+    u = load_update_ops<!MERGED && COLOR_MODE != KS_COLOR_MODE_COLOR, BATCH>(F, rays, key, voxel_ref(T, vox), tab);
   }
   __syncthreads();
 
@@ -174,7 +198,7 @@
       for (unsigned long long j = wbase + 64ull; j < n_pairs; ++j) {
         const uint64_t k = pairs[j];
         if ((uint32_t)(k >> F.seq_bits) != hvox) break;
-        const UpdateOps t = load_update_ops<!MERGED && COLOR_MODE != KS_COLOR_MODE_COLOR>(F, rays, k, v);
+        const UpdateOps t = load_update_ops<!MERGED && COLOR_MODE != KS_COLOR_MODE_COLOR, BATCH>(F, rays, k, v, tab);
         if (sub == 0u) {
           tsdf_combine<COLOR_MODE == KS_COLOR_MODE_COLOR>(F.tsdf, t.sdf, t.uw, t.color, dist, weight, color);
         } else if (sub < 7u) {
@@ -219,6 +243,20 @@
     const bool wr = active && sub < 7u;
     rec[wr ? sub : 7u] = wr ? outv : make_uint4(0u, 0u, 0u, 0u);
   }
+}
+template <int COLOR_MODE, bool MERGED>
+__global__ void __launch_bounds__(256) k_apply(FrameParams F, unsigned long long n_pairs,
+                                               const uint64_t* __restrict__ pairs, const RayDesc* __restrict__ rays,
+                                               const float* __restrict__ deltas, TileTable T, Pool P,
+                                               const uint32_t* __restrict__ label_lut,
+                                               unsigned long long* __restrict__ long_list, Counters* C) {
+  apply_body<COLOR_MODE, MERGED, false>(F, n_pairs, pairs, rays, deltas, T, P, label_lut, nullptr);
+}
+template <int COLOR_MODE>
+__global__ void __launch_bounds__(256) k_apply_batch(FrameParams F, unsigned long long n_pairs, const uint64_t* __restrict__ pairs,
+                                                     const TailFrame* __restrict__ tab, TileTable T, Pool P,
+                                                     const uint32_t* __restrict__ label_lut) {
+  apply_body<COLOR_MODE, false, true>(F, n_pairs, pairs, nullptr, nullptr, T, P, label_lut, tab);
 }
 
 constexpr uint32_t kRunPer = 4;
@@ -729,13 +767,13 @@
   }
 }
 
-template <int COLOR_MODE>
-__global__ void __launch_bounds__(128) k_apply_long(FrameParams F, unsigned long long n_pairs,
-                                                   const uint64_t* __restrict__ pairs, const RayDesc* __restrict__ rays,
-                                                   const float* __restrict__ deltas, TileTable T, Pool P,
-                                                   const uint32_t* __restrict__ label_lut,
-                                                   const unsigned long long* __restrict__ long_list, const Counters* C,
-                                                   const LongHdr* __restrict__ H = nullptr) {
+template <int COLOR_MODE, bool BATCH>
+__device__ __forceinline__ void apply_long_body(FrameParams F, unsigned long long n_pairs,
+                                                const uint64_t* __restrict__ pairs, const RayDesc* __restrict__ rays,
+                                                const float* __restrict__ deltas, TileTable T, Pool P,
+                                                const uint32_t* __restrict__ label_lut,
+                                                const unsigned long long* __restrict__ long_list, const Counters* C,
+                                                const LongHdr* __restrict__ H, const TailFrame* __restrict__ tab) {
   __shared__ float s_inc[2][64][kNumLabels];
   __shared__ int s_cnt[2];
   __shared__ uint32_t s_best;
@@ -809,7 +847,7 @@
       key_n[i] = pairs[min(base + 64ull * (PF + i) + lane, last)];
     }
 #pragma unroll
-    for (int i = 0; i < PF; ++i) d_q[i] = rays[ray_index(F, (uint32_t)key_q[i] & F.point_mask)];
+    for (int i = 0; i < PF; ++i) d_q[i] = pair_ray<BATCH>(F, rays, tab, key_q[i]);
 
     auto batch = [&](const uint64_t key_cur, const RayDesc& d) -> bool {
       const bool in = (base + lane < n_pairs) && ((uint32_t)(key_cur >> F.seq_bits) == vox);
@@ -821,9 +859,11 @@
       }
       float sdf = 0.f, uw = 0.f;
       if (in) {
-        const f3 v_point_origin = sub3({d.px, d.py, d.pz}, F.T.t);
+        const f3 origin = pair_origin<BATCH>(F, tab, key_cur);
+        const f3 v_vo = BATCH ? sub3(c, origin) : v_voxel_origin;
+        const f3 v_point_origin = sub3({d.px, d.py, d.pz}, origin);
         const float dist_G = norm3(v_point_origin);
-        const float dist_G_V = dot3(v_voxel_origin, v_point_origin) / dist_G;
+        const float dist_G_V = dot3(v_vo, v_point_origin) / dist_G;
         sdf = dist_G - dist_G_V;
         uw = d.weight;
         if (Pm.use_dropoff && sdf < -Pm.voxel_size) {
@@ -889,7 +929,7 @@
         const uint64_t key_cur = key_q[j];
         const RayDesc d = d_q[j];
         key_q[j] = key_n[j];
-        d_q[j] = rays[ray_index(F, (uint32_t)key_n[j] & F.point_mask)];
+        d_q[j] = pair_ray<BATCH>(F, rays, tab, key_n[j]);
         key_n[j] = pairs[min(base + 64ull * (2 * PF) + lane, last)];
         more = batch(key_cur, d);
         if (!more) break;
@@ -909,13 +949,30 @@
     __syncthreads();
   }
 }
-
 template <int COLOR_MODE>
-__global__ void __launch_bounds__(256) k_apply_xlong(FrameParams F, unsigned long long n_pairs,
-                                                    const uint64_t* __restrict__ pairs, const RayDesc* __restrict__ rays,
-                                                    const float* __restrict__ deltas, TileTable T, Pool P,
-                                                    const uint32_t* __restrict__ label_lut,
-                                                    const unsigned long long* __restrict__ xlong_list, const uint32_t* __restrict__ n_runs_ptr) {
+__global__ void __launch_bounds__(128) k_apply_long(FrameParams F, unsigned long long n_pairs,
+                                                   const uint64_t* __restrict__ pairs, const RayDesc* __restrict__ rays,
+                                                   const float* __restrict__ deltas, TileTable T, Pool P,
+                                                   const uint32_t* __restrict__ label_lut,
+                                                   const unsigned long long* __restrict__ long_list, const Counters* C,
+                                                   const LongHdr* __restrict__ H = nullptr) {
+  apply_long_body<COLOR_MODE, false>(F, n_pairs, pairs, rays, deltas, T, P, label_lut, long_list, C, H, nullptr);
+}
+template <int COLOR_MODE>
+__global__ void __launch_bounds__(128) k_apply_long_batch(FrameParams F, unsigned long long n_pairs, const uint64_t* __restrict__ pairs,
+                                                         const TailFrame* __restrict__ tab, TileTable T, Pool P,
+                                                         const uint32_t* __restrict__ label_lut,
+                                                         const unsigned long long* __restrict__ long_list, const Counters* C) {
+  apply_long_body<COLOR_MODE, true>(F, n_pairs, pairs, nullptr, nullptr, T, P, label_lut, long_list, C, nullptr, tab);
+}
+
+template <int COLOR_MODE, bool BATCH>
+__device__ __forceinline__ void apply_xlong_body(FrameParams F, unsigned long long n_pairs,
+                                                 const uint64_t* __restrict__ pairs, const RayDesc* __restrict__ rays,
+                                                 const float* __restrict__ deltas, TileTable T, Pool P,
+                                                 const uint32_t* __restrict__ label_lut,
+                                                 const unsigned long long* __restrict__ xlong_list, const uint32_t* __restrict__ n_runs_ptr,
+                                                 const TailFrame* __restrict__ tab) {
   __shared__ float s_inc[2][16][kNumLabels][4];
   __shared__ float4 s_tab[3][64];
   __shared__ int s_cnt[3];
@@ -939,7 +996,7 @@
       const unsigned long long last = n_pairs - 1ull;
       auto key_of = [&](unsigned long long own) { return pairs[min(start + 64ull * ((unsigned long long)f + 2ull * own) + lane, last)]; };
       uint64_t key_q[2] = {key_of(0), key_of(1)}, key_n[2] = {key_of(2), key_of(3)};
-      RayDesc d_q[2] = {rays[ray_index(F, (uint32_t)key_q[0] & F.point_mask)], rays[ray_index(F, (uint32_t)key_q[1] & F.point_mask)]};
+      RayDesc d_q[2] = {pair_ray<BATCH>(F, rays, tab, key_q[0]), pair_ray<BATCH>(F, rays, tab, key_q[1])};
       unsigned long long own = 0;
       bool h_in = false;
       uint32_t h_kind = 0, h_lab = 0, h_rp = 0;
@@ -948,15 +1005,17 @@
         const unsigned long long b = (unsigned long long)f + 2ull * own;
         const uint64_t key_cur = key_q[0];
         const RayDesc d = d_q[0];
-        const RayDesc d_new = rays[ray_index(F, (uint32_t)key_n[0] & F.point_mask)];
+        const RayDesc d_new = pair_ray<BATCH>(F, rays, tab, key_n[0]);
         const uint64_t key_new = key_of(own + 4ull);
         const bool in = (start + 64ull * b + lane < n_pairs) && ((uint32_t)(key_cur >> F.seq_bits) == vox);
         const int cnt = (int)__popcll(__ballot(in));
         float sdf = 0.f, uw = 0.f;
         if (in) {
-          const f3 v_point_origin = sub3({d.px, d.py, d.pz}, F.T.t);
+          const f3 origin = pair_origin<BATCH>(F, tab, key_cur);
+          const f3 v_vo = BATCH ? sub3(c, origin) : v_voxel_origin;
+          const f3 v_point_origin = sub3({d.px, d.py, d.pz}, origin);
           const float dist_G = norm3(v_point_origin);
-          const float dist_G_V = dot3(v_voxel_origin, v_point_origin) / dist_G;
+          const float dist_G_V = dot3(v_vo, v_point_origin) / dist_G;
           sdf = dist_G - dist_G_V;
           uw = d.weight;
           if (Pm.use_dropoff && sdf < -Pm.voxel_size) {
@@ -1111,5 +1170,37 @@
     __syncthreads();
   }
 }
-
-}
+template <int COLOR_MODE>
+__global__ void __launch_bounds__(256) k_apply_xlong(FrameParams F, unsigned long long n_pairs,
+                                                    const uint64_t* __restrict__ pairs, const RayDesc* __restrict__ rays,
+                                                    const float* __restrict__ deltas, TileTable T, Pool P,
+                                                    const uint32_t* __restrict__ label_lut,
+                                                    const unsigned long long* __restrict__ xlong_list, const uint32_t* __restrict__ n_runs_ptr) {
+  apply_xlong_body<COLOR_MODE, false>(F, n_pairs, pairs, rays, deltas, T, P, label_lut, xlong_list, n_runs_ptr, nullptr);
+}
+template <int COLOR_MODE>
+__global__ void __launch_bounds__(256) k_apply_xlong_batch(FrameParams F, unsigned long long n_pairs, const uint64_t* __restrict__ pairs,
+                                                          const TailFrame* __restrict__ tab, TileTable T, Pool P,
+                                                          const uint32_t* __restrict__ label_lut,
+                                                          const unsigned long long* __restrict__ xlong_list, const uint32_t* __restrict__ n_runs_ptr) {
+  apply_xlong_body<COLOR_MODE, true>(F, n_pairs, pairs, nullptr, nullptr, T, P, label_lut, xlong_list, n_runs_ptr, tab);
+}
+
+struct PairLists {
+  const uint64_t* src[8];
+  unsigned long long off[9];
+};
+__global__ void __launch_bounds__(256) k_cat_pairs(PairLists L, uint64_t* __restrict__ out) {
+  const uint64_t* __restrict__ src = L.src[blockIdx.y];
+  const unsigned long long n = L.off[blockIdx.y + 1] - L.off[blockIdx.y];
+  uint64_t* __restrict__ dst = out + L.off[blockIdx.y];
+  for (unsigned long long i = (unsigned long long)blockIdx.x * 256ull + threadIdx.x; i < n; i += (unsigned long long)gridDim.x * 256ull) dst[i] = src[i];
+}
+struct TailFrames {
+  TailFrame f[8];
+};
+__global__ void __launch_bounds__(64) k_set_tail_frames(TailFrames B, TailFrame* __restrict__ out) {
+  if (threadIdx.x == 0) out[blockIdx.x] = B.f[blockIdx.x];
+}
+
+}
diff --git a/kimera_semantics_amd/csrc/ks_k_march.h b/kimera_semantics_amd/csrc/ks_k_march.h
--- a/kimera_semantics_amd/csrc/ks_k_march.h
+++ b/kimera_semantics_amd/csrc/ks_k_march.h
@@ -606,7 +606,7 @@
     count = cnt[si] & ~kCntBroke;
     base = s_bt[si / kScanBlock] + lp[si];
     key_lo = ((uint64_t)((d.info & 0x1fu) | (((d.info >> 8) & 3u) << 5) | (((d.info >> 10) & 1u) << 7)) << 56) |
-             (uint64_t)((F.method == KS_METHOD_MERGED && clearing) ? (p | F.clear_bit) : p);
+             (uint64_t)((F.method == KS_METHOD_MERGED && clearing) ? (p | F.clear_bit) : (p | ((F.frame_bits >> 8) << (F.frame_bits & 0xffu))));
     own_key = F.ray_keys ? F.ray_keys[p] : 0ull;
     round.setup(F.T.t, {d.px, d.py, d.pz}, clearing, F.carving != 0, F.max_ray, F.voxel_size_inv, F.trunc,
                 F.method == KS_METHOD_MERGED);
@@ -705,7 +705,7 @@
     count = cnt[si] & ~kCntBroke;
     base = s_bt[si / kScanBlock] + lp[si];
     key_lo = ((uint64_t)((d.info & 0x1fu) | (((d.info >> 8) & 3u) << 5) | (((d.info >> 10) & 1u) << 7)) << 56) |
-             (uint64_t)((F.method == KS_METHOD_MERGED && clearing) ? (p | F.clear_bit) : p);
+             (uint64_t)((F.method == KS_METHOD_MERGED && clearing) ? (p | F.clear_bit) : (p | ((F.frame_bits >> 8) << (F.frame_bits & 0xffu))));
     dda.setup(F.T.t, {d.px, d.py, d.pz}, clearing, F.carving != 0, F.max_ray, F.voxel_size_inv, F.trunc,
               F.method == KS_METHOD_MERGED);
   }
diff --git a/kimera_semantics_amd/csrc/ks_types.h b/kimera_semantics_amd/csrc/ks_types.h
--- a/kimera_semantics_amd/csrc/ks_types.h
+++ b/kimera_semantics_amd/csrc/ks_types.h
@@ -169,6 +169,7 @@
   float start_inv;
   float log_match, log_non_match;
   TsdfParams tsdf;
+  uint32_t frame_bits;
   uint64_t start_offset, observed_offset;
   uint32_t obs_tag, obs_tag_lo;
   uint64_t* observed;
@@ -192,6 +193,13 @@
   uint8_t dynamic_labels[32];
 };
 
+struct TailFrame {
+  const RayDesc* rays;
+  f3 t;
+  uint32_t point_mask, order_groups, order_per;
+  uint32_t pad[2];
+};
+
 __device__ __forceinline__ uint32_t point_order(const FrameParams& F, const uint32_t* order, uint32_t p) {
   if (F.sorted_order) return order[p];
   if (F.order_groups * F.order_per <= p) return p;
@@ -215,6 +223,15 @@
 
 __device__ __forceinline__ uint32_t ray_index(const FrameParams& F, uint32_t p) {
   return (F.method == KS_METHOD_FAST) ? point_order(F, F.order, p) : p;
+}
+
+__device__ __forceinline__ const TailFrame& tail_frame(const FrameParams& F, const TailFrame* __restrict__ tab, uint64_t key) {
+  return tab[((uint32_t)key & ((1u << F.seq_bits) - 1u)) >> (F.frame_bits & 0xffu)];
+}
+__device__ __forceinline__ uint32_t tail_ray_index(const TailFrame& f, uint64_t key) {
+  const uint32_t p = (uint32_t)key & f.point_mask;
+  if (f.order_groups * f.order_per <= p) return p;
+  return (p % f.order_groups) * f.order_per + p / f.order_groups;
 }
 
 __device__ __forceinline__ uint32_t point_position(const FrameParams& F, const uint32_t* inv_order, uint32_t idx) {
```

Result: faster. 1085 Mvoxel-updates/s (median of 6 runs) (+7.0%).
